# welcomyou/sherpa-vietnamese-asr

Measured on AMD Instinct MI355X. Metric: audio-sec/sec (xRT) Zipformer-68M offline decode, higher is better.
Workload: dtype bf16; 1 GPU; zipformer-68m greedy_search, batched planner chunks, 1 h per GPU; model=zipformer-68m, weights=greedy-calibrated, chunks_per_gpu=121, batch_pipeline=True, encoder_frames_per_gpu=98813

## Files before the change

include/zasr.h:

```cpp
#ifndef ZASR_H_
#define ZASR_H_

#include <stdint.h>

#ifdef __cplusplus
extern "C" {
#endif

typedef struct zasr_recognizer zasr_recognizer;
typedef struct zasr_result zasr_result;

enum {
  ZASR_OK = 0,
  ZASR_ERR_INVALID = 1,
  ZASR_ERR_NOT_FOUND = 2,
  ZASR_ERR_RUNTIME = 3,
};

enum {
  ZASR_PRECISION_FP32 = 0,
  ZASR_PRECISION_BF16 = 1,
  ZASR_PRECISION_BF16_ENC = 2,
  ZASR_PRECISION_BF16X3 = 3,
  ZASR_PRECISION_BF16X6 = 4,
  ZASR_PRECISION_F16X3 = 5
};

typedef struct zasr_config {
  const char* model_dir;
  const char* decoding_method;
  int32_t max_active_paths;
  float blank_penalty;
  const int32_t* hotword_tokens;
  const int32_t* hotword_lens;
  const float* hotword_scores;
  int32_t num_hotwords;
  int32_t device_id;
  int32_t precision;
} zasr_config;

int zasr_create(const zasr_config* cfg, zasr_recognizer** out);
void zasr_destroy(zasr_recognizer* h);

int zasr_convert_model(const char* model_dir, const char* out_dir);

int zasr_convert_stage_model(const char* kind, const char* model_dir, const char* out_dir);

int zasr_fbank(zasr_recognizer* h, const float* wav, int64_t n, int32_t sample_rate, float* out,
               int64_t cap, int64_t* n_frames);

int zasr_silence_flags(const float* d_wav, int64_t n, int32_t frame_len, float threshold,
                       uint8_t* d_flags, void* stream);

int zasr_decode_batch(zasr_recognizer* h, const float* const* wav, const int64_t* n,
                      int32_t count, int32_t beam, zasr_result** out);

int zasr_decode_features(zasr_recognizer* h, const float* const* feats, const int64_t* n_frames,
                         int32_t count, int32_t beam, zasr_result** out);

int zasr_decode_device(zasr_recognizer* h, const float* d_wav, const int64_t* wav_off,
                       const int64_t* n, int32_t count, int32_t beam, void* stream,
                       zasr_result** out);

int zasr_decode_device_batches(zasr_recognizer* h, const float* d_wav, const int64_t* wav_off,
                               const int64_t* n, int32_t count, const int32_t* batch_sizes,
                               int32_t n_batches, int32_t beam, void* stream, zasr_result** out);

int zasr_decode_host_batches(zasr_recognizer* h, const float* wav, const int64_t* wav_off,
                             const int64_t* n, int32_t count, const int32_t* batch_sizes,
                             int32_t n_batches, int32_t beam, void* stream, zasr_result** out);

int zasr_encode_features(zasr_recognizer* h, const float* const* feats, const int64_t* n_frames,
                         int32_t count, float* out, int64_t cap, int64_t* t_out);

int zasr_search_encoder_out(zasr_recognizer* h, const float* const* enc, const int64_t* t_out,
                            int32_t count, int32_t beam, zasr_result** out);

int32_t zasr_result_count(const zasr_result* r);
int32_t zasr_result_num_tokens(const zasr_result* r, int32_t i);
int32_t zasr_result_num_frames(const zasr_result* r, int32_t i);
const int32_t* zasr_result_tokens(const zasr_result* r, int32_t i);
const int32_t* zasr_result_frames(const zasr_result* r, int32_t i);
const double* zasr_result_log_probs(const zasr_result* r, int32_t i);
const float* zasr_result_token_stats(const zasr_result* r, int32_t i);
void zasr_result_free(zasr_result* r);

typedef struct zasr_stream zasr_stream;
int zasr_set_tokens(zasr_recognizer* h, const char* tokens_path);
int zasr_create_stream(zasr_recognizer* h, zasr_stream** out);
void zasr_destroy_stream(zasr_stream* s);
int zasr_stream_accept_waveform(zasr_stream* s, int32_t sample_rate, const float* samples,
                                int64_t n);
int zasr_decode_stream(zasr_recognizer* h, zasr_stream* s);
int zasr_decode_streams(zasr_recognizer* h, zasr_stream* const* streams, int32_t n);
int32_t zasr_stream_is_decoded(const zasr_stream* s);
int32_t zasr_stream_num_tokens(const zasr_stream* s);
int32_t zasr_stream_num_frames(const zasr_stream* s);
const int32_t* zasr_stream_tokens(const zasr_stream* s);
const int32_t* zasr_stream_frames(const zasr_stream* s);
const double* zasr_stream_log_probs(const zasr_stream* s);
const float* zasr_stream_token_stats(const zasr_stream* s);
int zasr_stream_result_json(const zasr_stream* s, char* buf, int64_t cap, int64_t* needed);

typedef struct zasr_campp zasr_campp;
int zasr_campp_create(const char* model_dir, int32_t device_id, zasr_campp** out);
void zasr_campp_destroy(zasr_campp* h);
int32_t zasr_campp_embedding_dim(const zasr_campp* h);
int zasr_campp_fbank(zasr_campp* h, const float* wav, int64_t n, float* out, int64_t cap,
                     int64_t* n_frames);
int zasr_campp_embed(zasr_campp* h, const float* feats, int32_t count, int32_t n_frames,
                     float* out);
int zasr_campp_embed_device(zasr_campp* h, const float* d_feats, int32_t count,
                            int32_t n_frames, float* d_out, void* stream);
int zasr_campp_windows_device(zasr_campp* h, const float* d_wav, const int64_t* region_off,
                              const int64_t* region_len, int32_t n_regions, int32_t window_frames,
                              int32_t step_frames, float* d_feats, int64_t max_windows,
                              int32_t* window_region, int32_t* window_first,
                              int32_t* window_nframes, int64_t* n_windows, void* stream);

typedef struct zasr_vibert zasr_vibert;
int zasr_vibert_create(const char* model_dir, int32_t device_id, zasr_vibert** out);
void zasr_vibert_destroy(zasr_vibert* h);
int32_t zasr_vibert_num_labels(const zasr_vibert* h);
int32_t zasr_vibert_num_detect(const zasr_vibert* h);
int zasr_vibert_run(zasr_vibert* h, const int64_t* input_ids, const int64_t* attention_mask,
                    const int64_t* token_type_ids, const int64_t* input_offsets, int32_t batch,
                    int32_t n_tokens, int32_t n_words, float* logits, float* detect_logits);

typedef struct zasr_vad zasr_vad;
int zasr_vad_create(const char* model_dir, int32_t device_id, zasr_vad** out);
void zasr_vad_destroy(zasr_vad* h);
int zasr_vad_probs(zasr_vad* h, const float* audio, const int64_t* offsets,
                   const int64_t* lengths, int32_t n_files, int32_t auto_boost, float* probs);
int zasr_vad_probs_device(zasr_vad* h, const float* d_audio, const int64_t* offsets,
                          const int64_t* lengths, int32_t n_files, int32_t auto_boost,
                          float* d_probs, void* stream);
int32_t zasr_vad_last_passes(const zasr_vad* h);
int zasr_vad_window(zasr_vad* h, const float* input, const float* state, int32_t n, float* prob,
                    float* state_out);

int32_t zasr_vocab_size(const zasr_recognizer* h);
int32_t zasr_joiner_dim(const zasr_recognizer* h);
int zasr_model_routes(zasr_recognizer* h, char* buf, int64_t cap);
int zasr_fbank_set_mel_banks(zasr_recognizer* h, const float* banks, int32_t n_bins);
int zasr_selftest_launch(int32_t block_threads);
int zasr_selftest_gemm_h3r(int32_t M, int32_t K, int32_t N, int32_t epi, const float* A,
                           const float* W, const float* bias, float* C);
int zasr_selftest_ffn_h3(int32_t R, int32_t D, int32_t F, const float* Y, const float* W1,
                         const float* b1, const float* W2, const float* b2,
                         const float* byp_orig, const float* byp_scale, float* X);
int zasr_selftest_ffn_bf16(int32_t R, int32_t D, int32_t F, const float* W1, const float* b1,
                           const float* W2, const float* b2, const float* byp_orig,
                           const float* byp_scale, float* X, int32_t form);
int zasr_selftest_ffn_bf16_oop(int32_t R, int32_t D, int32_t F, const float* W1, const float* b1,
                               const float* W2, const float* b2, const float* byp_orig,
                               const float* byp_scale, float* X, float* Xout, int32_t form);
int zasr_selftest_ffn_h3_oop(int32_t R, int32_t D, int32_t F, const float* W1, const float* b1,
                             const float* W2, const float* b2, const float* byp_orig,
                             const float* byp_scale, float* X, float* Xout);
int zasr_selftest_seam(int32_t nseq, const int32_t* L, int32_t d, int32_t ds, int32_t dn,
                       int32_t ds_next, int32_t c0, int32_t ldo, const float* xd,
                       const float* orig, const float* s, const float* wn8, const float* wo2,
                       float* next, float* xnext, float* out, float* next_ref, float* xnext_ref,
                       float* out_ref);
int zasr_selftest_attn_block_map(const int32_t* lens, int32_t nseq, int32_t units_per_seq,
                                 int32_t order, uint32_t* out, int64_t cap, int32_t* grid);

int zasr_profile_enable(zasr_recognizer* h, int32_t on);
int zasr_profile_reset(zasr_recognizer* h);
int zasr_profile_report(zasr_recognizer* h, char* buf, int64_t cap);

const char* zasr_last_error(void);
const char* zasr_version(void);

#ifdef __cplusplus
}
#endif
#endif
```

sherpa-vietnamese-asr_amd/csrc/engine.cpp:

```cpp
#include "engine.h"

#include <algorithm>
#include <cmath>
#include <cstring>
#include <deque>
#include <numeric>
#include <cstdlib>
#include <sstream>

#include "common.h"
#include "gemm.h"
#include "host_io.h"
#include "onnx_io.h"

namespace zasr {

namespace {
struct HwNode {
  int tok = -1;
  double tok_score = 0, node_score = 0, out_score = 0;
  bool is_end = false;
  std::vector<std::pair<int, int>> kids;
  int fail = 0, out = -1;
  int child(int t) const {
// ... 71 lines not shown
          break;
        }
      }
      nd[kid].out = o;
      if (o >= 0) nd[kid].out_score += nd[o].out_score;
      q.push_back(kid);
    }
  }
  dfa.tok2cls.assign(V, -1);
  std::vector<int> cls_tok;
  for (size_t i = 1; i < nd.size(); ++i) {
    int t = nd[i].tok;
    if (dfa.tok2cls[t] < 0) {
      dfa.tok2cls[t] = (int)cls_tok.size();
      cls_tok.push_back(t);
    }
  }
  dfa.num_states = (int)nd.size();
  dfa.num_cls = (int)cls_tok.size();
  dfa.next.resize((size_t)dfa.num_states * dfa.num_cls);
  dfa.delta.resize((size_t)dfa.num_states * dfa.num_cls);
  dfa.node_score.resize(dfa.num_states);
  for (int s = 0; s < dfa.num_states; ++s) {
    dfa.node_score[s] = nd[s].node_score;
    for (int c = 0; c < dfa.num_cls; ++c) {
      int t = cls_tok[c];
      int n;
      double score;
      int d = nd[s].child(t);
      if (d >= 0) {
        n = d;
        score = nd[n].tok_score;
      } else {
        n = nd[s].fail;
        while (nd[n].child(t) < 0) {
          n = nd[n].fail;
          if (nd[n].tok == -1) break;
        }
        int c2 = nd[n].child(t);
        if (c2 >= 0) n = c2;
        score = nd[n].node_score - nd[s].node_score;
      }
      if (nd[n].out_score != 0) {
        double matched = nd[n].is_end ? nd[n].node_score
                                      : (nd[n].out >= 0 ? nd[nd[n].out].node_score
                                                        : nd[n].node_score);
        score = score + matched - nd[n].node_score;
        n = 0;
      }
      dfa.next[(size_t)s * dfa.num_cls + c] = n;
      dfa.delta[(size_t)s * dfa.num_cls + c] = score;
    }
  }
  return dfa;
}

namespace {

ModelConfig parse_config(const std::string& text) {
  Json j = Json::parse(text);
  ModelConfig c;
  c.name = j.has("name") ? j.at("name").str : "zipformer";
  c.dims = j.at("encoder_dims").as_int_vec();
  c.layers = j.at("num_layers").as_int_vec();
  c.ff = j.at("ff_dims").as_int_vec();
  c.heads = j.at("num_heads").as_int_vec();
  c.ds = j.at("downsampling").as_int_vec();
  c.kernels = j.at("cnn_kernels").as_int_vec();
  c.qd = (int)j.at("query_head_dim").num;
  c.vd = (int)j.at("value_head_dim").num;
  c.pd = (int)j.at("pos_head_dim").num;
  c.pos_dim = (int)j.at("pos_dim").num;
  c.V = (int)j.at("vocab_size").num;
  c.dec_dim = (int)j.at("decoder_dim").num;
  c.joiner_dim = (int)j.at("joiner_dim").num;
  c.context = (int)j.at("context_size").num;
  if (j.has("layer1_channels")) c.c1 = (int)j.at("layer1_channels").num;
  if (j.has("layer2_channels")) c.c2 = (int)j.at("layer2_channels").num;
  if (j.has("layer3_channels")) c.c3 = (int)j.at("layer3_channels").num;
  ZASR_REQUIRE(c.qd == 32 && c.pd == 4, "kernels are specialised for query_head_dim 32, pos_head_dim 4");
  ZASR_REQUIRE(c.c1 == 8 && c.c2 == 32 && c.c3 == 128, "Conv2dSubsampling channels must be 8/32/128");
  ZASR_REQUIRE(c.context == 2, "decoder context_size must be 2");
  ZASR_REQUIRE(c.dec_dim == c.joiner_dim, "decoder_dim must equal joiner_dim");
  size_t ns = c.dims.size();
  ZASR_REQUIRE(c.layers.size() == ns && c.ff.size() == ns && c.heads.size() == ns &&
                   c.ds.size() == ns && c.kernels.size() == ns,
               "inconsistent stack config");
  for (size_t i = 0; i < ns; ++i) {
    ZASR_REQUIRE(c.dims[i] % 16 == 0, "encoder dims must be multiples of 16");
    ZASR_REQUIRE(c.ds[i] >= 1 && c.ds[i] <= 8, "downsampling factor must be 1..8");
  }
  return c;
}

}

template <class T>
T* Engine::ws(const std::string& name, size_t count) {
  size_t bytes = std::max<size_t>(count * sizeof(T), 256);
  Buf& b = ws_tag_.empty() ? ws_[name] : ws_[ws_tag_ + name];
  if (b.bytes < bytes) {
    if (b.p) {
      ZASR_HIP_CHECK(hipDeviceSynchronize());
      ZASR_HIP_CHECK(hipFree(b.p));
    }
    size_t alloc = bytes + bytes / 8;
    ZASR_HIP_CHECK(hipMalloc(&b.p, alloc));
    b.bytes = alloc;
  }
  return reinterpret_cast<T*>(b.p);
}

void Engine::upload(void* dst, const void* src, size_t bytes) {
  PinArena& a = pin_[pin_cur_];
  const size_t need = (bytes + 255) & ~size_t(255);
  if (a.used + need <= a.cap) {
    char* h = a.p + a.used;
    a.used += need;
    std::memcpy(h, src, bytes);
    ZASR_HIP_CHECK(hipMemcpyAsync(dst, h, bytes, hipMemcpyHostToDevice, st_));
    return;
  }
  a.want += need;
  ZASR_HIP_CHECK(hipMemcpyAsync(dst, src, bytes, hipMemcpyHostToDevice, st_));
}

void Engine::pin_reset(int arena) {
  PinArena& a = pin_[arena];
  const size_t want = std::max(a.want + a.used, a.cap);
  if (want > a.cap) {
    if (a.p) ZASR_HIP_CHECK(hipHostFree(a.p));
    a.cap = want + want / 4 + 4096;
    ZASR_HIP_CHECK(hipHostMalloc(reinterpret_cast<void**>(&a.p), a.cap, hipHostMallocDefault));
  }
  a.used = 0;
  a.want = 0;
  pin_cur_ = arena;
}

Engine::Engine(const std::string& dir, int device, int beam, bool greedy,
               const std::vector<std::vector<int>>& hotwords, const std::vector<float>& hotword_scores,
               int precision)
    : device_(device), beam_(beam), greedy_(greedy), precision_(precision) {
  ZASR_REQUIRE(precision >= 0 && precision <= 5,
               "precision must be 0 (fp32), 1 (bf16), 2 (bf16 encoder, f32 joiner + search), 3 "
               "(bf16x3: two-piece split-bf16 products), 4 (bf16x6: three-piece, f32 quality) or "
               "5 (f16x3: fp16 hi + scaled lo pieces, f32 quality)");
  SafeTensors W;
  ModelConfig cfg = parse_config(load_model_dir(dir, W));
  model_.cfg = cfg;
  hw_host_ = build_hotword_dfa(hotwords, hotword_scores, cfg.V);
  ZASR_HIP_CHECK(hipSetDevice(device_));
  if (const char* e = getenv("ZASR_SEARCH_CUS")) search_cus_ = atoi(e);
  int ncu = 0;
  ZASR_HIP_CHECK(hipDeviceGetAttribute(&ncu, hipDeviceAttributeMultiprocessorCount, device_));
  if (search_cus_ > 0 && search_cus_ < ncu) {
    std::vector<uint32_t> ms((ncu + 31) / 32, 0u), me((ncu + 31) / 32, 0u);
    for (int c = 0; c < ncu; ++c) (c < search_cus_ ? ms : me)[c / 32] |= 1u << (c % 32);
    ZASR_HIP_CHECK(hipExtStreamCreateWithCUMask(&stream2_, (uint32_t)ms.size(), ms.data()));
    ZASR_HIP_CHECK(hipExtStreamCreateWithCUMask(&stream3_, (uint32_t)ms.size(), ms.data()));
    ZASR_HIP_CHECK(hipExtStreamCreateWithCUMask(&stream_, (uint32_t)me.size(), me.data()));
    for (auto& x : enc_extra_)
      ZASR_HIP_CHECK(hipExtStreamCreateWithCUMask(&x, (uint32_t)me.size(), me.data()));
  } else {
    search_cus_ = 0;
    ZASR_HIP_CHECK(hipStreamCreateWithFlags(&stream_, hipStreamNonBlocking));
    int least = 0, greatest = 0;
    ZASR_HIP_CHECK(hipDeviceGetStreamPriorityRange(&least, &greatest));
    ZASR_HIP_CHECK(hipStreamCreateWithPriority(&stream2_, hipStreamNonBlocking, greatest));
    ZASR_HIP_CHECK(hipStreamCreateWithPriority(&stream3_, hipStreamNonBlocking, greatest));
    for (auto& x : enc_extra_) ZASR_HIP_CHECK(hipStreamCreateWithFlags(&x, hipStreamNonBlocking));
  }
  for (auto& e : part_ev_) ZASR_HIP_CHECK(hipEventCreateWithFlags(&e, hipEventDisableTiming));
  st_ = stream_;

  auto dev = [&](const float* src, size_t n) -> float* {
    float* p = nullptr;
    ZASR_HIP_CHECK(hipMalloc(&p, std::max<size_t>(n, 1) * sizeof(float)));
    ZASR_HIP_CHECK(hipMemcpy(p, src, n * sizeof(float), hipMemcpyHostToDevice));
    model_.allocations.push_back(p);
    return p;
  };
  auto tensor = [&](const std::string& name, std::initializer_list<int64_t> shape) {
    const HostTensor& t = W.get(name);
    std::vector<int64_t> want(shape);
    ZASR_REQUIRE(t.shape == want, "shape mismatch for " + name);
    return t;
  };
  auto lin = [&](const std::string& pre, int N, int K, bool bias = true) {
    DLin l;
    l.N = N;
    l.K = K;
    const float* hw = tensor(pre + ".weight", {N, K}).data;
    if (precision_ == 5) {
      for (size_t i = 0; i < (size_t)N * K; ++i)
        ZASR_REQUIRE(std::fabs(hw[i]) < 65504.f,
                     "precision f16x3: weight " + pre + " exceeds the fp16 range; use bf16x6");
    }
    l.w = dev(hw, (size_t)N * K);
    if (bias) l.b = dev(tensor(pre + ".bias", {N}).data, N);
    return l;
  };
  auto vec = [&](const std::string& name, int n) { return dev(tensor(name, {n}).data, n); };
  auto scalar = [&](const std::string& name) {
    const HostTensor& t = W.get(name);
    ZASR_REQUIRE(t.numel == 1, name + " must be a scalar");
    return t.data[0];
  };

  {
    const HostTensor& w0 = tensor("encoder_embed.conv.0.weight", {8, 1, 3, 3});
    model_.conv0_w = dev(w0.data, 72);
    model_.conv0_b = vec("encoder_embed.conv.0.bias", 8);
    const HostTensor& w4 = tensor("encoder_embed.conv.4.weight", {32, 8, 3, 3});
    std::vector<float> p4(32 * 72);
    for (int o = 0; o < 32; ++o)
      for (int c = 0; c < 8; ++c)
        for (int kk = 0; kk < 9; ++kk) p4[o * 72 + kk * 8 + c] = w4.data[(o * 8 + c) * 9 + kk];
    model_.conv4 = DLin{dev(p4.data(), p4.size()), vec("encoder_embed.conv.4.bias", 32), 32, 72};
    const HostTensor& w7 = tensor("encoder_embed.conv.7.weight", {128, 32, 3, 3});
    std::vector<float> p7(128 * 288);
    for (int o = 0; o < 128; ++o)
      for (int c = 0; c < 32; ++c)
        for (int kk = 0; kk < 9; ++kk) p7[o * 288 + kk * 32 + c] = w7.data[(o * 32 + c) * 9 + kk];
    model_.conv7 = DLin{dev(p7.data(), p7.size()), vec("encoder_embed.conv.7.bias", 128), 128, 288};
    model_.dw_w = dev(tensor("encoder_embed.convnext.depthwise_conv.weight", {128, 1, 7, 7}).data,
                      128 * 49);
    model_.dw_b = vec("encoder_embed.convnext.depthwise_conv.bias", 128);
    model_.pw1 = DLin{dev(tensor("encoder_embed.convnext.pointwise_conv1.weight", {384, 128, 1, 1})
                              .data, 384 * 128),
                      vec("encoder_embed.convnext.pointwise_conv1.bias", 384), 384, 128};
    model_.pw2 = DLin{dev(tensor("encoder_embed.convnext.pointwise_conv2.weight", {128, 384, 1, 1})
                              .data, 128 * 384),
                      vec("encoder_embed.convnext.pointwise_conv2.bias", 128), 128, 384};
    const int d0 = cfg.dims[0];
    const HostTensor& wo = tensor("encoder_embed.out.weight", {d0, 128 * 19});
    std::vector<float> po((size_t)d0 * 2432);
    for (int n = 0; n < d0; ++n)
      for (int c = 0; c < 128; ++c)
        for (int f = 0; f < 19; ++f) po[(size_t)n * 2432 + f * 128 + c] = wo.data[(size_t)n * 2432 + c * 19 + f];
    model_.out = DLin{dev(po.data(), po.size()), vec("encoder_embed.out.bias", d0), d0, 2432};
    model_.out_norm_b = vec("encoder_embed.out_norm.bias", d0);
    model_.out_norm_ls = scalar("encoder_embed.out_norm.log_scale");
  }
  const int qd = cfg.qd, vd = cfg.vd, pd = cfg.pd;
  for (size_t i = 0; i < cfg.dims.size(); ++i) {
    DStack s;
    s.d = cfg.dims[i];
    s.F = cfg.ff[i];
    s.h = cfg.heads[i];
    s.ds = cfg.ds[i];
    s.K = cfg.kernels[i];
    const int d = s.d, F = s.F, h = s.h;
    std::string pre = "encoder.encoders." + std::to_string(i) + ".";
    if (s.ds != 1) {
      const HostTensor& b = tensor(pre + "downsample.bias", {s.ds});
      double mx = -1e30, sum = 0;
      for (int u = 0; u < s.ds; ++u) mx = std::max(mx, (double)b.data[u]);
      std::vector<double> e(s.ds);
      for (int u = 0; u < s.ds; ++u) sum += (e[u] = std::exp((double)b.data[u] - mx));
      for (int u = 0; u < s.ds; ++u) s.ds_w[u] = (float)(e[u] / sum);
      s.comb = vec(pre + "out_combiner.bypass_scale", d);
      pre += "encoder.";
    }
    for (int j = 0; j < cfg.layers[i]; ++j) {
      DLayer L;
      std::string p = pre + "layers." + std::to_string(j) + ".";
      L.bypass = vec(p + "bypass.bypass_scale", d);
      L.bypass_mid = vec(p + "bypass_mid.bypass_scale", d);
      L.attn_in = lin(p + "self_attn_weights.in_proj", (2 * qd + pd) * h, d);
      const HostTensor& pw = tensor(p + "self_attn_weights.linear_pos.weight", {pd * h, cfg.pos_dim});
      L.pos_w.assign(pw.data, pw.data + pw.numel);
      for (int a = 0; a < 2; ++a) {
        std::string n = p + "self_attn" + std::to_string(a + 1);
        L.sa_in[a] = lin(n + ".in_proj", vd * h, d);
        L.sa_out[a] = lin(n + ".out_proj", d, vd * h);
      }
      const int fdims[3] = {(F * 3) / 4, F, (F * 5) / 4};
      for (int a = 0; a < 3; ++a) {
        std::string n = p + "feed_forward" + std::to_string(a + 1);
        L.ff_in[a] = lin(n + ".in_proj", fdims[a], d);
        L.ff_out[a] = lin(n + ".out_proj", d, fdims[a]);
      }
      const int hid = 3 * d / 4;
      L.na_in = lin(p + "nonlin_attention.in_proj", 3 * hid, d);
      L.na_out = lin(p + "nonlin_attention.out_proj", d, hid);
      for (int a = 0; a < 2; ++a) {
        std::string n = p + "conv_module" + std::to_string(a + 1);
        L.cv_in[a] = lin(n + ".in_proj", 2 * d, d);
        L.cv_out[a] = lin(n + ".out_proj", d, d);
        L.cv_dw_w[a] = dev(tensor(n + ".depthwise_conv.weight", {d, 1, s.K}).data, (size_t)d * s.K);
        L.cv_dw_b[a] = vec(n + ".depthwise_conv.bias", d);
      }
      L.norm_b = vec(p + "norm.bias", d);
      L.norm_ls = scalar(p + "norm.log_scale");
      s.layers.push_back(std::move(L));
    }
    model_.stacks.push_back(std::move(s));
  }
  {
    const HostTensor& b = tensor("encoder.downsample_output.bias", {2});
    double mx = std::max(b.data[0], b.data[1]);
    double e0 = std::exp(b.data[0] - mx), e1 = std::exp(b.data[1] - mx);
    model_.out_ds_w[0] = (float)(e0 / (e0 + e1));
    model_.out_ds_w[1] = (float)(e1 / (e0 + e1));
  }
// ... 86 lines not shown
            }
            ++routes_.ffn_fused_h3;
            for (auto [l, w] : {std::pair<DLin*, std::vector<float>*>{&L.ff_in[a], &w1},
                                std::pair<DLin*, std::vector<float>*>{&L.ff_out[a], &w2}}) {
              std::vector<__bf16> pk(2 * w->size());
              ffn_pack_h3_host(w->data(), l->N, l->K, pk.data());
              void* p = nullptr;
              ZASR_HIP_CHECK(hipMalloc(&p, pk.size() * 2));
              model_.allocations.push_back(p);
              ZASR_HIP_CHECK(hipMemcpy(p, pk.data(), pk.size() * 2, hipMemcpyHostToDevice));
              l->wp = p;
            }
          }
    }
    if (cfg.joiner_dim == 256 || cfg.joiner_dim == 512) {
      const long pe = gemm_rp_packed_elems(cfg.V, cfg.joiner_dim);
      void* p = nullptr;
      ZASR_HIP_CHECK(hipMalloc(&p, (size_t)pe * 2 * stored_pieces(split_pieces())));
      model_.allocations.push_back(p);
      for (int t = 0; t < stored_pieces(split_pieces()); ++t)
        gemm_rp_pack_weights(reinterpret_cast<const __bf16*>(model_.joiner.wx) + (long)t * cfg.V * cfg.joiner_dim,
                             cfg.V, cfg.joiner_dim, reinterpret_cast<__bf16*>(p) + t * pe, stream_);
      model_.joiner_packed = p;
      model_.joiner_plane = pe;
    }
    for (auto& s : model_.stacks)
      for (auto& L : s.layers) {
        for (int a = 0; a < 2; ++a) glu_interleave(L.cv_in[a]);
        for (DLin* l : {&L.attn_in, &L.na_in, &L.na_out}) mkx(*l);
        for (int a = 0; a < 2; ++a)
          for (DLin* l : {&L.sa_in[a], &L.sa_out[a], &L.cv_in[a], &L.cv_out[a]}) mkx(*l);
        for (int a = 0; a < 3; ++a)
          for (DLin* l : {&L.ff_in[a], &L.ff_out[a]}) mkx(*l);
      }
    ZASR_HIP_CHECK(hipStreamSynchronize(stream_));
    if (split_pieces() == kPiecesF16) {
      auto mkr = [&](DLin& l) {
        if (!gemm_h3r_supported(l.K, l.N, EPI_NONE)) return;
        std::vector<float> w((size_t)l.N * l.K);
        ZASR_HIP_CHECK(hipMemcpy(w.data(), l.w, w.size() * 4, hipMemcpyDeviceToHost));
        if (!ffn_h3_weights_ok(w.data(), (long)w.size())) {
          ++routes_.gemm_x3_range;
          return;
        }
        ++routes_.gemm_h3r;
        std::vector<__bf16> pk(2 * w.size());
        ffn_pack_h3_host(w.data(), l.N, l.K, pk.data());
        void* p = nullptr;
        ZASR_HIP_CHECK(hipMalloc(&p, pk.size() * 2));
        model_.allocations.push_back(p);
        ZASR_HIP_CHECK(hipMemcpy(p, pk.data(), pk.size() * 2, hipMemcpyHostToDevice));
        l.wr = p;
      };
      for (auto& s : model_.stacks)
        for (auto& L : s.layers) {
          for (DLin* l : {&L.attn_in, &L.na_in, &L.na_out}) mkr(*l);
          for (int a = 0; a < 2; ++a)
            for (DLin* l : {&L.sa_in[a], &L.sa_out[a], &L.cv_in[a], &L.cv_out[a]}) mkr(*l);
        }
      if (model_.pw1.K == 128 && model_.pw2.N == 128 && ffn_h3_supported(128, model_.pw1.N)) {
        std::vector<float> w1((size_t)model_.pw1.N * 128), w2(w1.size());
        ZASR_HIP_CHECK(hipMemcpy(w1.data(), model_.pw1.w, w1.size() * 4, hipMemcpyDeviceToHost));
        ZASR_HIP_CHECK(hipMemcpy(w2.data(), model_.pw2.w, w2.size() * 4, hipMemcpyDeviceToHost));
        const bool ok = ffn_h3_weights_ok(w1.data(), (long)w1.size()) && ffn_h3_weights_ok(w2.data(), (long)w2.size());
        routes_.cnx_ffn_h3 = ok ? 1 : 0;
        if (ok)
          for (auto [l, w] : {std::pair<DLin*, std::vector<float>*>{&model_.pw1, &w1},
                              std::pair<DLin*, std::vector<float>*>{&model_.pw2, &w2}}) {
            std::vector<__bf16> pk(2 * w->size());
            ffn_pack_h3_host(w->data(), l->N, l->K, pk.data());
            void* p = nullptr;
            ZASR_HIP_CHECK(hipMalloc(&p, pk.size() * 2));
            model_.allocations.push_back(p);
            ZASR_HIP_CHECK(hipMemcpy(p, pk.data(), pk.size() * 2, hipMemcpyHostToDevice));
            l->wr = p;
          }
      }
    }
  }
  if (precision_ == 1 || precision_ == 2) {
    for (auto& s : model_.stacks)
      for (auto& L : s.layers)
        for (int a = 0; a < 2; ++a) glu_interleave(L.cv_in[a]);
    auto mk = [&](DLin& l) {
      void* p = nullptr;
      ZASR_HIP_CHECK(hipMalloc(&p, (size_t)l.N * l.K * 2));
      model_.allocations.push_back(p);
      convert_to_bf16(l.w, p, (long)l.N * l.K, stream_);
      l.wh = p;
    };
    for (DLin* l : {&model_.conv4, &model_.conv7, &model_.pw1, &model_.pw2, &model_.out,
                    &model_.enc_proj})
      mk(*l);
    if (precision_ == 1) mk(model_.joiner);
    if (precision_ == 1 && (cfg.joiner_dim == 256 || cfg.joiner_dim == 512)) {
      void* p = nullptr;
      ZASR_HIP_CHECK(hipMalloc(&p, (size_t)gemm_rp_packed_elems(cfg.V, cfg.joiner_dim) * 2));
      model_.allocations.push_back(p);
      gemm_rp_pack_weights(model_.joiner.wh, cfg.V, cfg.joiner_dim, p, stream_);
      model_.joiner_packed = p;
    }
    for (auto& s : model_.stacks)
      for (auto& L : s.layers) {
        {
          DLin& l = L.attn_in;
          const int h = s.h;
          std::vector<float> rs(l.N, 1.f), bias(l.N);
          const float kLog2e = 1.4426950408889634f;
          for (int r = 0; r < l.N; ++r)
            if (r < 32 * h || r >= 64 * h) rs[r] = kLog2e;
          ZASR_HIP_CHECK(hipMemcpy(bias.data(), l.b, l.N * sizeof(float), hipMemcpyDeviceToHost));
          for (int r = 0; r < l.N; ++r) bias[r] *= rs[r];
          float* d_rs = dev(rs.data(), rs.size());
          l.bh = dev(bias.data(), bias.size());
          void* p = nullptr;
          ZASR_HIP_CHECK(hipMalloc(&p, (size_t)l.N * l.K * 2));
          model_.allocations.push_back(p);
          convert_rows_to_bf16(l.w, d_rs, p, l.N, l.K, stream_);
          l.wh = p;
        }
        for (DLin* l : {&L.na_in, &L.na_out}) mk(*l);
        for (int a = 0; a < 2; ++a)
          for (DLin* l : {&L.sa_in[a], &L.sa_out[a], &L.cv_in[a], &L.cv_out[a]}) mk(*l);
        for (int a = 0; a < 3; ++a)
          for (DLin* l : {&L.ff_in[a], &L.ff_out[a]}) mk(*l);
      }
    ZASR_HIP_CHECK(hipStreamSynchronize(stream_));
    for (DLin* l : {&model_.pw1, &model_.pw2}) {
      std::vector<__bf16> h((size_t)l->N * l->K), pk(h.size());
      ZASR_HIP_CHECK(hipMemcpy(h.data(), l->wh, h.size() * 2, hipMemcpyDeviceToHost));
      pack_frag32_host(h.data(), l->N, l->K, pk.data());
      void* p = nullptr;
      ZASR_HIP_CHECK(hipMalloc(&p, pk.size() * 2));
      model_.allocations.push_back(p);
      ZASR_HIP_CHECK(hipMemcpy(p, pk.data(), pk.size() * 2, hipMemcpyHostToDevice));
      l->wp = p;
    }
    for (auto& s : model_.stacks)
      for (auto& L : s.layers)
        for (int a = 0; a < 3; ++a) {
          const int F = L.ff_in[a].N, d = L.ff_in[a].K;
          if (d < 256 || !ffn_fused_supported(d) || F % 32 != 0 || F > 2048) continue;
          for (DLin* l : {&L.ff_in[a], &L.ff_out[a]}) {
            std::vector<__bf16> h((size_t)l->N * l->K), pk(h.size());
            ZASR_HIP_CHECK(hipMemcpy(h.data(), l->wh, h.size() * 2, hipMemcpyDeviceToHost));
            ffn_pack_host(h.data(), l->N, l->K, pk.data());
            void* p = nullptr;
            ZASR_HIP_CHECK(hipMalloc(&p, pk.size() * 2));
            model_.allocations.push_back(p);
            ZASR_HIP_CHECK(hipMemcpy(p, pk.data(), pk.size() * 2, hipMemcpyHostToDevice));
            l->wp = p;
          }
        }
  }
  {
    const double gb = (double)cfg.V * cfg.V * cfg.joiner_dim * 4.0 / 1e9;
    double max_gb = 24.0;
    if (const char* e = getenv("ZASR_DEC_TABLE_MAX_GB")) max_gb = atof(e);
    if (gb <= max_gb) {
      void* p = nullptr;
      ZASR_HIP_CHECK(hipMalloc(&p, (size_t)cfg.V * cfg.V * cfg.joiner_dim * sizeof(float)));
      model_.allocations.push_back(p);
      model_.dec_table = reinterpret_cast<float*>(p);
      DecoderW dw{model_.dec_tap0, model_.dec_tap1, model_.dec_proj.b, cfg.joiner_dim};
      launch_dec_table(dw, model_.dec_proj.w, cfg.V, model_.dec_table, stream_);
      ZASR_HIP_CHECK(hipStreamSynchronize(stream_));
    }
  }

  {
    std::vector<double> tw(512);
    for (int j = 0; j < 256; ++j) {
      double a = -2.0 * M_PI * j / 512.0;
      tw[2 * j] = std::cos(a);
      tw[2 * j + 1] = std::sin(a);
    }
    ZASR_HIP_CHECK(hipMalloc(&d_twiddle_, 512 * sizeof(double)));
    ZASR_HIP_CHECK(hipMemcpy(d_twiddle_, tw.data(), 512 * sizeof(double), hipMemcpyHostToDevice));
    std::vector<float> win(400);
    for (int i = 0; i < 400; ++i)
      win[i] = (float)std::pow(0.5 - 0.5 * std::cos(2.0 * M_PI / 399.0 * i), 0.85);
    d_window_ = dev(win.data(), 400);
    auto mel = [](float f) { return 1127.0f * logf(1.0f + f / 700.0f); };
    const float mlo = mel(20.0f), mhi = mel(7600.0f);
    const float delta = (mhi - mlo) / 81.0f;
    std::vector<float> banks(80 * 256, 0.f);
    for (int b = 0; b < 80; ++b) {
      float left = mlo + (float)b * delta, center = mlo + (float)(b + 1) * delta,
            right = mlo + (float)(b + 2) * delta;
      for (int i = 0; i < 256; ++i) {
        float m = mel(31.25f * (float)i);
        if (m > left && m < right)
          banks[b * 256 + i] = (m <= center) ? (m - left) / (center - left) : (right - m) / (right - center);
      }
    }
    set_mel_banks(banks.data(), 256);
  }
  hw_.num_states = hw_host_.num_states;
  hw_.num_cls = hw_host_.num_cls;
  if (hw_host_.num_states > 0) {
    int *t2c = nullptr, *nx = nullptr;
    double *dl = nullptr, *ns = nullptr;
    ZASR_HIP_CHECK(hipMalloc(&t2c, hw_host_.tok2cls.size() * sizeof(int)));
    ZASR_HIP_CHECK(hipMalloc(&nx, std::max<size_t>(hw_host_.next.size(), 1) * sizeof(int)));
    ZASR_HIP_CHECK(hipMalloc(&dl, std::max<size_t>(hw_host_.delta.size(), 1) * sizeof(double)));
    ZASR_HIP_CHECK(hipMalloc(&ns, hw_host_.node_score.size() * sizeof(double)));
    ZASR_HIP_CHECK(hipMemcpy(t2c, hw_host_.tok2cls.data(), hw_host_.tok2cls.size() * sizeof(int), hipMemcpyHostToDevice));
    ZASR_HIP_CHECK(hipMemcpy(nx, hw_host_.next.data(), hw_host_.next.size() * sizeof(int), hipMemcpyHostToDevice));
    ZASR_HIP_CHECK(hipMemcpy(dl, hw_host_.delta.data(), hw_host_.delta.size() * sizeof(double), hipMemcpyHostToDevice));
    ZASR_HIP_CHECK(hipMemcpy(ns, hw_host_.node_score.data(), hw_host_.node_score.size() * sizeof(double), hipMemcpyHostToDevice));
    model_.allocations.push_back(t2c);
    model_.allocations.push_back(nx);
    model_.allocations.push_back(dl);
    model_.allocations.push_back(ns);
    hw_.tok2cls = t2c;
    hw_.next = nx;
    hw_.delta = dl;
    hw_.node_score = ns;
  }
  ZASR_HIP_CHECK(hipHostMalloc(reinterpret_cast<void**>(&h_pinned_), 64, hipHostMallocDefault));
  ZASR_HIP_CHECK(hipDeviceSynchronize());
}

void Engine::set_mel_banks(const float* banks, int n_bins) {
  ZASR_REQUIRE(n_bins == 256 || n_bins == 257, "mel banks: 256 or 257 bins per filter");
  std::vector<int> meta(240);
  std::vector<float> wts;
  for (int b = 0; b < 80; ++b) {
    const float* row = banks + (size_t)b * n_bins;
    if (n_bins == 257)
      ZASR_REQUIRE(row[256] == 0.f, "mel banks: the Nyquist bin must carry no weight");
    int st = -1, en = -1;
    for (int i = 0; i < 256; ++i)
      if (row[i] != 0.f) {
        if (st < 0) st = i;
        en = i;
      }
    if (st < 0) st = en = 0;
    meta[b] = st;
    meta[80 + b] = en - st + 1;
    meta[160 + b] = (int)wts.size();
    for (int i = st; i <= en; ++i) wts.push_back(row[i]);
  }
  ZASR_HIP_CHECK(hipDeviceSynchronize());
  if (!d_mel_meta_) ZASR_HIP_CHECK(hipMalloc(&d_mel_meta_, 240 * sizeof(int)));
  ZASR_HIP_CHECK(hipMemcpy(d_mel_meta_, meta.data(), 240 * sizeof(int), hipMemcpyHostToDevice));
  if (d_mel_w_) ZASR_HIP_CHECK(hipFree(d_mel_w_));
  d_mel_w_ = nullptr;
  ZASR_HIP_CHECK(hipMalloc(&d_mel_w_, wts.size() * sizeof(float)));
  ZASR_HIP_CHECK(hipMemcpy(d_mel_w_, wts.data(), wts.size() * sizeof(float), hipMemcpyHostToDevice));
}

std::string Engine::routes_json() const {
  std::ostringstream os;
  os << "{\"precision\": " << precision_ << ", \"ffn_fused_h3\": " << routes_.ffn_fused_h3
     << ", \"ffn_gemm_pair\": " << routes_.ffn_gemm_pair << ", \"gemm_h3r\": " << routes_.gemm_h3r
     << ", \"gemm_x3_range\": " << routes_.gemm_x3_range << ", \"cnx_ffn_h3\": " << routes_.cnx_ffn_h3
     << ", \"dec_table\": " << (model_.dec_table ? 1 : 0) << "}";
  return os.str();
}

Engine::~Engine() {
  (void)hipSetDevice(device_);
  (void)hipStreamSynchronize(stream_);
  for (void* p : model_.allocations) (void)hipFree(p);
  for (auto& s : model_.stacks)
    for (auto& l : s.layers)
      if (l.pos_tab) (void)hipFree(l.pos_tab);
  for (auto& kv : ws_)
    if (kv.second.p) (void)hipFree(kv.second.p);
  if (d_twiddle_) (void)hipFree(d_twiddle_);
  if (d_mel_meta_) (void)hipFree(d_mel_meta_);
  if (d_mel_w_) (void)hipFree(d_mel_w_);
  for (auto e : event_pool_) (void)hipEventDestroy(e);
  for (auto& pe : prof_pending_) {
    (void)hipEventDestroy(pe.a);
    (void)hipEventDestroy(pe.b);
  }
  if (copy_st_) (void)hipStreamSynchronize(copy_st_);
  for (auto e : upload_ev_)
    if (e) (void)hipEventDestroy(e);
  if (copy_st_) (void)hipStreamDestroy(copy_st_);
  (void)hipStreamSynchronize(stream2_);
  (void)hipStreamSynchronize(stream3_);
  if (stream4_) (void)hipStreamSynchronize(stream4_);
  if (h_pinned_) (void)hipHostFree(h_pinned_);
  for (auto& r : res_pin_)
    if (r.p) (void)hipHostFree(r.p);
  for (auto& a : pin_)
    if (a.p) (void)hipHostFree(a.p);
  for (auto e : part_ev_) (void)hipEventDestroy(e);
  (void)hipStreamDestroy(stream2_);
  (void)hipStreamDestroy(stream3_);
  if (stream4_) (void)hipStreamDestroy(stream4_);
  for (auto x : enc_extra_) {
    (void)hipStreamSynchronize(x);
    (void)hipStreamDestroy(x);
  }
  (void)hipStreamDestroy(stream_);
}

void Engine::ensure_pos_tables(int need) {
  if (need <= model_.pmax) return;
  ZASR_HIP_CHECK(hipDeviceSynchronize());
  int pmax = 1024;
  while (pmax < need) pmax *= 2;
// ... 80 lines not shown
    acc.second += ms;
    event_pool_.push_back(pe.a);
    event_pool_.push_back(pe.b);
  }
  prof_pending_.clear();
  std::ostringstream os;
  for (auto& kv : prof_acc_) os << kv.first << " " << kv.second.first << " " << kv.second.second << "\n";
  return os.str();
}

std::string Engine::shape_key(const char* cls, int M, int K, int N, bool w16, bool a16, bool c16,
                              int epi) {
  std::ostringstream os;
  os << cls << "|" << M << "|" << K << "|" << N << "|" << (int)w16 << "|" << (int)a16 << "|"
     << (int)c16 << "|" << epi;
  return os.str();
}

void Engine::linear(const DLin& l, const float* A, int lda, int M, float* C, int ldc, int epi,
                    const char* cls, const float* byp_orig, const float* byp_scale) {
  GemmParams p{};
  p.A = A;
  p.lda = lda;
  p.B = l.w;
  p.sbk = 1;
  p.sbn = l.K;
  p.C = C;
  p.ldc = ldc;
  p.bias = l.b;
  p.M = M;
  p.N = l.N;
  p.K = l.K;
  p.alpha = 1.f;
  p.max_M = M;
  ZASR_REQUIRE(byp_orig == nullptr || l.wx, "bypass epilogue: split-mode weights only");
  p.byp_orig = byp_orig;
  p.byp_scale = byp_scale;
  if (prof_shapes_ && prof_on_)
    prof_begin(shape_key(cls, M, l.K, l.N, l.wh != nullptr, false, false, epi));
  else
    prof_begin(cls);
  if (l.wr && lda == l.K && byp_orig == nullptr && gemm_h3r_supported(l.K, l.N, epi))
    gemm_h3r(A, l.wr, l.b, C, ldc, M, l.N, l.K, epi, st_);
  else if (l.wx)
    gemm_x3(p, l.wx, (long)l.N * l.K, epi, ALOAD_DENSE, st_, split_pieces());
  else if (l.wh)
    gemm_bf16(p, l.wh, epi, ALOAD_DENSE, st_);
  else
    gemm_f32(p, epi, ALOAD_DENSE, false, st_);
  prof_end();
}

void Engine::linear_h(const DLin& l, const void* A, bool a_bf16, int lda, int M, void* C,
                      bool c_bf16, int ldc, int epi, const float* byp_orig,
                      const float* byp_scale) {
  ZASR_REQUIRE(l.wh != nullptr, "linear_h needs bf16 weights");
  GemmParams p{};
  p.A = reinterpret_cast<const float*>(A);
  p.lda = lda;
  p.B = l.w;
  p.sbk = 1;
  p.sbn = l.K;
  p.C = reinterpret_cast<float*>(C);
  p.ldc = ldc;
  p.bias = l.bh ? l.bh : l.b;
  p.M = M;
  p.N = l.N;
  p.K = l.K;
  p.alpha = 1.f;
  p.max_M = M;
  p.byp_orig = byp_orig;
  p.byp_scale = byp_scale;
  if (prof_shapes_ && prof_on_)
    prof_begin(shape_key("enc_gemm", M, l.K, l.N, true, a_bf16, c_bf16, epi));
  else
    prof_begin("enc_gemm");
  gemm_bf16(p, l.wh, epi, ALOAD_DENSE, st_, a_bf16, c_bf16);
  prof_end();
}

void Engine::run_fbank(const float* d_wav, const std::vector<long>& wav_off,
                       const std::vector<long>& n, float* d_feats, std::vector<int>& frames) {
  const int B = (int)n.size();
  std::vector<long> off(B);
  std::vector<int> ns(B), fo(B + 1, 0);
  frames.resize(B);
  for (int b = 0; b < B; ++b) {
    off[b] = wav_off[b];
    ns[b] = (int)n[b];
    frames[b] = n[b] > 0 ? (int)((n[b] + 80) / 160) : 0;
    fo[b + 1] = fo[b] + frames[b];
  }
  long* d_off = ws<long>("fb_wavoff", B);
  int* d_meta = ws<int>("fb_meta", 2 * B + 1);
  std::vector<int> meta(ns);
  meta.insert(meta.end(), fo.begin(), fo.end());
  upload(d_off, off.data(), B * sizeof(long));
  upload(d_meta, meta.data(), meta.size() * sizeof(int));
  FbankTables t{d_twiddle_, d_window_, d_mel_meta_, d_mel_meta_ + 80, d_mel_meta_ + 160, d_mel_w_};
  prof_begin("fbank");
  launch_fbank(d_wav, d_off, d_meta, d_meta + B, B, fo[B], t, d_feats, st_);
  prof_end();
}

namespace {
struct LevelMeta {
  std::vector<int> len;
  std::vector<int> off;
  int total = 0, maxlen = 0;
};
LevelMeta make_level(const std::vector<int>& len) {
  LevelMeta m;
  m.len = len;
  m.off.assign(len.size() + 1, 0);
  for (size_t b = 0; b < len.size(); ++b) {
    m.off[b + 1] = m.off[b] + len[b];
    m.maxlen = std::max(m.maxlen, len[b]);
  }
  m.total = m.off.back();
  return m;
}
struct MetaPack {
  std::vector<char> bytes;
  size_t add(const void* p, size_t n) {
    size_t at = (bytes.size() + 15) & ~size_t(15);
    bytes.resize(at + n);
    if (n) std::memcpy(bytes.data() + at, p, n);
    return at;
  }
};
}

bool Engine::ff1_fused(const DStack& S, const DLayer& Ly) const {
  const DLin& fi = Ly.ff_in[0];
  if (fi.wh) return ffn_fused_supported(S.d) && (S.d < 256 || fi.wp);
  return fi.wp && split_pieces() == kPiecesF16 && ffn_h3_oop_ok(S.d);
}

float* Engine::layer_forward(const DStack& S, const DLayer& Ly, float* X, float* Xalt, int R,
                             const int* d_off, const int* d_map,
                             const std::vector<int>& lens, const long* d_aoff,
                             const void* d_slices_nl, int maxL, const int* d_o8, int R8,
                             const AttnBlockMaps& bm, bool orig_ready, bool copy_for_next) {
  const int d = S.d, h = S.h, B = (int)lens.size();
  const int hid = 3 * d / 4;
  const bool oop = ff1_fused(S, Ly);
  float* O = X;
  if (!oop) {
    O = ws<float>("ly_orig", (size_t)R * d);
    if (!orig_ready)
      ZASR_HIP_CHECK(hipMemcpyAsync(O, X, (size_t)R * d * sizeof(float), hipMemcpyDeviceToDevice, st_));
  }
  const bool bf16 = precision_ == 1 || precision_ == 2;
  const int np = split_pieces();
  float* qkp = nullptr;
  float* A = nullptr;
  __bf16* A16 = nullptr;
  float* stats = nullptr;
  AttnFlashArgs fa{};
  if (bf16) {
    __bf16* qkp16 = ws<__bf16>("ly_qkp_h", (size_t)R * 68 * h);
    linear_h(Ly.attn_in, X, false, d, R, qkp16, true, 68 * h, EPI_NONE);
    A16 = ws<__bf16>("ly_attn_h", 1);
    stats = ws<float>("ly_attn_stats", (size_t)R * h);
    fa = AttnFlashArgs{qkp16, h, Ly.pos_tab, model_.pmax, d_off, d_aoff, B, maxL, A16,
                       nullptr, nullptr, stats, stats};
  } else if (np) {
    qkp = ws<float>("ly_qkp", (size_t)R * 68 * h);
    linear(Ly.attn_in, X, d, R, qkp, 68 * h, EPI_NONE);
    A = ws<float>("ly_attn", 1);
    stats = ws<float>("ly_attn_stats", (size_t)R * h);
    fa = AttnFlashArgs{qkp, h, Ly.pos_tab, model_.pmax, d_off, d_aoff, B, maxL, A,
                       nullptr, nullptr, stats, stats, np};
    if (np != kPiecesF16) {
      AttnFlashArgs a = fa;
      a.map = bm.head0;
      a.map_len = bm.n_head0;
      prof_begin("attn_softmax");
      launch_attn_flash(a, 0, st_);
      prof_end();
    }
  } else {
    qkp = ws<float>("ly_qkp", (size_t)R * 68 * h);
    linear(Ly.attn_in, X, d, R, qkp, 68 * h, EPI_NONE);
    A = ws<float>("ly_attn", 1);
    stats = ws<float>("ly_attn_stats", (size_t)R * h * 2);
    AttnArgs a{qkp, h, Ly.pos_tab, model_.pmax, d_off, d_aoff, B, maxL, A, stats, 1};
    prof_begin("attn_softmax");
    launch_attn_softmax(a, st_);
    prof_end();
  }
  auto ff = [&](int k, const float* src = nullptr) {
    const DLin& fi = Ly.ff_in[k];
    const float* bo = (bf16 && k == 1) ? O : nullptr;
    const float* bs = (bf16 && k == 1) ? Ly.bypass_mid : nullptr;
    if (fi.wh && ffn_fused_supported(d) && (d < 256 || fi.wp)) {
      prof_begin("ffn_fused");
      launch_ffn_fused(X, R, d, fi.N, d < 256 ? fi.wh : fi.wp, fi.b,
                       d < 256 ? Ly.ff_out[k].wh : Ly.ff_out[k].wp, Ly.ff_out[k].b, st_, bo, bs, src);
      prof_end();
      return;
    }
    ZASR_REQUIRE(src == nullptr || (!fi.wh && fi.wp && np == kPiecesF16),
                 "feed-forward: only the fused kernels run out of place");
    if (fi.wh) {
      __bf16* H = ws<__bf16>("ly_hid_h", (size_t)R * fi.N);
      linear_h(fi, X, false, d, R, H, true, fi.N, EPI_SWOOSHL);
      linear_h(Ly.ff_out[k], H, true, fi.N, R, X, false, d, EPI_RESADD, bo, bs);
    } else if (fi.wp && np == kPiecesF16) {
      prof_begin("ffn_fused");
      launch_ffn_fused_h3(X, R, d, fi.N, fi.wp, fi.b, Ly.ff_out[k].wp, Ly.ff_out[k].b, st_,
                          k == 1 ? O : nullptr, k == 1 ? Ly.bypass_mid : nullptr, nullptr, src);
      prof_end();
    } else {
      const bool byp = k == 1 && Ly.ff_out[k].wx != nullptr;
      float* H = ws<float>("ly_hid", (size_t)R * fi.N);
      linear(fi, X, d, R, H, fi.N, EPI_SWOOSHL);
      linear(Ly.ff_out[k], H, fi.N, R, X, d, EPI_RESADD, "enc_gemm", byp ? O : nullptr,
             byp ? Ly.bypass_mid : nullptr);
    }
  };
  auto self_attn = [&](int k) {
    if (bf16) {
      __bf16* vv = ws<__bf16>("ly_vv_h", (size_t)R * 12 * h);
      __bf16* oa = ws<__bf16>("ly_oa_h", (size_t)R * 12 * h);
      linear_h(Ly.sa_in[k], X, false, d, R, vv, true, 12 * h, EPI_NONE);
      AttnFlashArgs a = fa;
      a.v = vv;
      a.out = oa;
      a.map = bm.heads;
      a.map_len = bm.n_heads;
      prof_begin("attn_apply");
      launch_attn_flash(a, k == 0 ? 1 : 2, st_);
      prof_end();
      linear_h(Ly.sa_out[k], oa, true, 12 * h, R, X, false, d, EPI_RESADD);
      return;
    }
    float* vv = ws<float>("ly_vv", (size_t)R * 12 * h);
    float* oa = ws<float>("ly_oa", (size_t)R * 12 * h);
    linear(Ly.sa_in[k], X, d, R, vv, 12 * h, EPI_NONE);
    if (np) {
      AttnFlashArgs a = fa;
      a.v = vv;
      a.out = oa;
      a.map = bm.heads;
      a.map_len = bm.n_heads;
      prof_begin("attn_apply");
      launch_attn_flash(a, k == 0 ? 1 : 2, st_);
      prof_end();
      linear(Ly.sa_out[k], oa, 12 * h, R, X, d, EPI_RESADD);
      return;
    }
    AttnSAArgs sa{qkp, h, Ly.pos_tab, model_.pmax, d_off, B, maxL, stats, vv, oa, stats};
    prof_begin("attn_apply");
    launch_attn_sa(sa, k == 0, false, st_);
    prof_end();
    linear(Ly.sa_out[k], oa, 12 * h, R, X, d, EPI_RESADD);
  };
  auto conv = [&](int k) {
    if (Ly.cv_in[k].wh) {
      __bf16* dc = ws<__bf16>("ly_dc_h", (size_t)R * d);
      if (Ly.cv_in[k].glu) {
        __bf16* g = ws<__bf16>("ly_glu_h", (size_t)R * d);
        linear_h(Ly.cv_in[k], X, false, d, R, g, true, d, EPI_GLU);
        prof_begin("dwconv1d");
        launch_dwconv1d_post_glu_bf16(g, d_off, d_map, R, d, S.K, Ly.cv_dw_w[k], Ly.cv_dw_b[k], dc, st_);
        prof_end();
      } else {
        __bf16* g2 = ws<__bf16>("ly_g2_h", (size_t)R * 2 * d);
        linear_h(Ly.cv_in[k], X, false, d, R, g2, true, 2 * d, EPI_NONE);
        prof_begin("dwconv1d");
        launch_glu_dwconv1d_bf16(g2, d_off, d_map, R, d, S.K, Ly.cv_dw_w[k], Ly.cv_dw_b[k], dc, st_);
        prof_end();
      }
      linear_h(Ly.cv_out[k], dc, true, d, R, X, false, d, EPI_RESADD);
      return;
    }
    float* dc = ws<float>("ly_dc", (size_t)R * d);
    if (Ly.cv_in[k].glu) {
      float* g = ws<float>("ly_glu", (size_t)R * d);
      linear(Ly.cv_in[k], X, d, R, g, d, EPI_GLU);
      prof_begin("dwconv1d");
      launch_dwconv1d_post_glu(g, d_off, d_map, R, d, S.K, Ly.cv_dw_w[k], Ly.cv_dw_b[k], dc, st_);
      prof_end();
    } else {
      float* g2 = ws<float>("ly_g2", (size_t)R * 2 * d);
      linear(Ly.cv_in[k], X, d, R, g2, 2 * d, EPI_NONE);
      prof_begin("dwconv1d");
      launch_glu_dwconv1d(g2, d_off, d_map, R, d, S.K, Ly.cv_dw_w[k], Ly.cv_dw_b[k], dc, st_);
      prof_end();
    }
    linear(Ly.cv_out[k], dc, d, R, X, d, EPI_RESADD);
  };
  if (oop) {
    X = Xalt;
    ff(0, O);
  } else {
    ff(0);
  }
  if (bf16) {
    __bf16* h3 = ws<__bf16>("ly_h3_h", (size_t)R * 3 * hid);
    __bf16* t1t = ws<__bf16>("ly_t1t", (size_t)hid * R8);
    __bf16* z = ws<__bf16>("ly_z_h", (size_t)R * hid);
    linear_h(Ly.na_in, X, false, d, R, h3, true, 3 * hid, EPI_NONE);
    prof_begin("elementwise");
    launch_nonlin_prep_t(h3, true, d_off, d_o8, d_map, R, hid, R8, t1t, st_);
    prof_end();
    AttnFlashArgs a = fa;
    a.t1t = t1t;
    a.o8 = d_o8;
    a.ldt = R8;
    a.hid = hid;
    a.y = h3 + 2 * hid;
    a.ldy = 3 * hid;
    a.z = z;
    a.map = bm.head0;
    a.map_len = bm.n_head0;
    prof_begin("attn_nonlin");
    launch_attn_flash(a, 3, st_);
    prof_end();
    linear_h(Ly.na_out, z, true, hid, R, X, false, d, EPI_RESADD);
  } else if (np) {
    float* h3 = ws<float>("ly_h3", (size_t)R * 3 * hid);
    __bf16* t1t = ws<__bf16>("ly_t1t_x", (size_t)stored_pieces(np) * hid * R8);
    float* z = ws<float>("ly_z", (size_t)R * hid);
    linear(Ly.na_in, X, d, R, h3, 3 * hid, EPI_NONE);
    prof_begin("elementwise");
    launch_nonlin_prep_t(h3, false, d_off, d_o8, d_map, R, hid, R8, t1t, st_, np);
    prof_end();
    if (np == kPiecesF16) {
      AttnFlashArgs a = fa;
      a.t1t = t1t;
      a.o8 = d_o8;
      a.ldt = R8;
      a.hid = hid;
      a.y = h3 + 2 * hid;
      a.ldy = 3 * hid;
      a.z = z;
      a.map = bm.head0;
      a.map_len = bm.n_head0;
      prof_begin("attn_nonlin");
      launch_attn_flash(a, 3, st_);
      prof_end();
    } else {
    GemmParams p{};
    p.A = A;
    p.B = nullptr;
    p.sbk = 1;
    p.sbn = R8;
    p.C = z;
    p.ldc = hid;
    p.N = hid;
    p.alpha = 1.f;
    p.aux = h3 + 2 * hid;
    p.ldaux = 3 * hid;
    p.slices = reinterpret_cast<const GemmSlice*>(d_slices_nl);
    p.num_slices = B;
    p.max_M = maxL;
    prof_begin("attn_nonlin");
    gemm_x3(p, t1t, (long)hid * R8, EPI_MULAUX, ALOAD_DENSE, st_, np);
    prof_end();
    }
    linear(Ly.na_out, z, hid, R, X, d, EPI_RESADD);
  } else {
    float* h3 = ws<float>("ly_h3", (size_t)R * 3 * hid);
    float* t1 = ws<float>("ly_t1", (size_t)R * hid);
    float* z = ws<float>("ly_z", (size_t)R * hid);
    linear(Ly.na_in, X, d, R, h3, 3 * hid, EPI_NONE);
    prof_begin("elementwise");
    launch_nonlin_prep(h3, t1, R, hid, st_);
    prof_end();
    GemmParams p{};
    p.A = A;
    p.B = t1;
    p.sbk = hid;
    p.sbn = 1;
    p.C = z;
    p.ldc = hid;
    p.N = hid;
    p.alpha = 1.f;
    p.aux = h3 + 2 * hid;
    p.ldaux = 3 * hid;
    p.slices = reinterpret_cast<const GemmSlice*>(d_slices_nl);
    p.num_slices = B;
    p.max_M = maxL;
    prof_begin("attn_nonlin");
    gemm_f32(p, EPI_MULAUX, ALOAD_DENSE, true, st_);
    prof_end();
    linear(Ly.na_out, z, hid, R, X, d, EPI_RESADD);
  }
  self_attn(0);
  conv(0);
  ff(1);
  if (!bf16 && Ly.ff_out[1].wx == nullptr) {
    prof_begin("elementwise");
    launch_bypass(X, O, Ly.bypass_mid, R, d, st_);
    prof_end();
  }
  self_attn(1);
  conv(1);
  ff(2);
  prof_begin("elementwise");
  launch_bias_norm(X, R, d, Ly.norm_b, Ly.norm_ls, O, Ly.bypass, st_,
                   copy_for_next ? ws<float>("ly_orig", (size_t)R * d) : nullptr);
  prof_end();
  return X;
}

void Engine::run_encoder(const float* d_feats, const std::vector<int>& T, float* d_enc,
                         std::vector<int>& t_out) {
  const ModelConfig& cfg = model_.cfg;
  const int B = (int)T.size();
  std::vector<int> t1(B), l2(B), L(B), tout(B);
  for (int b = 0; b < B; ++b) {
    ZASR_REQUIRE(T[b] >= 9, "encoder needs >= 9 fbank frames per chunk");
    t1[b] = T[b] - 2;
    l2[b] = (T[b] - 3) / 2;
    L[b] = (T[b] - 7) / 2;
    tout[b] = (L[b] + 1) / 2;
  }
  t_out = tout;
  LevelMeta mfb = make_level(T), mc1 = make_level(t1), mc2 = make_level(l2), mL = make_level(L),
            mout = make_level(tout);
  const int ns = (int)model_.stacks.size();
  std::vector<LevelMeta> mst(ns);
  std::vector<std::vector<long>> aoff(ns);
  std::vector<std::vector<GemmSlice>> sl_nl(ns);
  std::vector<std::vector<int>> o8(ns);
  std::vector<int> R8(ns, 0);
  const bool bf16 = precision_ == 1 || precision_ == 2;
  const bool flash = bf16 || split_pieces() > 0;
  size_t attn_floats = 0;
  int maxL_all = 0;
  for (int i = 0; i < ns; ++i) {
    const DStack& s = model_.stacks[i];
    std::vector<int> len(B);
    for (int b = 0; b < B; ++b) len[b] = (L[b] + s.ds - 1) / s.ds;
    mst[i] = make_level(len);
    maxL_all = std::max(maxL_all, mst[i].maxlen);
    long acc = 0;
    const int hid = 3 * s.d / 4;
    int c8 = 0;
    for (int b = 0; b < B; ++b) {
      const int Lb = len[b], L4 = (Lb + 3) & ~3, L8 = (Lb + 31) & ~31;
      const int Lp = flash ? L8 : L4;
      aoff[i].push_back(acc);
      o8[i].push_back(c8);
      GemmSlice g{};
      g.a_off = acc;
      g.b_off = flash ? (long)c8 : (long)mst[i].off[b] * hid;
      g.c_off = (long)mst[i].off[b] * hid;
      g.aux_off = (long)mst[i].off[b] * 3 * hid;
      g.M = Lb;
      g.K = flash ? L8 : Lb;
      g.lda = Lp;
      sl_nl[i].push_back(g);
      acc += (long)Lb * Lp;
      c8 += L8;
    }
    o8[i].push_back(c8);
    R8[i] = c8;
    attn_floats = std::max(attn_floats, (size_t)acc);
  }
  ensure_pos_tables(maxL_all + 192);
  std::vector<GemmSlice> sl_c2(B), sl_c3(B);
  for (int b = 0; b < B; ++b) {
    sl_c2[b] = GemmSlice{(long)mc1.off[b] * 640, 0, (long)mc2.off[b] * 39 * 32, 0, l2[b] * 39, 72, 0, 0};
    sl_c3[b] = GemmSlice{(long)mc2.off[b] * 39 * 32, 0, (long)mL.off[b] * 19 * 128, 0, L[b] * 19, 288, 0, 0};
  }
  MetaPack mp;
  size_t o_fb = mp.add(mfb.off.data(), (B + 1) * 4), o_c1 = mp.add(mc1.off.data(), (B + 1) * 4),
         o_L = mp.add(mL.off.data(), (B + 1) * 4), o_out = mp.add(mout.off.data(), (B + 1) * 4);
  size_t o_c2s = mp.add(sl_c2.data(), B * sizeof(GemmSlice)),
         o_c3s = mp.add(sl_c3.data(), B * sizeof(GemmSlice));
  std::vector<size_t> o_st(ns), o_ao(ns), o_sn(ns), o_o8(ns), o_bmh(ns), o_bm0(ns);
  std::vector<int> n_bmh(ns, 0), n_bm0(ns, 0);
  std::vector<unsigned> bmap;
  for (int i = 0; i < ns; ++i) {
    o_st[i] = mp.add(mst[i].off.data(), (B + 1) * 4);
    o_o8[i] = mp.add(o8[i].data(), (B + 1) * 4);
    o_ao[i] = mp.add(aoff[i].data(), B * sizeof(long));
    o_sn[i] = mp.add(sl_nl[i].data(), sl_nl[i].size() * sizeof(GemmSlice));
    if (flash) {
      const DStack& s = model_.stacks[i];
      const int np = split_pieces();
      const bool fused_nl = bf16 || np == kPiecesF16;
      n_bmh[i] = build_attn_block_map(mst[i].len.data(), B, s.h, 0, bmap);
      o_bmh[i] = mp.add(bmap.data(), bmap.size() * sizeof(unsigned));
      n_bm0[i] = build_attn_block_map(mst[i].len.data(), B,
                                      fused_nl ? attn_nonlin_chunks(3 * s.d / 4, bf16 ? 1 : np) : 1,
                                      0, bmap);
      o_bm0[i] = mp.add(bmap.data(), bmap.size() * sizeof(unsigned));
    }
  }
  char* d_meta = ws<char>("enc_meta", mp.bytes.size());
  upload(d_meta, mp.bytes.data(), mp.bytes.size());
  auto I = [&](size_t o) { return reinterpret_cast<const int*>(d_meta + o); };
  int* c1_map = ws<int>("map_c1", mc1.total);
  int* L_map = ws<int>("map_L", mL.total);
  int* out_map = ws<int>("map_out", mout.total);
  launch_row2seq(I(o_c1), B, mc1.total, c1_map, st_);
  launch_row2seq(I(o_L), B, mL.total, L_map, st_);
  launch_row2seq(I(o_out), B, mout.total, out_map, st_);
  std::vector<int*> st_map(ns);
  for (int i = 0; i < ns; ++i) {
    st_map[i] = ws<int>("map_st" + std::to_string(i), mst[i].total);
    launch_row2seq(I(o_st[i]), B, mst[i].total, st_map[i], st_);
  }

  const bool fe16 = model_.conv4.wh != nullptr && model_.conv7.wh != nullptr;
  void* c1 = fe16 ? (void*)ws<__bf16>("fe_c1_h", (size_t)mc1.total * 640)
                  : (void*)ws<float>("fe_c1", (size_t)mc1.total * 640);
  prof_begin("frontend_conv");
  launch_conv1(d_feats, I(o_fb), I(o_c1), c1_map, mc1.total, model_.conv0_w, model_.conv0_b, c1,
               fe16, st_, split_pieces() == kPiecesF16);
  prof_end();
  void* c2 = fe16 ? (void*)ws<__bf16>("fe_c2_h", (size_t)mc2.total * 39 * 32)
                  : (void*)ws<float>("fe_c2", (size_t)mc2.total * 39 * 32);
  {
    GemmParams p{};
    p.A = reinterpret_cast<const float*>(c1);
    p.B = model_.conv4.w;
    p.sbk = 1;
    p.sbn = 72;
    p.C = reinterpret_cast<float*>(c2);
    p.ldc = 32;
    p.bias = model_.conv4.b;
    p.N = 32;
    p.alpha = 1.f;
    p.slices = reinterpret_cast<const GemmSlice*>(d_meta + o_c2s);
    p.num_slices = B;
    p.max_M = mc2.maxlen * 39;
    prof_begin("frontend_conv");
    if (fe16)
      gemm_bf16(p, model_.conv4.wh, EPI_SWOOSHR, ALOAD_CONV2, st_, true, true);
    else if (model_.conv4.wx)
      gemm_x3(p, model_.conv4.wx, 32L * 72, EPI_SWOOSHR, ALOAD_CONV2, st_, split_pieces());
    else if (model_.conv4.wh)
      gemm_bf16(p, model_.conv4.wh, EPI_SWOOSHR, ALOAD_CONV2, st_);
    else
      gemm_f32(p, EPI_SWOOSHR, ALOAD_CONV2, false, st_);
    prof_end();
  }
  const int d0 = cfg.dims[0];
  float* e0 = ws<float>("fe_e0", (size_t)mL.total * d0);
  {
// ... 831 lines not shown
```

sherpa-vietnamese-asr_amd/csrc/engine.h:

```cpp
#pragma once
#include <hip/hip_runtime.h>

#include <map>
#include <mutex>
#include <string>
#include <vector>

#include "gemm.h"
#include "kernels.h"

namespace zasr {

struct ModelConfig {
  std::string name;
  std::vector<int> dims, layers, ff, heads, ds, kernels;
  int qd = 32, vd = 12, pd = 4, pos_dim = 48;
  int V = 0, dec_dim = 0, joiner_dim = 0, context = 2;
  int c1 = 8, c2 = 32, c3 = 128;
  int max_dim() const {
    int m = 0;
    for (int d : dims) m = d > m ? d : m;
    return m;
  }
};
// ... 33 lines not shown
  ModelConfig cfg;
  float *conv0_w = nullptr, *conv0_b = nullptr;
  DLin conv4, conv7, pw1, pw2, out, enc_proj, dec_proj, joiner;
  float *dw_w = nullptr, *dw_b = nullptr;
  float* out_norm_b = nullptr;
  float out_norm_ls = 0.f;
  std::vector<DStack> stacks;
  float out_ds_w[2] = {0, 0};
  float* dec_emb = nullptr;
  float* dec_conv = nullptr;
  void* joiner_packed = nullptr;
  long joiner_plane = 0;
  float* dec_table = nullptr;
  float* dec_tap0 = nullptr;
  float* dec_tap1 = nullptr;
  int pmax = 0;
  std::vector<void*> allocations;
};

struct HotwordDFA {
  int num_states = 0, num_cls = 0;
  std::vector<int> tok2cls, next;
  std::vector<double> delta, node_score;
};
HotwordDFA build_hotword_dfa(const std::vector<std::vector<int>>& phrases,
                             const std::vector<float>& scores, int V);

struct TokenResult {
  std::vector<int> tok, frame;
  std::vector<double> lp;
  std::vector<float> stats;
  int t_out = 0;
};

class Engine {
 public:
  Engine(const std::string& model_dir, int device, int beam, bool greedy,
         const std::vector<std::vector<int>>& hotwords, const std::vector<float>& hotword_scores,
         int precision);
  ~Engine();

  int vocab() const { return model_.cfg.V; }
  int joiner_dim() const { return model_.cfg.joiner_dim; }
  int default_beam() const { return beam_; }
  hipStream_t stream() const { return stream_; }

  std::vector<TokenResult> decode_device(const float* d_wav, const std::vector<long>& wav_off,
                                         const std::vector<long>& n, int beam, hipStream_t st);
  std::vector<TokenResult> decode_device_batches(const float* d_wav, const std::vector<long>& wav_off,
                                                 const std::vector<long>& n,
                                                 const std::vector<int>& batch_sizes, int beam,
                                                 hipStream_t st);
  std::vector<TokenResult> decode_host_batches(const float* h_wav, const std::vector<long>& wav_off,
                                               const std::vector<long>& n,
                                               const std::vector<int>& batch_sizes, int beam,
                                               hipStream_t st);
  std::vector<TokenResult> decode_features(const std::vector<const float*>& feats,
                                           const std::vector<long>& frames, int beam);
  void fbank_host(const float* wav, long n, float* out);
  void encode_host(const std::vector<const float*>& feats, const std::vector<long>& frames,
                   std::vector<float>& out, std::vector<int>& t_out);
  std::vector<TokenResult> search_host(const std::vector<const float*>& enc,
                                       const std::vector<long>& t_out, int beam);

  void profile_enable(int mode) {
    prof_on_ = mode > 0;
    prof_shapes_ = mode == 2;
  }
  void profile_reset();
  std::string profile_report();

  std::string routes_json() const;
  void set_mel_banks(const float* banks, int n_bins);

  std::mutex mu;

 private:
  struct Buf {
    void* p = nullptr;
    size_t bytes = 0;
  };
  template <class T>
  T* ws(const std::string& name, size_t count);
  void upload(void* dst, const void* src, size_t bytes);

  struct Pending {
    int B = 0;
    std::vector<int> valid, t_out;
    float* enc = nullptr;
    hipEvent_t ready = nullptr;
  };
  void encode_stage(const float* d_wav, const std::vector<long>& wav_off, const std::vector<long>& n,
                    int out_slot, int ws_slot, hipStream_t stream, Pending& p);
  std::vector<TokenResult> search_stage(Pending& p, int beam);
  std::vector<TokenResult> decode_batches_two_searches(const float* d_wav,
                                                       const std::vector<long>& wav_off,
                                                       const std::vector<long>& n,
                                                       const std::vector<int>& batch_sizes,
                                                       int beam, hipStream_t main_st);
  struct PinArena {
    char* p = nullptr;
    size_t cap = 0, used = 0, want = 0;
  };
  static constexpr int kMaxEnc = 3;
  static constexpr int kMaxJobs = 3;
  PinArena pin_[kMaxEnc + 1 + kMaxJobs];
  std::string ws_tag_;
  int pin_cur_ = 0;
  void pin_reset(int arena);

  void run_fbank(const float* d_wav, const std::vector<long>& wav_off, const std::vector<long>& n,
                 float* d_feats, std::vector<int>& frames);
  void run_encoder(const float* d_feats, const std::vector<int>& T, float* d_enc,
                   std::vector<int>& t_out);
  std::vector<TokenResult> run_search(const float* d_enc, const std::vector<int>& t_out, int beam);
  struct SearchJob {
    int S_all = 0, S = 0, cap = 0, set = 0, Tmax = 0;
    std::vector<int> order, t_out;
    bool check_finite = false;
    hipStream_t stream = nullptr;
  };
  void launch_search(const float* d_enc, const std::vector<int>& t_out, int beam, int set,
                     hipStream_t stream, bool split_groups, SearchJob& job);
  std::vector<TokenResult> collect_search(SearchJob& job);
  struct ResPin {
    char* p = nullptr;
    size_t cap = 0;
  };
  ResPin res_pin_[kMaxJobs];
  float* layer_forward(const DStack& stk, const DLayer& ly, float* X, float* Xalt, int R,
                       const int* d_off, const int* d_map, const std::vector<int>& lens,
                       const long* d_aoff, const void* d_slices_nl, int maxL, const int* d_o8,
                       int R8, const AttnBlockMaps& bm, bool orig_ready, bool copy_for_next);
  bool ff1_fused(const DStack& stk, const DLayer& ly) const;
  void linear(const DLin& l, const float* A, int lda, int M, float* C, int ldc, int epi,
              const char* cls = "enc_gemm", const float* byp_orig = nullptr,
              const float* byp_scale = nullptr);
  void linear_h(const DLin& l, const void* A, bool a_bf16, int lda, int M, void* C, bool c_bf16,
                int ldc, int epi, const float* byp_orig = nullptr,
                const float* byp_scale = nullptr);
  void ensure_pos_tables(int max_len);

  struct ProfEvent {
    std::string name;
    hipEvent_t a, b;
  };
  void prof_begin(const char* name);
  void prof_begin(const std::string& name);
  void prof_end();
  static std::string shape_key(const char* cls, int M, int K, int N, bool w16, bool a16,
                               bool c16, int epi);
  bool prof_on_ = false;
  bool prof_shapes_ = false;
  std::vector<ProfEvent> prof_pending_;
  std::map<std::string, std::pair<long, double>> prof_acc_;
  std::vector<hipEvent_t> event_pool_;
  hipEvent_t take_event();

  DModel model_;
  struct Routes {
    int ffn_fused_h3 = 0, ffn_gemm_pair = 0;
    int gemm_h3r = 0, gemm_x3_range = 0;
    int cnx_ffn_h3 = -1;
  } routes_;
  int device_ = 0;
  int beam_ = 8;
  [[maybe_unused]] bool greedy_ = false;
  void order_after_encoders(const hipStream_t* enc_st, int E, hipStream_t main_st);
  int precision_ = 0;
  int split_pieces() const {
    return precision_ == 3 ? 2 : precision_ == 4 ? 3 : precision_ == 5 ? kPiecesF16 : 0;
  }
  hipStream_t stream_ = nullptr;
  hipStream_t stream2_ = nullptr;
  hipStream_t stream3_ = nullptr;
  hipStream_t stream4_ = nullptr;
  int search_cus_ = 0;
  hipStream_t enc_extra_[kMaxEnc - 1] = {};
  hipEvent_t part_ev_[kMaxEnc + 4 + kMaxJobs] = {};
  hipStream_t st_ = nullptr;
  const float* host_wav_ = nullptr;
  hipStream_t copy_st_ = nullptr;
  hipEvent_t upload_ev_[kMaxEnc + 1] = {};
  std::map<std::string, Buf> ws_;
  double* d_twiddle_ = nullptr;
  float* d_window_ = nullptr;
  int* d_mel_meta_ = nullptr;
  float* d_mel_w_ = nullptr;
  int* h_pinned_ = nullptr;
  HotwordDFA hw_host_;
  HotwordTables hw_{};
};

}
```

sherpa-vietnamese-asr_amd/csrc/ffn_kernels.hip:

```cpp
#include <cmath>
#include <cstring>
#include <cstdlib>
#include <type_traits>
#include <vector>

#include "common.h"
#include "kernels.h"

namespace zasr {

#ifdef ZASR_FFN_STAMPS
__device__ long long g_ffn_stamps[4896];
#define FFN_STAMP(i) \
  if (blockIdx.x == 0 && threadIdx.x == 0 && (i) < 4896) g_ffn_stamps[(i)] = clock64();
#else
#define FFN_STAMP(i)
#endif

namespace {

__device__ __forceinline__ void lds_barrier() {
  asm volatile("s_waitcnt lgkmcnt(0)" ::: "memory");
  __builtin_amdgcn_s_barrier();
}

typedef float f32x16 __attribute__((ext_vector_type(16)));
typedef __bf16 bf16x8 __attribute__((ext_vector_type(8)));
typedef __bf16 bf16x4 __attribute__((ext_vector_type(4)));

constexpr int kTok = 128;
constexpr int kMaxF = 2048;
constexpr int kW2Ld = 40;

__device__ __forceinline__ int w2_slot(int k) { return (k & 0x13) | ((k & 4) << 1) | ((k & 8) >> 1); }

__device__ __forceinline__ __amdgpu_buffer_rsrc_t wave_rsrc(const void* p, long bytes) {
  const unsigned lo = __builtin_amdgcn_readfirstlane((unsigned)(unsigned long)p);
  const unsigned hi = __builtin_amdgcn_readfirstlane((unsigned)((unsigned long)p >> 32));
  const int n = __builtin_amdgcn_readfirstlane((int)bytes);
  return __builtin_amdgcn_make_buffer_rsrc((void*)(((unsigned long)hi << 32) | lo), 0, n, 0x00020000);
}
template <typename V>
__device__ __forceinline__ V buf_load16(__amdgpu_buffer_rsrc_t rs, int voff, int soff) {
  return __builtin_bit_cast(V, __builtin_amdgcn_raw_buffer_load_b128(rs, voff, soff, 0));
}

}

__device__ __forceinline__ void lds_wait_ge(int* p, int target) {
  while (__hip_atomic_load(p, __ATOMIC_ACQUIRE, __HIP_MEMORY_SCOPE_WORKGROUP) < target)
    __builtin_amdgcn_s_sleep(1);
}
__device__ __forceinline__ void lds_signal(int* p, int lane) {
  asm volatile("s_waitcnt lgkmcnt(0)" ::: "memory");
  if (lane == 0) __hip_atomic_fetch_add(p, 1, __ATOMIC_RELEASE, __HIP_MEMORY_SCOPE_WORKGROUP);
}

template <int D, bool OOP = false>
__global__ __launch_bounds__(256, (D <= 192 ? 2 : 1)) void ffn_fused_kernel(float* __restrict__ X, int R, int F,
                                                           const __bf16* __restrict__ W1,
                                                           const float* __restrict__ b1,
                                                           const __bf16* __restrict__ W2,
                                                           const float* __restrict__ b2,
                                                           const float* __restrict__ byp_orig,
                                                           const float* __restrict__ byp_scale,
                                                           const float* __restrict__ Xsrc) {
  const float* Xin = OOP ? Xsrc : X;
  constexpr int KS = D / 16;
  constexpr int OT = D / 32;
  constexpr int W1LD = D + 8;
  constexpr int W1P = 32 * D / 8;
  constexpr int W2P = D * 4;
  constexpr int P1 = (W1P + 255) / 256, P2 = (W2P + 255) / 256;
  __shared__ __attribute__((aligned(16))) __bf16 sW1[2][32 * W1LD];
  __shared__ __attribute__((aligned(16))) __bf16 sW2[2][D * kW2Ld];
  __shared__ float sB1[2][32];

  const int tid = threadIdx.x, lane = tid & 63, wid = tid >> 6;
  const int col = lane & 31, h2 = lane >> 5;
  const int tok = blockIdx.x * kTok + wid * 32 + col;
  const int tokc = tok < R ? tok : R - 1;
  const int nch = (F + 31) / 32;

  bf16x8 g1[P1], g2[P2];
  float gb = 0.f;
  auto gload = [&](int c) {
#pragma unroll
    for (int i = 0; i < P1; ++i) {
      const int e = tid + 256 * i < W1P ? tid + 256 * i : W1P - 1;
      const int row = e / (D / 8), k8 = e - row * (D / 8);
      int hr = c * 32 + row;
      hr = hr < F ? hr : F - 1;
      g1[i] = *reinterpret_cast<const bf16x8*>(W1 + (long)hr * D + 8 * k8);
    }
#pragma unroll
    for (int i = 0; i < P2; ++i) {
      const int e = tid + 256 * i < W2P ? tid + 256 * i : W2P - 1;
      const int row = e >> 2, q = e & 3;
      const int k0 = c * 32 + 8 * q;
      bf16x8 v = *reinterpret_cast<const bf16x8*>(W2 + (long)row * F + (k0 < F ? k0 : 0));
      if (k0 >= F) {
#pragma unroll
        for (int t = 0; t < 8; ++t) v[t] = (__bf16)0.f;
      }
      g2[i] = v;
    }
    const int bi = c * 32 + (tid & 31);
    const float bv = b1[bi < F ? bi : F - 1];
    gb = bi < F ? bv : 0.f;
  };
  auto sstore = [&](int buf) {
#pragma unroll
    for (int i = 0; i < P1; ++i) {
      const int e = tid + 256 * i;
      if (e < W1P) {
        const int row = e / (D / 8), k8 = e - row * (D / 8);
        *reinterpret_cast<bf16x8*>(&sW1[buf][row * W1LD + 8 * k8]) = g1[i];
      }
    }
#pragma unroll
    for (int i = 0; i < P2; ++i) {
      const int e = tid + 256 * i;
      if (e >= W2P) break;
      const int row = e >> 2, q = e & 3;
      bf16x4 lo, hi;
      lo[0] = g2[i][0]; lo[1] = g2[i][1]; lo[2] = g2[i][2]; lo[3] = g2[i][3];
      hi[0] = g2[i][4]; hi[1] = g2[i][5]; hi[2] = g2[i][6]; hi[3] = g2[i][7];
      *reinterpret_cast<bf16x4*>(&sW2[buf][row * kW2Ld + w2_slot(8 * q)]) = lo;
      *reinterpret_cast<bf16x4*>(&sW2[buf][row * kW2Ld + w2_slot(8 * q + 4)]) = hi;
    }
    if (tid < 32) sB1[buf][tid] = gb;
  };

  gload(0);
  bf16x8 xf[KS];
  {
    const float* xr = Xin + (long)tokc * D + 8 * h2;
#pragma unroll
    for (int s = 0; s < KS; ++s) {
      const float4 a = *reinterpret_cast<const float4*>(xr + 16 * s);
      const float4 b = *reinterpret_cast<const float4*>(xr + 16 * s + 4);
      xf[s][0] = (__bf16)a.x; xf[s][1] = (__bf16)a.y; xf[s][2] = (__bf16)a.z; xf[s][3] = (__bf16)a.w;
      xf[s][4] = (__bf16)b.x; xf[s][5] = (__bf16)b.y; xf[s][6] = (__bf16)b.z; xf[s][7] = (__bf16)b.w;
    }
  }
  sstore(0);
  __syncthreads();

  f32x16 o[OT];
#pragma unroll
  for (int t = 0; t < OT; ++t)
#pragma unroll
    for (int r = 0; r < 16; ++r) o[t][r] = 0.f;

  for (int c = 0; c < nch; ++c) {
    const int cur = c & 1;
    if (c + 1 < nch) gload(c + 1);
    f32x16 hacc;
#pragma unroll
    for (int r = 0; r < 16; ++r) hacc[r] = 0.f;
    const __bf16* w1 = &sW1[cur][col * W1LD + 8 * h2];
#pragma unroll
    for (int s = 0; s < KS; ++s)
      hacc = __builtin_amdgcn_mfma_f32_32x32x16_bf16(*reinterpret_cast<const bf16x8*>(w1 + 16 * s),
                                                     xf[s], hacc, 0, 0, 0);
    bf16x8 pf[2];
#pragma unroll
    for (int r = 0; r < 16; ++r) {
      const int hrow = (r & 3) + 8 * (r >> 2) + 4 * h2;
      pf[r >> 3][r & 7] = (__bf16)swooshl_fast(hacc[r] + sB1[cur][hrow]);
    }
#pragma unroll
    for (int t = 0; t < OT; ++t) {
      const __bf16* w2 = &sW2[cur][(t * 32 + col) * kW2Ld + 8 * h2];
      o[t] = __builtin_amdgcn_mfma_f32_32x32x16_bf16(*reinterpret_cast<const bf16x8*>(w2), pf[0], o[t], 0, 0, 0);
      o[t] = __builtin_amdgcn_mfma_f32_32x32x16_bf16(*reinterpret_cast<const bf16x8*>(w2 + 16), pf[1], o[t], 0, 0, 0);
    }
    if (c + 1 < nch) sstore(cur ^ 1);
    __syncthreads();
  }

  if (tok >= R) return;
  float* xr = X + (long)tok * D;
  const float* xi = OOP ? Xin + (long)tok * D : xr;
#pragma unroll
  for (int t = 0; t < OT; ++t)
#pragma unroll
    for (int g = 0; g < 4; ++g) {
      const int ch = t * 32 + 8 * g + 4 * h2;
      const float4 bb = *reinterpret_cast<const float4*>(b2 + ch);
      float4 v = *reinterpret_cast<const float4*>(xi + ch);
      v.x += o[t][4 * g + 0] + bb.x;
      v.y += o[t][4 * g + 1] + bb.y;
      v.z += o[t][4 * g + 2] + bb.z;
      v.w += o[t][4 * g + 3] + bb.w;
      if (byp_orig != nullptr) {
        const float4 b0 = *reinterpret_cast<const float4*>(byp_orig + (long)tok * D + ch);
        const float4 k = *reinterpret_cast<const float4*>(byp_scale + ch);
        v.x = b0.x + (v.x - b0.x) * k.x;
        v.y = b0.y + (v.y - b0.y) * k.y;
        v.z = b0.z + (v.z - b0.z) * k.z;
        v.w = b0.w + (v.w - b0.w) * k.w;
      }
      *reinterpret_cast<float4*>(xr + ch) = v;
    }
}

template <int D, bool EB = true, bool OOP = false>
__global__ __launch_bounds__(512, 1) void ffn_wide_kernel(float* __restrict__ X, int R, int F,
                                                          const __bf16* __restrict__ W1,
                                                          const float* __restrict__ b1,
                                                          const __bf16* __restrict__ W2,
                                                          const float* __restrict__ b2,
                                                          const float* __restrict__ byp_orig,
                                                          const float* __restrict__ byp_scale,
                                                          const float* __restrict__ Xsrc) {
  const float* Xin = OOP ? Xsrc : X;
  typedef float f32x4 __attribute__((ext_vector_type(4)));
  constexpr int TT = 64, HC = 128, NW = 8;
  constexpr int XLD = D + 16, HLD = HC + 16;
  constexpr int KS = D / 32;
  constexpr int OW = D / NW, OT = OW / 16;
  __shared__ __attribute__((aligned(16))) __bf16 sX[TT * XLD];
  constexpr int NB = D >= 384 ? 2 : 1;
  __shared__ __attribute__((aligned(16))) __bf16 sH[NB][TT * HLD];
  __shared__ __attribute__((aligned(16))) float sB1[kMaxF];

  const int tid = threadIdx.x, lane = tid & 63;
  const int wid = __builtin_amdgcn_readfirstlane(tid >> 6);
  const int r16 = lane & 15, g4 = lane >> 4;
  const long t0 = (long)blockIdx.x * TT;

  FFN_STAMP(0)
  {
    constexpr int NE = TT * D / 4 / (64 * NW);
    float4 v[NE];
#pragma unroll
    for (int i = 0; i < NE; ++i) {
      const int e = tid + 64 * NW * i, row = e / (D / 4), c4 = e - row * (D / 4);
      const long r = t0 + row < R ? t0 + row : R - 1;
      v[i] = *reinterpret_cast<const float4*>(Xin + r * D + 4 * c4);
    }
#pragma unroll
    for (int i = 0; i < NE; ++i) {
      const int e = tid + 64 * NW * i, row = e / (D / 4), c4 = e - row * (D / 4);
      bf16x4 b;
      b[0] = (__bf16)v[i].x; b[1] = (__bf16)v[i].y; b[2] = (__bf16)v[i].z; b[3] = (__bf16)v[i].w;
      *reinterpret_cast<bf16x4*>(&sX[row * XLD + 4 * c4]) = b;
    }
  }

  f32x4 o[OT][4];
#pragma unroll
  for (int t = 0; t < OT; ++t)
#pragma unroll
    for (int u = 0; u < 4; ++u) o[t][u] = f32x4{0.f, 0.f, 0.f, 0.f};

  const int nch = (F + HC - 1) / HC;
  const int S2 = F / 32;
  bf16x8 w1f[KS];
  auto load_w1 = [&](int c) {
    const int rg = min((c * HC) / 16 + wid, F / 16 - 1);
    const __bf16* p = W1 + ((long)rg * KS * 64 + lane) * 8;
#pragma unroll
    for (int s = 0; s < KS; ++s) w1f[s] = *reinterpret_cast<const bf16x8*>(p + s * 512);
  };
#ifndef ZASR_FFN_W2SETS
#define ZASR_FFN_W2SETS 2
#endif

  constexpr int W2S = ZASR_FFN_W2SETS;
  bf16x8 w2f[W2S][4][OT];
  auto load_w2 = [&](int c, auto set) {
    constexpr int S = decltype(set)::value;
#pragma unroll
    for (int s = 0; s < 4; ++s) {
      const int ks = min(c * (HC / 32) + s, S2 - 1);
#pragma unroll
      for (int t = 0; t < OT; ++t)
        w2f[S][s][t] = *reinterpret_cast<const bf16x8*>(W2 + (((long)(wid * OW / 16 + t) * S2 + ks) * 64 + lane) * 8);
    }
  };
  using I0 = std::integral_constant<int, 0>;
  using I1 = std::integral_constant<int, W2S - 1>;
  load_w1(0);
  load_w2(0, I0{});
  for (int e = tid; e < F; e += 64 * NW) sB1[e] = b1[e];
  lds_barrier();
  FFN_STAMP(1)
  auto chunk = [&](int c, auto set) {
    constexpr int S = decltype(set)::value;
    const int hid0 = c * HC + wid * 16;
    const bool hvalid = hid0 < F;
    FFN_STAMP(2 + 4 * c)
    __bf16* sHc = sH[NB == 2 ? (c & 1) : 0];
    f32x4 ha[4];
#pragma unroll
    for (int u = 0; u < 4; ++u) ha[u] = f32x4{0.f, 0.f, 0.f, 0.f};
#pragma unroll
    for (int s = 0; s < KS; ++s) {
#pragma unroll
      for (int u = 0; u < 4; ++u) {
        const bf16x8 xb = *reinterpret_cast<const bf16x8*>(&sX[(16 * u + r16) * XLD + 32 * s + 8 * g4]);
        ha[u] = __builtin_amdgcn_mfma_f32_16x16x32_bf16(w1f[s], xb, ha[u], 0, 0, 0);
      }
    }
    FFN_STAMP(3 + 4 * c)
    if constexpr (NB == 1) lds_barrier();
    FFN_STAMP(4 + 4 * c)
    if (hvalid) {
      const float4 bb = *reinterpret_cast<const float4*>(&sB1[hid0 + 4 * g4]);
      const float bv[4] = {bb.x, bb.y, bb.z, bb.w};
#pragma unroll
      for (int u = 0; u < 4; ++u) {
        bf16x4 p;
#pragma unroll
        for (int q = 0; q < 4; ++q) p[q] = (__bf16)swooshl_fast(ha[u][q] + bv[q]);
        *reinterpret_cast<bf16x4*>(&sHc[(16 * u + r16) * HLD + wid * 16 + 4 * g4]) = p;
      }
    } else {
      const bf16x4 z = {(__bf16)0.f, (__bf16)0.f, (__bf16)0.f, (__bf16)0.f};
#pragma unroll
      for (int u = 0; u < 4; ++u) *reinterpret_cast<bf16x4*>(&sHc[(16 * u + r16) * HLD + wid * 16 + 4 * g4]) = z;
    }
    lds_barrier();
    FFN_STAMP(5 + 4 * c)
    load_w1(min(c + 1, nch - 1));
    if constexpr (W2S == 2) load_w2(min(c + 1, nch - 1), std::integral_constant<int, 1 - S>{});
#pragma unroll
    for (int s = 0; s < 4; ++s) {
      bf16x8 hf[4];
#pragma unroll
      for (int u = 0; u < 4; ++u) hf[u] = *reinterpret_cast<const bf16x8*>(&sHc[(16 * u + r16) * HLD + 32 * s + 8 * g4]);
#pragma unroll
      for (int t = 0; t < OT; ++t)
#pragma unroll
        for (int u = 0; u < 4; ++u) o[t][u] = __builtin_amdgcn_mfma_f32_16x16x32_bf16(w2f[S][s][t], hf[u], o[t][u], 0, 0, 0);
    }
    if constexpr (W2S == 1) load_w2(min(c + 1, nch - 1), I0{});
  };
  for (int c = 0; c < nch; c += W2S) {
    chunk(c, I0{});
    if constexpr (W2S == 2) {
      if (c + 1 < nch) chunk(c + 1, I1{});
    }
  }

  if constexpr (EB) {
    float4 bv[OT], kv[OT];
#pragma unroll
    for (int t = 0; t < OT; ++t) {
      const int ch = wid * OW + 16 * t + 4 * g4;
      bv[t] = *reinterpret_cast<const float4*>(b2 + ch);
      if (byp_orig != nullptr) kv[t] = *reinterpret_cast<const float4*>(byp_scale + ch);
    }
#pragma unroll
    for (int u0 = 0; u0 < 4; u0 += 2) {
    float4 xv[2][OT], b0v[2][OT];
#pragma unroll
    for (int du = 0; du < 2; ++du) {
      const long tok = min(t0 + 16 * (u0 + du) + r16, (long)R - 1);
#pragma unroll
      for (int t = 0; t < OT; ++t) {
        const int ch = wid * OW + 16 * t + 4 * g4;
        xv[du][t] = *reinterpret_cast<const float4*>(Xin + tok * D + ch);
        if (byp_orig != nullptr) b0v[du][t] = *reinterpret_cast<const float4*>(byp_orig + tok * D + ch);
      }
    }
#pragma unroll
    for (int du = 0; du < 2; ++du) {
      const int u = u0 + du;
      const long tok = t0 + 16 * u + r16;
      if (tok >= R) continue;
      float* xr = X + tok * D;
#pragma unroll
      for (int t = 0; t < OT; ++t) {
        const int ch = wid * OW + 16 * t + 4 * g4;
        float4 v = xv[du][t];
        v.x += o[t][u][0] + bv[t].x;
        v.y += o[t][u][1] + bv[t].y;
        v.z += o[t][u][2] + bv[t].z;
        v.w += o[t][u][3] + bv[t].w;
        if (byp_orig != nullptr) {
          const float4 b0 = b0v[du][t], k = kv[t];
          v.x = b0.x + (v.x - b0.x) * k.x;
          v.y = b0.y + (v.y - b0.y) * k.y;
          v.z = b0.z + (v.z - b0.z) * k.z;
          v.w = b0.w + (v.w - b0.w) * k.w;
        }
        *reinterpret_cast<float4*>(xr + ch) = v;
      }
    }
    }
    return;
  }
#pragma unroll
  for (int u = 0; u < 4; ++u) {
    const long tok = t0 + 16 * u + r16;
    if (tok >= R) continue;
    float* xr = X + tok * D;
    const float* xi = OOP ? Xin + tok * D : xr;
#pragma unroll
    for (int t = 0; t < OT; ++t) {
      const int ch = wid * OW + 16 * t + 4 * g4;
      const float4 bv = *reinterpret_cast<const float4*>(b2 + ch);
      float4 v = *reinterpret_cast<const float4*>(xi + ch);
      v.x += o[t][u][0] + bv.x;
      v.y += o[t][u][1] + bv.y;
      v.z += o[t][u][2] + bv.z;
      v.w += o[t][u][3] + bv.w;
      if (byp_orig != nullptr) {
        const float4 b0 = *reinterpret_cast<const float4*>(byp_orig + tok * D + ch);
        const float4 k = *reinterpret_cast<const float4*>(byp_scale + ch);
        v.x = b0.x + (v.x - b0.x) * k.x;
        v.y = b0.y + (v.y - b0.y) * k.y;
        v.z = b0.z + (v.z - b0.z) * k.z;
        v.w = b0.w + (v.w - b0.w) * k.w;
      }
      *reinterpret_cast<float4*>(xr + ch) = v;
    }
  }
}

template <int D, bool EB, bool OOP = false>
__global__ __launch_bounds__(512, 2) void ffn_rows_kernel(float* __restrict__ X, int R, int F,
                                                          const __bf16* W1,
                                                          const float* __restrict__ b1,
                                                          const __bf16* W2,
                                                          const float* __restrict__ b2,
                                                          const float* __restrict__ byp_orig,
                                                          const float* __restrict__ byp_scale,
                                                          int rpb, const float* __restrict__ Xsrc) {
  const float* Xin = OOP ? Xsrc : X;
  typedef float f32x4 __attribute__((ext_vector_type(4)));
  constexpr int TUM = 4, HC = 128, NW = 8;
  constexpr int XLD = D + 16, HLD = HC + 16;
  constexpr int KS = D / 32;
  constexpr int OW = D / NW, OT = OW / 16;
  __shared__ __attribute__((aligned(16))) __bf16 sX[16 * TUM * XLD];
  constexpr int NB = D >= 384 ? 2 : 1;
  __shared__ __attribute__((aligned(16))) __bf16 sH[NB][16 * TUM * HLD];
  __shared__ __attribute__((aligned(16))) float sB1[kMaxF];

  const int tid = threadIdx.x, lane = tid & 63;
  const int wid = __builtin_amdgcn_readfirstlane(tid >> 6);
  const int r16 = lane & 15, g4 = lane >> 4;
  const long r0 = (long)blockIdx.x * rpb;
  const long r1 = r0 + rpb < R ? r0 + rpb : R;
  const int nch = (F + HC - 1) / HC;
  const int S2 = F / 32;
  bf16x8 w1f[KS];
  auto load_w1 = [&](int c) {
    const int rg = min((c * HC) / 16 + wid, F / 16 - 1);
    const __bf16* p = W1 + ((long)rg * KS * 64 + lane) * 8;
#pragma unroll
    for (int s = 0; s < KS; ++s) w1f[s] = *reinterpret_cast<const bf16x8*>(p + s * 512);
  };
  constexpr int W2S = ZASR_FFN_W2SETS;
  bf16x8 w2f[W2S][4][OT];
  auto load_w2 = [&](int c, auto set) {
    constexpr int S = decltype(set)::value;
#pragma unroll
    for (int s = 0; s < 4; ++s) {
      const int ks = min(c * (HC / 32) + s, S2 - 1);
#pragma unroll
      for (int t = 0; t < OT; ++t)
        w2f[S][s][t] = *reinterpret_cast<const bf16x8*>(W2 + (((long)(wid * OW / 16 + t) * S2 + ks) * 64 + lane) * 8);
    }
  };
  using I0 = std::integral_constant<int, 0>;
  using I1 = std::integral_constant<int, W2S - 1>;
  for (int e = tid; e < F; e += 64 * NW) sB1[e] = b1[e];

  auto tile = [&](auto tu_c, const long t0) __attribute__((always_inline)) {
    constexpr int TU = decltype(tu_c)::value, TT = 16 * TU;
    int tix = tid;
    asm volatile("" : "+v"(tix));
    {
      static_assert(TT * D / 4 % (64 * NW) == 0, "X tile staging");
      constexpr int NE = TT * D / 4 / (64 * NW);
      float4 v[NE];
#pragma unroll
      for (int i = 0; i < NE; ++i) {
        const int e = tix + 64 * NW * i, row = e / (D / 4), c4 = e - row * (D / 4);
        const long r = t0 + row < R ? t0 + row : R - 1;
        v[i] = *reinterpret_cast<const float4*>(Xin + r * D + 4 * c4);
      }
#pragma unroll
      for (int i = 0; i < NE; ++i) {
        const int e = tix + 64 * NW * i, row = e / (D / 4), c4 = e - row * (D / 4);
        bf16x4 b;
        b[0] = (__bf16)v[i].x; b[1] = (__bf16)v[i].y; b[2] = (__bf16)v[i].z; b[3] = (__bf16)v[i].w;
        *reinterpret_cast<bf16x4*>(&sX[row * XLD + 4 * c4]) = b;
      }
    }
    load_w1(0);
    load_w2(0, I0{});
    lds_barrier();

    f32x4 o[OT][TU];
#pragma unroll
    for (int t = 0; t < OT; ++t)
#pragma unroll
      for (int u = 0; u < TU; ++u) o[t][u] = f32x4{0.f, 0.f, 0.f, 0.f};

    auto chunk = [&](int c, auto set) __attribute__((always_inline)) {
      constexpr int S = decltype(set)::value;
      const int hid0 = c * HC + wid * 16;
      const bool hvalid = hid0 < F;
      __bf16* sHc = sH[NB == 2 ? (c & 1) : 0];
      f32x4 ha[TU];
#pragma unroll
      for (int u = 0; u < TU; ++u) ha[u] = f32x4{0.f, 0.f, 0.f, 0.f};
#pragma unroll
      for (int s = 0; s < KS; ++s) {
#pragma unroll
        for (int u = 0; u < TU; ++u) {
          const bf16x8 xb = *reinterpret_cast<const bf16x8*>(&sX[(16 * u + r16) * XLD + 32 * s + 8 * g4]);
          ha[u] = __builtin_amdgcn_mfma_f32_16x16x32_bf16(w1f[s], xb, ha[u], 0, 0, 0);
        }
      }
      if constexpr (NB == 1) lds_barrier();
      if (hvalid) {
        const float4 bb = *reinterpret_cast<const float4*>(&sB1[hid0 + 4 * g4]);
        const float bv[4] = {bb.x, bb.y, bb.z, bb.w};
#pragma unroll
        for (int u = 0; u < TU; ++u) {
          bf16x4 p;
#pragma unroll
          for (int q = 0; q < 4; ++q) p[q] = (__bf16)swooshl_fast(ha[u][q] + bv[q]);
          *reinterpret_cast<bf16x4*>(&sHc[(16 * u + r16) * HLD + wid * 16 + 4 * g4]) = p;
        }
      } else {
        const bf16x4 z = {(__bf16)0.f, (__bf16)0.f, (__bf16)0.f, (__bf16)0.f};
#pragma unroll
        for (int u = 0; u < TU; ++u) *reinterpret_cast<bf16x4*>(&sHc[(16 * u + r16) * HLD + wid * 16 + 4 * g4]) = z;
      }
      lds_barrier();
      const int cn = min(c + 1, nch - 1);
      load_w1(cn);
      if constexpr (W2S == 2) load_w2(cn, std::integral_constant<int, 1 - S>{});
#pragma unroll
      for (int s = 0; s < 4; ++s) {
        bf16x8 hf[TU];
#pragma unroll
        for (int u = 0; u < TU; ++u) hf[u] = *reinterpret_cast<const bf16x8*>(&sHc[(16 * u + r16) * HLD + 32 * s + 8 * g4]);
#pragma unroll
        for (int t = 0; t < OT; ++t)
#pragma unroll
          for (int u = 0; u < TU; ++u) o[t][u] = __builtin_amdgcn_mfma_f32_16x16x32_bf16(w2f[S][s][t], hf[u], o[t][u], 0, 0, 0);
      }
      if constexpr (W2S == 1) load_w2(cn, I0{});
    };
    for (int c = 0; c < nch; c += W2S) {
      chunk(c, I0{});
      if constexpr (W2S == 2) {
        if (c + 1 < nch) chunk(c + 1, I1{});
      }
    }

    int g4e = g4;
    asm volatile("" : "+v"(g4e));
    float4 bv[OT], kv[OT];
#pragma unroll
    for (int t = 0; t < OT; ++t) {
      const int ch = wid * OW + 16 * t + 4 * g4e;
      bv[t] = *reinterpret_cast<const float4*>(b2 + ch);
      if (byp_orig != nullptr) kv[t] = *reinterpret_cast<const float4*>(byp_scale + ch);
    }
    constexpr int UB = EB ? 2 : 1;
#pragma unroll
    for (int u0 = 0; u0 < TU; u0 += UB) {
      float4 xv[UB][OT], b0v[UB][OT];
// ... 357 lines not shown
      }
    }
  } else {
#pragma unroll
  for (int u = 0; u < TU; ++u) {
    const long tok = t0 + 16 * u + r16;
    if (tok >= r1) continue;
    float* xr = X + tok * D;
    const float* xi = OOP ? Xin + tok * D : xr;
#pragma unroll
    for (int t = 0; t < OT; ++t) {
      const int ch = wid * OW + 16 * t + 4 * g4;
      const float4 bv = *reinterpret_cast<const float4*>(b2 + ch);
      float4 v = *reinterpret_cast<const float4*>(xi + ch);
      v.x += o[t][u][0] * kF16LoInv + bv.x;
      v.y += o[t][u][1] * kF16LoInv + bv.y;
      v.z += o[t][u][2] * kF16LoInv + bv.z;
      v.w += o[t][u][3] * kF16LoInv + bv.w;
      if (byp_orig != nullptr) {
        const float4 b0 = *reinterpret_cast<const float4*>(byp_orig + tok * D + ch);
        const float4 k = *reinterpret_cast<const float4*>(byp_scale + ch);
        v.x = b0.x + (v.x - b0.x) * k.x;
        v.y = b0.y + (v.y - b0.y) * k.y;
        v.z = b0.z + (v.z - b0.z) * k.z;
        v.w = b0.w + (v.w - b0.w) * k.w;
      }
      *reinterpret_cast<float4*>(xr + ch) = v;
    }
  }
  }
  FFN_TSTAMP(90)
#ifdef ZASR_FFN_STAMPS
  ++kt;
#endif
  };

  using T1 = std::integral_constant<int, 1>;
  using T2 = std::integral_constant<int, 2>;
  using T3 = std::integral_constant<int, 3>;
  using TM = std::integral_constant<int, TUM>;
  long t0 = r0;
  for (; t0 + TTM <= r1; t0 += TTM) tile(TM{}, t0);
  const int tail = (int)((r1 - t0 + 15) / 16);
  if (tail == 1) tile(T1{}, t0);
  if constexpr (TUM > 2) if (tail == 2) tile(T2{}, t0);
  if constexpr (TUM > 3) if (tail == 3) tile(T3{}, t0);
  if constexpr (TUM > 4) if (tail == 4) tile(std::integral_constant<int, 4>{}, t0);
  if constexpr (TUM > 5) if (tail == 5) tile(std::integral_constant<int, 5>{}, t0);
  if constexpr (TUM > 6) if (tail == 6) tile(std::integral_constant<int, 6>{}, t0);
  if constexpr (TUM > 7) if (tail == 7) tile(std::integral_constant<int, 7>{}, t0);
  static_assert(TUM <= 8, "tail tiles");
  if (tail == TUM) tile(TM{}, t0);
}

static int g_ffn_split = 1;
void ffn_h3_set_split(int on) { g_ffn_split = on; }

bool ffn_h3_supported(int D, int F) {
  return ((D == 128 || D == 256 || D == 384 || D == 512) && F % 32 == 0 && F >= 32) ||
         (D == 192 && F % 64 == 0 && F >= 64);
}

bool ffn_h3_oop_ok(int D) { return D == 192 || D == 256 || D == 384; }

bool ffn_h3_weights_ok(const float* w, long n) {
  for (long i = 0; i < n; ++i)
    if (!(std::fabs(w[i]) < 31.f)) return false;
  return true;
}

void ffn_pack_h3_host(const float* w, int rows, int cols, __bf16* out) {
  const size_t n = (size_t)rows * cols;
  std::vector<__bf16> piece(n);
  for (int t = 0; t < 2; ++t) {
    for (size_t i = 0; i < n; ++i) {
      const _Float16 hi = (_Float16)w[i];
      const _Float16 v = t == 0 ? hi : (_Float16)((w[i] - (float)hi) * 2048.f);
      std::memcpy(&piece[i], &v, 2);
    }
    ffn_pack_host(piece.data(), rows, cols, out + t * n);
  }
}

void launch_ffn_fused_h3(float* X, int R, int D, int F, const void* W1, const float* b1,
                         const void* W2, const float* b2, hipStream_t st, const float* byp_orig,
                         const float* byp_scale, const float* Y, const float* Xin) {
  if (R <= 0) return;
  if (Xin == X) Xin = nullptr;
  ZASR_REQUIRE(Xin == nullptr || Y == nullptr, "ffn_fused_h3: out of place reads its rows from Xin");
  if (Xin != nullptr) Y = Xin;
  if (Y == nullptr) Y = X;
  ZASR_REQUIRE(ffn_h3_supported(D, F), "ffn_fused_h3: unsupported model / feed-forward dim");
  const __bf16* w1 = reinterpret_cast<const __bf16*>(W1);
  const __bf16* w2 = reinterpret_cast<const __bf16*>(W2);
  static int cus[64] = {0};
  int dev = 0;
  ZASR_HIP_CHECK(hipGetDevice(&dev));
  if (dev < 0 || dev >= 64) dev = 0;
  if (cus[dev] == 0) {
    int n = 0;
    ZASR_HIP_CHECK(hipDeviceGetAttribute(&n, hipDeviceAttributeMultiprocessorCount, dev));
    cus[dev] = n > 0 ? n : 256;
  }
  const int bpc = D == 192 ? 2 : 1;
  const int rpb = 16 * cdiv(cdiv(R, bpc * persist_blocks(cus[dev])), 16);
  const dim3 grid(cdiv(R, rpb));
#define ZASR_FFNH3_(DV, TUV, NBV, NWV, OOPV)                                                          \
  if (NBV == 1 && g_ffn_split && DV != 128)                                                           \
    ZASR_LAUNCH((ffn_wide_h3_kernel<DV, TUV, NBV, NWV, NBV == 1, DV != 128, OOPV>), grid,              \
                dim3(64 * NWV), 0, st, X, R, F, w1, b1, w2, b2, byp_orig, byp_scale, rpb, Y);          \
  else                                                                                                 \
    ZASR_LAUNCH((ffn_wide_h3_kernel<DV, TUV, NBV, NWV, false, DV != 128, OOPV>), grid, dim3(64 * NWV), \
                0, st, X, R, F, w1, b1, w2, b2, byp_orig, byp_scale, rpb, Y)
#define ZASR_FFNH3(DV, TUV, NBV, NWV)        \
  if (Xin != nullptr) {                      \
    ZASR_FFNH3_(DV, TUV, NBV, NWV, true);    \
  } else {                                   \
    ZASR_FFNH3_(DV, TUV, NBV, NWV, false);   \
  }
  switch (D) {
    case 128: ZASR_FFNH3(128, 8, 1, 8); break;
    case 192: ZASR_FFNH3(192, 4, 1, 4); break;
    case 256: ZASR_FFNH3(256, 5, 1, 8); break;
    case 384: ZASR_FFNH3(384, 4, 1, 8); break;
    default: ZASR_FFNH3(512, 3, 2, 8); break;
  }
#undef ZASR_FFNH3
#undef ZASR_FFNH3_
}

void ffn_pack_host(const __bf16* w, int rows, int cols, __bf16* out) {
  for (int g = 0; g < rows / 16; ++g)
    for (int s = 0; s < cols / 32; ++s)
      for (int l = 0; l < 64; ++l)
        for (int j = 0; j < 8; ++j)
          out[(((size_t)g * (cols / 32) + s) * 64 + l) * 8 + j] =
              w[(size_t)(16 * g + (l & 15)) * cols + 32 * s + 8 * (l >> 4) + j];
}

static int g_ffnw_rows = -1;
void ffn_set_rows(int on) { g_ffnw_rows = on ? 1 : 0; }
int ffn_rows_on() {
  if (g_ffnw_rows < 0) {
    const char* e = getenv("ZASR_FFN_ROWS");
    g_ffnw_rows = e != nullptr && atoi(e) == 1 ? 1 : 0;
  }
  return g_ffnw_rows;
}

bool ffn_fused_supported(int D) {
  return D == 64 || D == 96 || D == 128 || D == 192 || D == 256 || D == 384 || D == 512;
}

void launch_ffn_fused(float* X, int R, int D, int F, const void* W1, const float* b1,
                      const void* W2, const float* b2, hipStream_t st, const float* byp_orig,
                      const float* byp_scale, const float* Xin) {
  if (R <= 0) return;
  if (Xin == X) Xin = nullptr;
  ZASR_REQUIRE(ffn_fused_supported(D), "ffn_fused: unsupported model dim");
  ZASR_REQUIRE(F % 8 == 0, "ffn_fused: feed-forward dim must be a multiple of 8");
  const __bf16* w1 = reinterpret_cast<const __bf16*>(W1);
  const __bf16* w2 = reinterpret_cast<const __bf16*>(W2);
  if (D >= 256) {
    ZASR_REQUIRE(F % 32 == 0 && F >= 32 && F <= kMaxF,
                 "ffn_fused: feed-forward dim must be a multiple of 32 in [32, 2048] for D >= 256");
    const dim3 grid(cdiv(R, 64));
    static int cus[64] = {0};
    int dev = 0;
    ZASR_HIP_CHECK(hipGetDevice(&dev));
    if (dev < 0 || dev >= 64) dev = 0;
    if (cus[dev] == 0) {
      int n = 0;
      ZASR_HIP_CHECK(hipDeviceGetAttribute(&n, hipDeviceAttributeMultiprocessorCount, dev));
      cus[dev] = n > 0 ? n : 256;
    }
    if (D == 384 && ffn_rows_on()) {
      const int rpb = 16 * cdiv(cdiv(R, persist_blocks(cus[dev])), 16);
      if (Xin != nullptr)
        ZASR_LAUNCH((ffn_rows_kernel<384, true, true>), dim3(cdiv(R, rpb)), dim3(512), 0, st, X, R, F, w1,
                    b1, w2, b2, byp_orig, byp_scale, rpb, Xin);
      else
        ZASR_LAUNCH((ffn_rows_kernel<384, true, false>), dim3(cdiv(R, rpb)), dim3(512), 0, st, X, R, F, w1,
                    b1, w2, b2, byp_orig, byp_scale, rpb, Xin);
      return;
    }
#define ZASR_FFNW(DV)                                                                                  \
  if (Xin != nullptr)                                                                                  \
    ZASR_LAUNCH((ffn_wide_kernel<DV, DV == 384, true>), grid, dim3(512), 0, st, X, R, F, w1, b1, w2, b2, \
                byp_orig, byp_scale, Xin);                                                             \
  else                                                                                                 \
    ZASR_LAUNCH((ffn_wide_kernel<DV, DV == 384, false>), grid, dim3(512), 0, st, X, R, F, w1, b1, w2,  \
                b2, byp_orig, byp_scale, Xin)
    switch (D) {
      case 256: ZASR_FFNW(256); break;
      case 384: ZASR_FFNW(384); break;
      default: ZASR_FFNW(512); break;
    }
#undef ZASR_FFNW
    return;
  }
  const dim3 grid(cdiv(R, kTok));
#define ZASR_FFN(DV)                                                                                \
  if (Xin != nullptr)                                                                               \
    ZASR_LAUNCH((ffn_fused_kernel<DV, true>), grid, dim3(256), 0, st, X, R, F, w1, b1, w2, b2, byp_orig, \
                byp_scale, Xin);                                                                    \
  else                                                                                              \
    ZASR_LAUNCH((ffn_fused_kernel<DV, false>), grid, dim3(256), 0, st, X, R, F, w1, b1, w2, b2,     \
                byp_orig, byp_scale, Xin)
  switch (D) {
    case 64: ZASR_FFN(64); break;
    case 96: ZASR_FFN(96); break;
    case 128: ZASR_FFN(128); break;
    default: ZASR_FFN(192); break;
  }
#undef ZASR_FFN
}

}
```

sherpa-vietnamese-asr_amd/csrc/kernels.h:

```cpp
#pragma once
#include <cstdint>
#include <vector>

#include <hip/hip_runtime.h>

namespace zasr {

struct FbankTables {
  const double* twiddle;
  const float* window;
  const int* mel_start;
  const int* mel_len;
  const int* mel_woff;
  const float* mel_w;
};
void launch_fbank(const float* wav, const long* wav_off, const int* nsamp, const int* fr_off,
                  int nseq, int total_frames, const FbankTables& tabs, float* out,
                  hipStream_t st, bool campp = false);

void launch_silence_flags(const float* wav, long n, int frame_len, float threshold,
                          unsigned char* flags, hipStream_t st);

void launch_selftest_noop(int block_threads);
void selftest_gemm_h3r(int M, int K, int N, int epi, const float* A, const float* W,
                       const float* bias, float* C);
void selftest_ffn_h3(int R, int D, int F, const float* Y, const float* W1, const float* b1,
                     const float* W2, const float* b2, const float* byp_orig,
                     const float* byp_scale, float* X, float* Xout = nullptr);
void selftest_ffn_bf16(int R, int D, int F, const float* W1, const float* b1, const float* W2,
                       const float* b2, const float* byp_orig, const float* byp_scale, float* X,
                       int form, float* Xout = nullptr);

struct CamppConv2d {
  const float* x;
  const float* w;
  const float* scale;
  const float* shift;
  const float* res;
  float* y;
  int n, ci, fi, fo, T, sf;
  int relu, tdnn_out;
  int in_tf;
  const float* wk = nullptr;
};
void campp_conv2d_permute_weights(const float* w, int ks, float* out);
void launch_campp_conv2d(const CamppConv2d& a, int ks, hipStream_t st);
void launch_campp_bnrelu(const float* x, int ldx, long R, int C, const float* s, const float* b,
                         float* y, hipStream_t st);
void launch_campp_im2col1d(const float* x, int ldx, int N, int Tin, int Tout, int C, int K,
                           int stride, int dil, int pad, float* out, hipStream_t st);
struct CamppCamMask {
  const float* h;
  const float* w1;
  const float* b1;
  const float* w2;
  const float* b2;
  float* mexp;
  int n, T, seg_len;
};
void launch_campp_cam_mask(const CamppCamMask& a, hipStream_t st);
void launch_campp_stats(const float* x, int N, int T, int C, const float* s, const float* b,
                        float* out, hipStream_t st);
void launch_campp_cmvn(float* x, const int* fr_off, int nseq, hipStream_t st);
void launch_campp_gather(const float* rows, const int* win_row, const int* win_n, int nwin,
                         int wf, float* out, hipStream_t st);

struct VibertEmbedArgs {
  const long* ids;
  const long* tt;
  const float* word;
  const float* pos;
  const float* type;
  const float* ln_g;
  const float* ln_b;
  float* x;
  int L, H;
  float eps;
};
void launch_vibert_embed(const VibertEmbedArgs& a, long rows, hipStream_t st);
void launch_vibert_layernorm(float* x, long rows, int H, const float* g, const float* b, float eps,
                             hipStream_t st);
struct VibertAttnArgs {
  const float* qkv;
  const long* mask;
  float* ctx;
  int L, H;
  float scale;
};
void launch_vibert_attention(const VibertAttnArgs& a, int B, int heads, hipStream_t st);
void launch_vibert_gather(const float* x, const long* offsets, int B, int L, int W, int H, float* g,
                          hipStream_t st);

struct VadFramesArgs {
  const float* audio;
  const long* off;
  const long* win_start;
  const unsigned* maxabs;
  const float* rows576;
  float* frames;
  int n_files;
};
void launch_vad_maxabs(const float* audio, const long* off, const long* len, int n_files,
                       unsigned* mx, hipStream_t st);
void launch_vad_frames(const VadFramesArgs& a, long n_windows, hipStream_t st);
void launch_vad_mag_im2col(const float* S, int ldS, int bins, int Kp, long n_windows, float* A,
                           hipStream_t st);
void launch_vad_im2col(const float* Y, long N, int T, int C, int stride, int Tout, float* A,
                       hipStream_t st);
struct VadLstmArgs {
  const float* gx;
  const float* whh;
  const float* bhh;
  const float* wd;
  float bd;
  const long* seg_start;
  const int* seg_count;
  const int* seg_warm;
  const float* init;
  float* s_out;
  float* e_out;
  float* probs;
};
void launch_vad_lstm(const VadLstmArgs& a, int n_segments, hipStream_t st);

void launch_conv1(const float* fb, const int* fb_off, const int* c1_off, const int* c1_map,
                  int total_rows, const float* w , const float* b, void* out,
                  bool out_bf16, hipStream_t st, bool fast = false);
void pack_frag32_host(const __bf16* w, int rows, int cols, __bf16* out);
void launch_convnext_bf16(const void* x, const int* L_off, const int* L_map, int total_rows,
                          const float* dw_w, const float* dw_b, const void* w1, const float* b1,
                          const void* w2, const float* b2, void* ytmp, void* out,
                          hipStream_t st);
void launch_convnext_mlp_h3(const float* y, const float* x, long npos, const void* w1p,
                            const float* b1, const void* w2p, const float* b2, float* out,
                            hipStream_t st);
void launch_dwconv2d_tiled(const float* x, const int* L_off, const int* L_map, int total_rows,
                           const float* w, const float* b, float* out, hipStream_t st);

void selftest_seam(int nseq, const int* L, int d, int ds, int dn, int ds_next, int c0, int ldo,
                   const float* xd, const float* orig, const float* s, const float* wn8,
                   const float* wo2, float* next, float* xnext, float* out, float* next_ref,
                   float* xnext_ref, float* out_ref);
void launch_bias_norm(float* x, int rows, int d, const float* bias, float log_scale,
                      const float* orig, const float* bypass_scale, hipStream_t st,
                      float* copy_out = nullptr);
void launch_bypass(float* x, const float* orig, const float* s, long rows, int d, hipStream_t st);
void launch_glu(const float* x2, float* g, long rows, int d, hipStream_t st);
void launch_dwconv1d_post_glu(const float* g, const int* off, const int* map, int total_rows,
                              int d, int K, const float* w, const float* b, float* out,
                              hipStream_t st);
void launch_dwconv1d_post_glu_bf16(const void* g, const int* off, const int* map,
                                   int total_rows, int d, int K, const float* w, const float* b,
                                   void* out, hipStream_t st);
void launch_glu_dwconv1d(const float* x2, const int* off, const int* map, int total_rows, int d,
                         int K, const float* w, const float* b, float* out, hipStream_t st);
void launch_glu_dwconv1d_bf16(const void* x2, const int* off, const int* map, int total_rows,
                              int d, int K, const float* w, const float* b, void* out,
                              hipStream_t st);
void launch_nonlin_prep(const float* h3, float* t1, long rows, int hid, hipStream_t st);
void launch_downsample(const float* x, const int* off_in, const int* off_out, const int* map_out,
                       int total_out, int d, int ds, const float* w_host8, float* out,
                       hipStream_t st);
void launch_upsample_combine(const float* xd, const float* orig, const int* off_in,
                             const int* off_ds, const int* map_in, int total_rows, int d, int ds,
                             const float* s, float* y, hipStream_t st);
void launch_stack_glue(const float* xd, const float* orig, const int* off_in, const int* off_ds,
                       const int* map_in, int rows, int d, int ds, const float* s, float* next,
                       int dn, float* full, int ldf, int c0, hipStream_t st);
struct SeamDesc {
  const float* xd = nullptr;
  const float* orig = nullptr;
  const float* s = nullptr;
  const int* off_in = nullptr;
  const int* off_ds = nullptr;
  const int* off_run = nullptr;
  const int* map_run = nullptr;
  int runs = 0;
  int rows = 0;
  int d = 0, ds = 1;
  float* next = nullptr;
  int dn = 0;
  int ds_next = 1;
  float* xnext = nullptr;
  const float* wn_host8 = nullptr;
  float* out = nullptr;
  const int* off_out = nullptr;
  const float* wo_host2 = nullptr;
  int ldo = 0, c0 = 0;
};
void launch_seam(const SeamDesc& s, hipStream_t st);
void launch_row2seq(const int* off, int nseq, int total, int* map, hipStream_t st);
void launch_copy_cols(const float* src, int lds, int c0, float* dst, int ldd, int d0, int ncols,
                      long rows, bool zero_rest, int dst_width, hipStream_t st);

struct AttnArgs {
  const float* qkp;
  int H;
  const float* pos_tab;
  int pmax;
  const int* row_off;
  const long* a_off;
  int nseq;
  int max_len;
  float* attn;
  float* stats;
  int write_heads;
};
void launch_attn_softmax(const AttnArgs& a, hipStream_t st);
struct AttnFlashArgs {
  const void* qkp;
  int H;
  const float* pos_tab;
  int pmax;
  const int* row_off;
  const long* a_off;
  int nseq;
  int max_len;
  void* attn;
  const void* v;
  void* out;
  const float* stats_in;
  float* stats_out;
  int pieces = 1;
  const void* t1t = nullptr;
  const int* o8 = nullptr;
  int ldt = 0;
  int hid = 0;
  const void* y = nullptr;
  int ldy = 0;
  void* z = nullptr;
  const unsigned* map = nullptr;
  int map_len = 0;
};
void launch_attn_flash(const AttnFlashArgs& a, int mode, hipStream_t st);
inline int attn_nonlin_frags(int hid, int pieces) {
  const int nft = (hid + 31) / 32;
  if (pieces != 1) return 3;
  return (nft % 5 == 0 || nft == 9) ? 5 : 6;
}
inline int attn_nonlin_chunks(int hid, int pieces) {
  const int nf = attn_nonlin_frags(hid, pieces);
  return ((hid + 31) / 32 + nf - 1) / nf;
}
constexpr int kAttnXcds = 8;
constexpr unsigned kAttnMapNone = 0xffffffffu;
constexpr int kAttnMapMaxSeq = 1 << 20, kAttnMapMaxUnits = 16, kAttnMapMaxTiles = 256;
inline unsigned attn_map_pack(int seq, int unit, int tile) {
  return (unsigned)seq << 12 | (unsigned)unit << 8 | (unsigned)tile;
}
struct AttnBlockMaps {
  const unsigned* heads;
  int n_heads;
  const unsigned* head0;
  int n_head0;
};
int build_attn_block_map(const int* lens, int nseq, int units_per_seq, int order,
                         std::vector<unsigned>& map);
void launch_nonlin_prep_t(const void* h3, bool h3_bf16, const int* off, const int* o8,
                          const int* map, int R, int hid, int R8, void* t1t, hipStream_t st,
                          int pieces = 1);
struct AttnSAArgs {
  const float* qkp;
  int H;
  const float* pos_tab;
  int pmax;
  const int* row_off;
  int nseq;
  int max_len;
  const float* stats;
  const float* v;
  float* out;
  float* stats_out;
};
void launch_attn_sa(const AttnSAArgs& a, bool online, bool bf16, hipStream_t st);

bool ffn_fused_supported(int D);
void ffn_pack_host(const __bf16* w, int rows, int cols, __bf16* out);
void launch_ffn_fused(float* X, int R, int D, int F, const void* W1, const float* b1,
                      const void* W2, const float* b2, hipStream_t st,
                      const float* byp_orig = nullptr, const float* byp_scale = nullptr,
                      const float* Xin = nullptr);
bool ffn_h3_supported(int D, int F);
void ffn_h3_set_split(int on);
void ffn_set_rows(int on);
int ffn_rows_on();
bool ffn_h3_weights_ok(const float* w, long n);
bool ffn_h3_oop_ok(int D);
void ffn_pack_h3_host(const float* w, int rows, int cols, __bf16* out);
void launch_ffn_fused_h3(float* X, int R, int D, int F, const void* W1, const float* b1,
                         const void* W2, const float* b2, hipStream_t st,
                         const float* byp_orig = nullptr, const float* byp_scale = nullptr,
                         const float* Y = nullptr, const float* Xin = nullptr);

struct SearchState {
  double* lp;
  int* lpf;
  unsigned long long* hash;
  int* len;
  int* y1;
  int* y2;
  int* hw;
  int* node;
  int* nh;
  int* node_tok;
  int* node_frame;
  int* node_parent;
  double* node_lp;
  float4* node_stats;
  int* node_count;
  int node_cap;
};
struct HotwordTables {
  int num_states;
  int num_cls;
  const int* tok2cls;
  const int* next;
  const double* delta;
  const double* node_score;
};
struct DecoderW {
  const float* tap0;
  const float* tap1;
  const float* bp;
  int D;
};
struct DecJoinArgs {
  DecoderW dw;
  const float* wp;
  const int* y1;
  const int* y2;
  const float* enc;
  const int* enc_off;
  void* J;
  int M, H, t;
  int j_bf16;
};
struct JoinerArgs {
  const float* J;
  const float* W;
  const float* bias;
  float* out;
  int M, V, D;
  const int* live_t = nullptr;
  const int* live_len = nullptr;
  int live_f = 0;
  const __bf16* Wx = nullptr;
  int pieces = 0;
};
struct JoinerBf16Args {
  const __bf16* J;
  const __bf16* W;
  const float* bias;
  float* out;
  int M, V, D;
  const int* live_t = nullptr;
  const int* live_len = nullptr;
  int live_f = 0;
};
struct DecTable {
  const float* table;
  int V;
  const float* enc;
  const int* enc_off;
  const int* enc_len;
  void* J;
  int D;
  int j_bf16;
  int j_packed = 0;
  int j_pieces = 0;
  long j_plane = 0;
};
struct JoinerPackedArgs {
  const void* Jp;
  const void* Wp;
  const float* bias;
  float* out;
  int M, V, D;
  const int* live_t = nullptr;
  const int* live_len = nullptr;
  int live_f = 0;
  int pieces = 0;
  long j_plane = 0, w_plane = 0;
};
void launch_joiner_packed(const JoinerPackedArgs& j, hipStream_t st);
void launch_nonfinite_check(const float* x, long n, int* flag, hipStream_t st);
inline long joiner_packed_rows(long M) { return (M + 63) / 64 * 64; }
void launch_search_init(const SearchState& s, int S, int Hmax, hipStream_t st);
void launch_decjoin(const DecJoinArgs& a, hipStream_t st);
void launch_joiner(const JoinerArgs& j, hipStream_t st);
void launch_joiner_bf16(const JoinerBf16Args& j, hipStream_t st);
void launch_dec_table(const DecoderW& dw, const float* wp, int V, float* table, hipStream_t st);
void launch_table_init(const DecTable& dt, int S, int Hmax, hipStream_t st);
void launch_search_step(const SearchState& s, const float* logits, int V, int S, int Hmax,
                        int beam, int t, const int* enc_len, const HotwordTables& hw,
                        const DecTable* dt, hipStream_t st);
void launch_greedy_spec_init(const DecTable& dt, int S, int F, int* t_cur, int* active,
                             hipStream_t st);
void launch_greedy_spec(const SearchState& s, const float* logits, int V, int S, int F,
                        int* t_cur, const int* enc_len, const HotwordTables& hw,
                        const DecTable& dt, int* active, int parity, hipStream_t st);
struct GreedyFusedArgs {
  JoinerPackedArgs j;
  int ldo;
  SearchState st;
  int* t_cur;
  const int* enc_len;
  HotwordTables hw;
  DecTable dt;
  int* active;
  int parity;
  int* cnt;
  int S;
};
void launch_joiner_greedy(const GreedyFusedArgs& a, hipStream_t st);
inline int joiner_greedy_ldo(int V) { return (V + 31) / 32 * 32; }
void launch_search_final(const SearchState& s, int S, int Hmax, const HotwordTables& hw,
                         int out_cap, int* out_tok, int* out_frame, double* out_lp,
                         float4* out_stats, int* out_count, hipStream_t st);

}
```

sherpa-vietnamese-asr_amd/csrc/selftest.cpp:

```cpp
#include <cstring>
#include <memory>
#include <vector>

#include "common.h"
#include "gemm.h"
#include "kernels.h"

namespace zasr {
namespace {
struct DevBuf {
  void* p = nullptr;
  explicit DevBuf(size_t bytes) { ZASR_HIP_CHECK(hipMalloc(&p, bytes > 0 ? bytes : 4)); }
  ~DevBuf() { (void)hipFree(p); }
  template <class T>
  T* as() const { return reinterpret_cast<T*>(p); }
};
void up(DevBuf& d, const void* h, size_t bytes) {
  if (bytes) ZASR_HIP_CHECK(hipMemcpy(d.p, h, bytes, hipMemcpyHostToDevice));
}
}

void selftest_gemm_h3r(int M, int K, int N, int epi, const float* A, const float* W,
                       const float* bias, float* C) {
  ZASR_REQUIRE(M >= 1, "selftest gemm_h3r: M >= 1");
  ZASR_REQUIRE(gemm_h3r_supported(K, N, epi), "selftest gemm_h3r: unsupported K / N / epilogue");
  ZASR_REQUIRE(ffn_h3_weights_ok(W, (long)N * K), "selftest gemm_h3r: |w| must stay below 31");
  const int ncol = epi == EPI_GLU ? N / 2 : N;
  std::vector<__bf16> pk(2 * (size_t)N * K);
  ffn_pack_h3_host(W, N, K, pk.data());
  DevBuf dA((size_t)M * K * 4), dW(pk.size() * 2), dB((size_t)N * 4), dC((size_t)M * ncol * 4);
  up(dA, A, (size_t)M * K * 4);
  up(dW, pk.data(), pk.size() * 2);
  if (bias) up(dB, bias, (size_t)N * 4);
  up(dC, C, (size_t)M * ncol * 4);
  gemm_h3r(dA.as<float>(), dW.p, bias ? dB.as<float>() : nullptr, dC.as<float>(), ncol, M, N, K,
           epi, nullptr);
  ZASR_HIP_CHECK(hipDeviceSynchronize());
  ZASR_HIP_CHECK(hipMemcpy(C, dC.p, (size_t)M * ncol * 4, hipMemcpyDeviceToHost));
}

void selftest_ffn_h3(int R, int D, int F, const float* Y, const float* W1, const float* b1,
                     const float* W2, const float* b2, const float* byp_orig,
                     const float* byp_scale, float* X, float* Xout) {
  ZASR_REQUIRE(R >= 1, "selftest ffn_h3: R >= 1");
  ZASR_REQUIRE(Xout == nullptr || Y == nullptr, "selftest ffn_h3: out of place reads X");
  ZASR_REQUIRE(ffn_h3_supported(D, F), "selftest ffn_h3: unsupported model / feed-forward dim");
  ZASR_REQUIRE(ffn_h3_weights_ok(W1, (long)F * D) && ffn_h3_weights_ok(W2, (long)F * D),
               "selftest ffn_h3: |w| must stay below 31");
  std::vector<__bf16> p1(2 * (size_t)F * D), p2(p1.size());
  ffn_pack_h3_host(W1, F, D, p1.data());
  ffn_pack_h3_host(W2, D, F, p2.data());
  const size_t xb = (size_t)R * D * 4;
  DevBuf dY(xb), dX(xb), d1(p1.size() * 2), d2(p2.size() * 2), db1((size_t)F * 4),
      db2((size_t)D * 4), dbo(byp_orig ? xb : 4), dbs((size_t)D * 4), dO(Xout ? xb : 4);
  if (Y) up(dY, Y, xb);
  up(dX, X, xb);
  if (Xout) up(dO, Xout, xb);
  up(d1, p1.data(), p1.size() * 2);
  up(d2, p2.data(), p2.size() * 2);
  up(db1, b1, (size_t)F * 4);
  up(db2, b2, (size_t)D * 4);
  if (byp_orig) {
    ZASR_REQUIRE(byp_scale != nullptr, "selftest ffn_h3: bypass needs its scale");
    up(dbo, byp_orig, xb);
    up(dbs, byp_scale, (size_t)D * 4);
  }
  launch_ffn_fused_h3(Xout ? dO.as<float>() : dX.as<float>(), R, D, F, d1.p, db1.as<float>(), d2.p,
                      db2.as<float>(), nullptr, byp_orig ? dbo.as<float>() : nullptr,
                      byp_orig ? dbs.as<float>() : nullptr, Y ? dY.as<float>() : nullptr,
                      Xout ? dX.as<float>() : nullptr);
  ZASR_HIP_CHECK(hipDeviceSynchronize());
  ZASR_HIP_CHECK(hipMemcpy(X, dX.p, xb, hipMemcpyDeviceToHost));
  if (Xout) ZASR_HIP_CHECK(hipMemcpy(Xout, dO.p, xb, hipMemcpyDeviceToHost));
}

void selftest_ffn_bf16(int R, int D, int F, const float* W1, const float* b1, const float* W2,
                       const float* b2, const float* byp_orig, const float* byp_scale, float* X,
                       int form, float* Xout) {
  ZASR_REQUIRE(form == 0 || form == 1, "selftest ffn_bf16: form 0 (default route) or 1 (rows form)");
  ZASR_REQUIRE(R >= 1, "selftest ffn_bf16: R >= 1");
  ZASR_REQUIRE(ffn_fused_supported(D), "selftest ffn_bf16: unsupported model dim");
  std::vector<__bf16> h1((size_t)F * D), h2((size_t)D * F);
  for (size_t i = 0; i < h1.size(); ++i) h1[i] = (__bf16)W1[i];
  for (size_t i = 0; i < h2.size(); ++i) h2[i] = (__bf16)W2[i];
  if (D >= 256) {
    std::vector<__bf16> p1(h1.size()), p2(h2.size());
    ffn_pack_host(h1.data(), F, D, p1.data());
    ffn_pack_host(h2.data(), D, F, p2.data());
    h1.swap(p1);
    h2.swap(p2);
  }
  const size_t xb = (size_t)R * D * 4;
  DevBuf dX(xb), d1(h1.size() * 2), d2(h2.size() * 2), db1((size_t)F * 4), db2((size_t)D * 4),
      dbo(byp_orig ? xb : 4), dbs((size_t)D * 4), dO(Xout ? xb : 4);
  up(dX, X, xb);
  if (Xout) up(dO, Xout, xb);
  up(d1, h1.data(), h1.size() * 2);
  up(d2, h2.data(), h2.size() * 2);
  up(db1, b1, (size_t)F * 4);
  up(db2, b2, (size_t)D * 4);
  if (byp_orig) {
    ZASR_REQUIRE(byp_scale != nullptr, "selftest ffn_bf16: bypass needs its scale");
    up(dbo, byp_orig, xb);
    up(dbs, byp_scale, (size_t)D * 4);
  }
  const int saved = ffn_rows_on();
  ffn_set_rows(form);
  try {
    launch_ffn_fused(Xout ? dO.as<float>() : dX.as<float>(), R, D, F, d1.p, db1.as<float>(), d2.p,
                     db2.as<float>(), nullptr, byp_orig ? dbo.as<float>() : nullptr,
                     byp_orig ? dbs.as<float>() : nullptr, Xout ? dX.as<float>() : nullptr);
  } catch (...) {
    ffn_set_rows(saved);
    throw;
  }
  ffn_set_rows(saved);
  ZASR_HIP_CHECK(hipDeviceSynchronize());
  ZASR_HIP_CHECK(hipMemcpy(X, dX.p, xb, hipMemcpyDeviceToHost));
  if (Xout) ZASR_HIP_CHECK(hipMemcpy(Xout, dO.p, xb, hipMemcpyDeviceToHost));
}

void selftest_seam(int nseq, const int* L, int d, int ds, int dn, int ds_next, int c0, int ldo,
                   const float* xd, const float* orig, const float* s, const float* wn8,
                   const float* wo2, float* next, float* xnext, float* out, float* next_ref,
                   float* xnext_ref, float* out_ref) {
  ZASR_REQUIRE(nseq >= 1 && d >= 4 && dn >= 0 && ds >= 1 && ds_next >= 1 && c0 >= 0,
               "selftest seam: sizes");
  ZASR_REQUIRE(ldo % 4 == 0 && ldo >= d, "selftest seam: output row stride >= d, a multiple of 4");
  const bool has_x = ds_next > 1 && dn > 0, has_out = c0 < d;
  auto level = [&](int f, std::vector<int>& off) {
    off.assign(nseq + 1, 0);
    for (int b = 0; b < nseq; ++b) {
      ZASR_REQUIRE(L[b] >= 1, "selftest seam: every sequence needs a frame");
      off[b + 1] = off[b] + (L[b] + f - 1) / f;
    }
    return off[nseq];
  };
  std::vector<int> oL, oS, oN, oO;
  const int rows = level(1, oL), rs = level(ds, oS), rn = level(ds_next, oN), ro = level(2, oO);
  const size_t ib = (size_t)(nseq + 1) * 4;
  DevBuf dL(ib), dS(ib), dN(ib), dO(ib), mL((size_t)rows * 4), mN((size_t)rn * 4),
      mO((size_t)ro * 4);
  up(dL, oL.data(), ib);
  up(dS, oS.data(), ib);
  up(dN, oN.data(), ib);
  up(dO, oO.data(), ib);
  launch_row2seq(dL.as<int>(), nseq, rows, mL.as<int>(), nullptr);
  launch_row2seq(dN.as<int>(), nseq, rn, mN.as<int>(), nullptr);
  launch_row2seq(dO.as<int>(), nseq, ro, mO.as<int>(), nullptr);
  const size_t bo = (size_t)rows * d * 4, bx = (size_t)rs * d * 4, bn = (size_t)rows * dn * 4,
               bxn = (size_t)rn * dn * 4, bout = (size_t)ro * ldo * 4, bfull = (size_t)rows * ldo * 4;
  DevBuf dorig(bo), dxd(bx), ds_(d * 4), dnext(bn), dxn(bxn), dout(bout), dnext_r(bn), dxn_r(bxn),
      dout_r(bout), dfull(bfull);
  up(dorig, orig, bo);
  if (ds > 1) {
    up(dxd, xd, bx);
    up(ds_, s, (size_t)d * 4);
  }
  up(dnext, next, bn);
  up(dnext_r, next, bn);
  if (has_x) {
    up(dxn, xnext, bxn);
    up(dxn_r, xnext, bxn);
  }
  up(dout, out, bout);
  up(dout_r, out, bout);
  ZASR_HIP_CHECK(hipMemset(dfull.p, 0, bfull > 0 ? bfull : 4));
  SeamDesc sd;
  sd.xd = dxd.as<float>();
  sd.orig = dorig.as<float>();
  sd.s = ds_.as<float>();
  sd.off_in = dL.as<int>();
  sd.off_ds = dS.as<int>();
  sd.off_run = ds_next > 1 ? dN.as<int>() : dO.as<int>();
  sd.map_run = ds_next > 1 ? mN.as<int>() : mO.as<int>();
  sd.runs = ds_next > 1 ? rn : ro;
  sd.rows = rows;
  sd.d = d;
  sd.ds = ds;
  sd.next = dn > 0 ? dnext.as<float>() : nullptr;
  sd.dn = dn;
  sd.ds_next = ds_next;
  if (has_x) {
    sd.xnext = dxn.as<float>();
    sd.wn_host8 = wn8;
  }
  if (has_out) {
    sd.out = dout.as<float>();
    sd.off_out = dO.as<int>();
    sd.wo_host2 = wo2;
    sd.ldo = ldo;
    sd.c0 = c0;
  }
  launch_seam(sd, nullptr);
  launch_stack_glue(dxd.as<float>(), dorig.as<float>(), dL.as<int>(), dS.as<int>(), mL.as<int>(),
                    rows, d, ds, ds_.as<float>(), dn > 0 ? dnext_r.as<float>() : nullptr, dn,
                    has_out ? dfull.as<float>() : nullptr, ldo, c0, nullptr);
  if (has_x)
    launch_downsample(dnext_r.as<float>(), dL.as<int>(), dN.as<int>(), mN.as<int>(), rn, dn,
                      ds_next, wn8, dxn_r.as<float>(), nullptr);
  if (has_out)
    launch_downsample(dfull.as<float>(), dL.as<int>(), dO.as<int>(), mO.as<int>(), ro, ldo, 2, wo2,
                      dout_r.as<float>(), nullptr);
  ZASR_HIP_CHECK(hipDeviceSynchronize());
  auto down = [](void* h, const DevBuf& dv, size_t bytes) {
    if (bytes) ZASR_HIP_CHECK(hipMemcpy(h, dv.p, bytes, hipMemcpyDeviceToHost));
  };
  down(next, dnext, bn);
  down(next_ref, dnext_r, bn);
  if (has_x) {
    down(xnext, dxn, bxn);
    down(xnext_ref, dxn_r, bxn);
  }
  down(out, dout, bout);
  down(out_ref, dout_r, bout);
}

}
```

sherpa-vietnamese-asr_amd/csrc/zasr_api.cpp:

```cpp
#include <cstdio>
#include <cstring>
#include <fstream>
#include <memory>
#include <mutex>
#include <sstream>
#include <string>
#include <vector>

#include "../../include/zasr.h"
#include "campp.h"
#include "common.h"
#include "vad.h"
#include "vibert.h"
#include "engine.h"
#include "host_io.h"
#include "onnx_io.h"

using zasr::Engine;
using zasr::TokenResult;

struct zasr_recognizer {
  std::unique_ptr<Engine> eng;
  std::string model_dir;
  std::string tokens_path;
// ... 515 lines not shown
    for (int i = 0; i < count; ++i) {
      if (n_frames[i] < 9) return fail(ZASR_ERR_INVALID, "chunk shorter than 9 fbank frames");
      need += ((n_frames[i] - 7) / 2 + 1) / 2;
    }
    if (need * e->joiner_dim() > cap) return fail(ZASR_ERR_INVALID, "output buffer too small");
    std::vector<float> enc;
    std::vector<int> to;
    e->encode_host(f, fr, enc, to);
    std::memcpy(out, enc.data(), enc.size() * sizeof(float));
    for (int i = 0; i < count; ++i) t_out[i] = to[i];
    return (int)ZASR_OK;
  });
}

int zasr_search_encoder_out(zasr_recognizer* h, const float* const* enc, const int64_t* t_out,
                            int32_t count, int32_t beam, zasr_result** out) {
  if (!h || !enc || !t_out || !out || count < 0) return fail(ZASR_ERR_INVALID, "null argument");
  *out = nullptr;
  return guarded([&]() {
    Engine* e = h->eng.get();
    std::lock_guard<std::mutex> lk(e->mu);
    std::vector<const float*> p(enc, enc + count);
    std::vector<long> t(t_out, t_out + count);
    auto r = std::make_unique<zasr_result>();
    r->items = e->search_host(p, t, resolve_beam(h, beam));
    *out = r.release();
    return (int)ZASR_OK;
  });
}

int32_t zasr_result_count(const zasr_result* r) { return r ? (int32_t)r->items.size() : 0; }
static const TokenResult* item(const zasr_result* r, int32_t i) {
  return (r && i >= 0 && i < (int32_t)r->items.size()) ? &r->items[i] : nullptr;
}
int32_t zasr_result_num_tokens(const zasr_result* r, int32_t i) {
  auto* t = item(r, i);
  return t ? (int32_t)t->tok.size() : 0;
}
int32_t zasr_result_num_frames(const zasr_result* r, int32_t i) {
  auto* t = item(r, i);
  return t ? t->t_out : 0;
}
const int32_t* zasr_result_tokens(const zasr_result* r, int32_t i) {
  auto* t = item(r, i);
  return t ? t->tok.data() : nullptr;
}
const int32_t* zasr_result_frames(const zasr_result* r, int32_t i) {
  auto* t = item(r, i);
  return t ? t->frame.data() : nullptr;
}
const double* zasr_result_log_probs(const zasr_result* r, int32_t i) {
  auto* t = item(r, i);
  return t ? t->lp.data() : nullptr;
}
const float* zasr_result_token_stats(const zasr_result* r, int32_t i) {
  auto* t = item(r, i);
  return t ? t->stats.data() : nullptr;
}
void zasr_result_free(zasr_result* r) { delete r; }

int32_t zasr_vocab_size(const zasr_recognizer* h) { return h ? h->eng->vocab() : 0; }
int32_t zasr_joiner_dim(const zasr_recognizer* h) { return h ? h->eng->joiner_dim() : 0; }

int zasr_profile_enable(zasr_recognizer* h, int32_t on) {
  if (!h) return fail(ZASR_ERR_INVALID, "null handle");
  if (on < 0 || on > 2) return fail(ZASR_ERR_INVALID, "profile mode must be 0, 1 or 2");
  h->eng->profile_enable((int)on);
  return ZASR_OK;
}
int zasr_profile_reset(zasr_recognizer* h) {
  if (!h) return fail(ZASR_ERR_INVALID, "null handle");
  return guarded([&]() {
    h->eng->profile_reset();
    return (int)ZASR_OK;
  });
}
int zasr_profile_report(zasr_recognizer* h, char* buf, int64_t cap) {
  if (!h || !buf || cap <= 0) return fail(ZASR_ERR_INVALID, "null argument");
  return guarded([&]() {
    std::string s = h->eng->profile_report();
    if ((int64_t)s.size() + 1 > cap) return fail(ZASR_ERR_INVALID, "report buffer too small");
    std::memcpy(buf, s.c_str(), s.size() + 1);
    return (int)ZASR_OK;
  });
}

int zasr_model_routes(zasr_recognizer* h, char* buf, int64_t cap) {
  if (!h || !buf || cap <= 0) return fail(ZASR_ERR_INVALID, "null argument");
  return guarded([&]() {
    const std::string s = h->eng->routes_json();
    if ((int64_t)s.size() + 1 > cap) return fail(ZASR_ERR_INVALID, "routes buffer too small");
    std::memcpy(buf, s.c_str(), s.size() + 1);
    return (int)ZASR_OK;
  });
}

int zasr_fbank_set_mel_banks(zasr_recognizer* h, const float* banks, int32_t n_bins) {
  if (!h || !banks) return fail(ZASR_ERR_INVALID, "null argument");
  if (n_bins != 256 && n_bins != 257) return fail(ZASR_ERR_INVALID, "n_bins must be 256 or 257");
  return guarded([&]() {
    std::lock_guard<std::mutex> lk(h->eng->mu);
    h->eng->set_mel_banks(banks, n_bins);
    return (int)ZASR_OK;
  });
}

int zasr_selftest_launch(int32_t block_threads) {
  if (block_threads <= 0) return fail(ZASR_ERR_INVALID, "block_threads must be positive");
  return guarded([&]() {
    zasr::launch_selftest_noop(block_threads);
    return (int)ZASR_OK;
  });
}

int zasr_selftest_gemm_h3r(int32_t M, int32_t K, int32_t N, int32_t epi, const float* A,
                           const float* W, const float* bias, float* C) {
  if (!A || !W || !C) return fail(ZASR_ERR_INVALID, "null argument");
  return guarded([&]() {
    zasr::selftest_gemm_h3r(M, K, N, epi, A, W, bias, C);
    return (int)ZASR_OK;
  });
}

int zasr_selftest_ffn_h3(int32_t R, int32_t D, int32_t F, const float* Y, const float* W1,
                         const float* b1, const float* W2, const float* b2,
                         const float* byp_orig, const float* byp_scale, float* X) {
  if (!Y || !W1 || !b1 || !W2 || !b2 || !X) return fail(ZASR_ERR_INVALID, "null argument");
  return guarded([&]() {
    zasr::selftest_ffn_h3(R, D, F, Y, W1, b1, W2, b2, byp_orig, byp_scale, X);
    return (int)ZASR_OK;
  });
}

int zasr_selftest_ffn_bf16(int32_t R, int32_t D, int32_t F, const float* W1, const float* b1,
                           const float* W2, const float* b2, const float* byp_orig,
                           const float* byp_scale, float* X, int32_t form) {
  if (!W1 || !b1 || !W2 || !b2 || !X) return fail(ZASR_ERR_INVALID, "null argument");
  return guarded([&]() {
    zasr::selftest_ffn_bf16(R, D, F, W1, b1, W2, b2, byp_orig, byp_scale, X, form);
    return (int)ZASR_OK;
  });
}

int zasr_selftest_ffn_bf16_oop(int32_t R, int32_t D, int32_t F, const float* W1, const float* b1,
                               const float* W2, const float* b2, const float* byp_orig,
                               const float* byp_scale, float* X, float* Xout, int32_t form) {
  if (!W1 || !b1 || !W2 || !b2 || !X || !Xout) return fail(ZASR_ERR_INVALID, "null argument");
  return guarded([&]() {
    zasr::selftest_ffn_bf16(R, D, F, W1, b1, W2, b2, byp_orig, byp_scale, X, form, Xout);
    return (int)ZASR_OK;
  });
}

int zasr_selftest_ffn_h3_oop(int32_t R, int32_t D, int32_t F, const float* W1, const float* b1,
                             const float* W2, const float* b2, const float* byp_orig,
                             const float* byp_scale, float* X, float* Xout) {
  if (!W1 || !b1 || !W2 || !b2 || !X || !Xout) return fail(ZASR_ERR_INVALID, "null argument");
  return guarded([&]() {
    zasr::selftest_ffn_h3(R, D, F, nullptr, W1, b1, W2, b2, byp_orig, byp_scale, X, Xout);
    return (int)ZASR_OK;
  });
}

int zasr_selftest_seam(int32_t nseq, const int32_t* L, int32_t d, int32_t ds, int32_t dn,
                       int32_t ds_next, int32_t c0, int32_t ldo, const float* xd,
                       const float* orig, const float* s, const float* wn8, const float* wo2,
                       float* next, float* xnext, float* out, float* next_ref, float* xnext_ref,
                       float* out_ref) {
  if (!L || !orig || !wn8 || !wo2 || !next || !xnext || !out || !next_ref || !xnext_ref ||
      !out_ref || (ds > 1 && (!xd || !s)))
    return fail(ZASR_ERR_INVALID, "null argument");
  return guarded([&]() {
    zasr::selftest_seam(nseq, L, d, ds, dn, ds_next, c0, ldo, xd, orig, s, wn8, wo2, next, xnext,
                        out, next_ref, xnext_ref, out_ref);
    return (int)ZASR_OK;
  });
}

int zasr_selftest_attn_block_map(const int32_t* lens, int32_t nseq, int32_t units_per_seq,
                                 int32_t order, uint32_t* out, int64_t cap, int32_t* grid) {
  if (!lens || !grid || (cap > 0 && !out) || cap < 0) return fail(ZASR_ERR_INVALID, "null argument");
  return guarded([&]() {
    std::vector<unsigned> map;
    *grid = zasr::build_attn_block_map(lens, nseq, units_per_seq, order, map);
    if ((int64_t)map.size() > cap) return fail(ZASR_ERR_INVALID, "block map buffer too small");
    std::copy(map.begin(), map.end(), out);
    return (int)ZASR_OK;
  });
}

int zasr_silence_flags(const float* d_wav, int64_t n, int32_t frame_len, float threshold,
                       uint8_t* d_flags, void* stream) {
  if (n < 0 || (n > 0 && (!d_wav || !d_flags))) return fail(ZASR_ERR_INVALID, "null argument");
  return guarded([&]() {
    zasr::launch_silence_flags(d_wav, (long)n, (int)frame_len, threshold, d_flags,
                               reinterpret_cast<hipStream_t>(stream));
    return (int)ZASR_OK;
  });
}

int zasr_set_tokens(zasr_recognizer* h, const char* tokens_path) {
  if (!h || !tokens_path) return fail(ZASR_ERR_INVALID, "null argument");
  return guarded([&]() {
    std::ifstream f(tokens_path);
    if (!f) return fail(ZASR_ERR_NOT_FOUND, std::string("tokens file not found: ") + tokens_path);
    std::lock_guard<std::mutex> lk(h->sym_mu);
    h->tokens_path = tokens_path;
    h->syms.reset();
    return (int)ZASR_OK;
  });
}

int zasr_create_stream(zasr_recognizer* h, zasr_stream** out) {
  if (!h || !out) return fail(ZASR_ERR_INVALID, "null argument");
  return guarded([&]() {
    auto* s = new zasr_stream;
    s->rec = h;
    *out = s;
    return (int)ZASR_OK;
  });
}

void zasr_destroy_stream(zasr_stream* s) { delete s; }

int zasr_stream_accept_waveform(zasr_stream* s, int32_t sample_rate, const float* samples,
                                int64_t n) {
  if (!s || n < 0 || (n > 0 && !samples)) return fail(ZASR_ERR_INVALID, "null argument");
  if (sample_rate != 16000) return fail(ZASR_ERR_INVALID, "sample rate must be 16000");
  if (s->decoded) return fail(ZASR_ERR_INVALID, "stream already decoded");
  return guarded([&]() {
    s->samples.insert(s->samples.end(), samples, samples + n);
    return (int)ZASR_OK;
  });
}

int zasr_decode_stream(zasr_recognizer* h, zasr_stream* s) {
  return zasr_decode_streams(h, &s, 1);
}

int zasr_decode_streams(zasr_recognizer* h, zasr_stream* const* ss, int32_t n) {
  if (!h || n < 0 || (n > 0 && !ss)) return fail(ZASR_ERR_INVALID, "null argument");
  for (int32_t i = 0; i < n; ++i) {
    if (!ss[i]) return fail(ZASR_ERR_INVALID, "null stream");
    if (ss[i]->rec != h) return fail(ZASR_ERR_INVALID, "stream belongs to another recognizer");
    for (int32_t j = 0; j < i; ++j)
      if (ss[j] == ss[i]) return fail(ZASR_ERR_INVALID, "stream listed twice");
  }
  return guarded([&]() {
    decode_streams_impl(h, ss, n);
    return (int)ZASR_OK;
  });
}

int32_t zasr_stream_is_decoded(const zasr_stream* s) { return s && s->decoded ? 1 : 0; }
int32_t zasr_stream_num_tokens(const zasr_stream* s) {
  return s ? (int32_t)s->res.tok.size() : 0;
}
int32_t zasr_stream_num_frames(const zasr_stream* s) { return s ? s->res.t_out : 0; }
const int32_t* zasr_stream_tokens(const zasr_stream* s) { return s ? s->res.tok.data() : nullptr; }
const int32_t* zasr_stream_frames(const zasr_stream* s) { return s ? s->res.frame.data() : nullptr; }
const double* zasr_stream_log_probs(const zasr_stream* s) { return s ? s->res.lp.data() : nullptr; }
const float* zasr_stream_token_stats(const zasr_stream* s) {
  return s ? s->res.stats.data() : nullptr;
}

int zasr_stream_result_json(const zasr_stream* s, char* buf, int64_t cap, int64_t* needed) {
  if (!s || !needed) return fail(ZASR_ERR_INVALID, "null argument");
  if (!s->decoded) return fail(ZASR_ERR_INVALID, "stream not decoded");
  return guarded([&]() {
    const std::shared_ptr<const std::vector<std::string>> tab = symbols(s->rec);
    const std::vector<std::string>& sym = *tab;
    const TokenResult& r = s->res;
    std::ostringstream os;
    std::string text;
    std::vector<std::string> toks;
    for (int t : r.tok) {
      toks.push_back(t >= 0 && t < (int)sym.size() ? sym[t] : std::string());
      text += toks.back();
    }
    os << "{\"lang\": \"\", \"emotion\": \"\", \"event\": \"\", \"text\": ";
    json_string(os, text);
    os << ", \"timestamps\": [";
    char b[40];
    for (size_t i = 0; i < r.frame.size(); ++i) {
      std::snprintf(b, sizeof b, "%s%.2f", i ? ", " : "", (float)(0.04f * (float)r.frame[i]));
      os << b;
    }
    os << "], \"tokens\": [";
    for (size_t i = 0; i < toks.size(); ++i) {
      if (i) os << ", ";
      json_string(os, toks[i]);
    }
    os << "], \"ys_log_probs\": [";
    for (size_t i = 0; i < r.lp.size(); ++i) {
      std::snprintf(b, sizeof b, "%s%.17g", i ? ", " : "", r.lp[i]);
      os << b;
    }
    os << "], \"words\": []}";
    const std::string js = os.str();
    *needed = (int64_t)js.size() + 1;
    if (!buf || cap < *needed) return fail(ZASR_ERR_INVALID, "result buffer too small");
    std::memcpy(buf, js.c_str(), js.size() + 1);
    return (int)ZASR_OK;
  });
}

// ... 5 lines not shown
```

sherpa-vietnamese-asr_amd/zasr/binding.py:

```python
from __future__ import annotations

import ctypes as C
import dataclasses
import os
from typing import List, Optional, Sequence

import numpy as np

_PKG = os.path.dirname(os.path.dirname(os.path.abspath(__file__)))
DEFAULT_LIB = os.path.join(_PKG, "lib", "libzasr.so")

EXPORTS = (
    "zasr_create", "zasr_destroy", "zasr_convert_model", "zasr_convert_stage_model", "zasr_fbank", "zasr_decode_batch", "zasr_decode_features",
    "zasr_decode_device", "zasr_decode_device_batches", "zasr_encode_features", "zasr_search_encoder_out",
    "zasr_result_count", "zasr_result_num_tokens", "zasr_result_num_frames",
    "zasr_result_tokens", "zasr_result_frames", "zasr_result_log_probs",
    "zasr_result_token_stats", "zasr_result_free", "zasr_vocab_size", "zasr_joiner_dim",
    "zasr_profile_enable", "zasr_profile_reset", "zasr_profile_report", "zasr_last_error",
    "zasr_version", "zasr_campp_create", "zasr_campp_destroy", "zasr_campp_embedding_dim",
    "zasr_campp_fbank", "zasr_campp_embed", "zasr_campp_embed_device", "zasr_campp_windows_device",
    "zasr_vibert_create", "zasr_vibert_destroy", "zasr_vibert_num_labels",
    "zasr_vibert_num_detect", "zasr_vibert_run",
    "zasr_vad_create", "zasr_vad_destroy", "zasr_vad_probs", "zasr_vad_probs_device",
    "zasr_vad_window", "zasr_vad_last_passes", "zasr_silence_flags",
    "zasr_create_stream", "zasr_destroy_stream", "zasr_stream_accept_waveform",
    "zasr_decode_stream", "zasr_decode_streams", "zasr_stream_is_decoded",
    "zasr_stream_num_tokens", "zasr_stream_num_frames", "zasr_stream_tokens",
    "zasr_stream_frames", "zasr_stream_log_probs", "zasr_stream_token_stats",
    "zasr_stream_result_json", "zasr_set_tokens", "zasr_model_routes",
    "zasr_fbank_set_mel_banks", "zasr_selftest_launch", "zasr_decode_host_batches",
    "zasr_selftest_gemm_h3r", "zasr_selftest_ffn_h3", "zasr_selftest_ffn_bf16",
    "zasr_selftest_attn_block_map", "zasr_selftest_seam", "zasr_selftest_ffn_bf16_oop",
    "zasr_selftest_ffn_h3_oop",
)


PRECISIONS = {"fp32": 0, "bf16": 1, "bf16_enc": 2, "bf16x3": 3, "bf16x6": 4, "f16x3": 5}


C_FP = C.POINTER(C.c_float)


class ZasrError(RuntimeError):
    pass


class _Config(C.Structure):
    _fields_ = [
        ("model_dir", C.c_char_p),
        ("decoding_method", C.c_char_p),
        ("max_active_paths", C.c_int32),
        ("blank_penalty", C.c_float),
        ("hotword_tokens", C.POINTER(C.c_int32)),
        ("hotword_lens", C.POINTER(C.c_int32)),
        ("hotword_scores", C.POINTER(C.c_float)),
        ("num_hotwords", C.c_int32),
        ("device_id", C.c_int32),
        ("precision", C.c_int32),
    ]


_lib = None


def load_library(path: Optional[str] = None) -> C.CDLL:
    global _lib
    if _lib is not None and path is None:
        return _lib
    p = path or os.environ.get("ZASR_LIB", DEFAULT_LIB)
    if not os.path.exists(p):
        raise ZasrError(f"libzasr.so not found at {p}; build it with "
                        f"`make -C sherpa-vietnamese-asr_amd/csrc` (or __graft_entry__.build())")
    lib = C.CDLL(p)
    P, I32, I64 = C.c_void_p, C.c_int32, C.c_int64
    fp = C.POINTER(C.c_float)
    lib.zasr_create.argtypes = [C.POINTER(_Config), C.POINTER(P)]
    lib.zasr_create.restype = C.c_int
    lib.zasr_destroy.argtypes = [P]
    lib.zasr_destroy.restype = None
    lib.zasr_convert_model.argtypes = [C.c_char_p, C.c_char_p]
    lib.zasr_convert_model.restype = C.c_int
    lib.zasr_convert_stage_model.argtypes = [C.c_char_p, C.c_char_p, C.c_char_p]
    lib.zasr_convert_stage_model.restype = C.c_int
    lib.zasr_fbank.argtypes = [P, fp, I64, I32, fp, I64, C.POINTER(I64)]
    lib.zasr_fbank.restype = C.c_int
    lib.zasr_decode_batch.argtypes = [P, C.POINTER(fp), C.POINTER(I64), I32, I32, C.POINTER(P)]
    lib.zasr_decode_batch.restype = C.c_int
    lib.zasr_decode_features.argtypes = [P, C.POINTER(fp), C.POINTER(I64), I32, I32, C.POINTER(P)]
    lib.zasr_decode_features.restype = C.c_int
    lib.zasr_decode_device.argtypes = [P, P, C.POINTER(I64), C.POINTER(I64), I32, I32, P,
                                       C.POINTER(P)]
    lib.zasr_decode_device.restype = C.c_int
    lib.zasr_decode_device_batches.argtypes = [P, P, C.POINTER(I64), C.POINTER(I64), I32,
                                               C.POINTER(I32), I32, I32, P, C.POINTER(P)]
    lib.zasr_decode_device_batches.restype = C.c_int
    lib.zasr_decode_host_batches.argtypes = [P, P, C.POINTER(I64), C.POINTER(I64), I32,
                                             C.POINTER(I32), I32, I32, P, C.POINTER(P)]
    lib.zasr_decode_host_batches.restype = C.c_int
    lib.zasr_encode_features.argtypes = [P, C.POINTER(fp), C.POINTER(I64), I32, fp, I64,
                                         C.POINTER(I64)]
    lib.zasr_encode_features.restype = C.c_int
    lib.zasr_search_encoder_out.argtypes = [P, C.POINTER(fp), C.POINTER(I64), I32, I32,
                                            C.POINTER(P)]
    lib.zasr_search_encoder_out.restype = C.c_int
    for n in ("zasr_result_count",):
        getattr(lib, n).argtypes = [P]
        getattr(lib, n).restype = I32
    for n in ("zasr_result_num_tokens", "zasr_result_num_frames"):
        getattr(lib, n).argtypes = [P, I32]
        getattr(lib, n).restype = I32
    lib.zasr_result_tokens.argtypes = [P, I32]
    lib.zasr_result_tokens.restype = C.POINTER(I32)
    lib.zasr_result_frames.argtypes = [P, I32]
    lib.zasr_result_frames.restype = C.POINTER(I32)
    lib.zasr_result_log_probs.argtypes = [P, I32]
    lib.zasr_result_log_probs.restype = C.POINTER(C.c_double)
    lib.zasr_result_token_stats.argtypes = [P, I32]
    lib.zasr_result_token_stats.restype = fp
    lib.zasr_result_free.argtypes = [P]
    lib.zasr_result_free.restype = None
    lib.zasr_vocab_size.argtypes = [P]
    lib.zasr_vocab_size.restype = I32
    lib.zasr_joiner_dim.argtypes = [P]
    lib.zasr_joiner_dim.restype = I32
    lib.zasr_profile_enable.argtypes = [P, I32]
    lib.zasr_profile_enable.restype = C.c_int
    lib.zasr_profile_reset.argtypes = [P]
    lib.zasr_profile_reset.restype = C.c_int
    lib.zasr_profile_report.argtypes = [P, C.c_char_p, I64]
    lib.zasr_profile_report.restype = C.c_int
    lib.zasr_last_error.argtypes = []
    lib.zasr_last_error.restype = C.c_char_p
    lib.zasr_version.argtypes = []
    lib.zasr_version.restype = C.c_char_p
    lib.zasr_campp_create.argtypes = [C.c_char_p, I32, C.POINTER(P)]
    lib.zasr_campp_create.restype = C.c_int
    lib.zasr_campp_destroy.argtypes = [P]
    lib.zasr_campp_destroy.restype = None
    lib.zasr_campp_embedding_dim.argtypes = [P]
    lib.zasr_campp_embedding_dim.restype = I32
    lib.zasr_campp_fbank.argtypes = [P, fp, I64, fp, I64, C.POINTER(I64)]
    lib.zasr_campp_fbank.restype = C.c_int
    lib.zasr_campp_embed.argtypes = [P, fp, I32, I32, fp]
    lib.zasr_campp_embed.restype = C.c_int
    lib.zasr_campp_embed_device.argtypes = [P, P, I32, I32, P, P]
    lib.zasr_campp_embed_device.restype = C.c_int
    i32p = C.POINTER(I32)
    lib.zasr_campp_windows_device.argtypes = [P, P, C.POINTER(I64), C.POINTER(I64), I32, I32, I32,
                                              P, I64, i32p, i32p, i32p, C.POINTER(I64), P]
    lib.zasr_campp_windows_device.restype = C.c_int
    lib.zasr_vibert_create.argtypes = [C.c_char_p, I32, C.POINTER(P)]
    lib.zasr_vibert_create.restype = C.c_int
    lib.zasr_vibert_destroy.argtypes = [P]
    lib.zasr_vibert_destroy.restype = None
    for n in ("zasr_vibert_num_labels", "zasr_vibert_num_detect"):
        getattr(lib, n).argtypes = [P]
        getattr(lib, n).restype = I32
    i64p = C.POINTER(I64)
    lib.zasr_vibert_run.argtypes = [P, i64p, i64p, i64p, i64p, I32, I32, I32, fp, fp]
    lib.zasr_vibert_run.restype = C.c_int
    lib.zasr_vad_create.argtypes = [C.c_char_p, I32, C.POINTER(P)]
    lib.zasr_vad_create.restype = C.c_int
    lib.zasr_vad_destroy.argtypes = [P]
    lib.zasr_vad_destroy.restype = None
    lib.zasr_vad_probs.argtypes = [P, fp, i64p, i64p, I32, I32, fp]
    lib.zasr_vad_probs.restype = C.c_int
    lib.zasr_vad_probs_device.argtypes = [P, P, i64p, i64p, I32, I32, P, P]
    lib.zasr_vad_probs_device.restype = C.c_int
    lib.zasr_vad_window.argtypes = [P, fp, fp, I32, fp, fp]
    lib.zasr_vad_window.restype = C.c_int
    lib.zasr_vad_last_passes.argtypes = [P]
    lib.zasr_vad_last_passes.restype = I32
    lib.zasr_silence_flags.argtypes = [P, I64, I32, C.c_float, P, P]
    lib.zasr_silence_flags.restype = C.c_int
    lib.zasr_create_stream.argtypes = [P, C.POINTER(P)]
    lib.zasr_create_stream.restype = C.c_int
    lib.zasr_destroy_stream.argtypes = [P]
    lib.zasr_destroy_stream.restype = None
    lib.zasr_stream_accept_waveform.argtypes = [P, I32, fp, I64]
    lib.zasr_stream_accept_waveform.restype = C.c_int
    lib.zasr_decode_stream.argtypes = [P, P]
    lib.zasr_decode_stream.restype = C.c_int
    lib.zasr_decode_streams.argtypes = [P, C.POINTER(P), I32]
    lib.zasr_decode_streams.restype = C.c_int
    for n in ("zasr_stream_is_decoded", "zasr_stream_num_tokens", "zasr_stream_num_frames"):
        getattr(lib, n).argtypes = [P]
        getattr(lib, n).restype = I32
    lib.zasr_stream_tokens.argtypes = [P]
    lib.zasr_stream_tokens.restype = C.POINTER(I32)
    lib.zasr_stream_frames.argtypes = [P]
    lib.zasr_stream_frames.restype = C.POINTER(I32)
    lib.zasr_stream_log_probs.argtypes = [P]
    lib.zasr_stream_log_probs.restype = C.POINTER(C.c_double)
    lib.zasr_stream_token_stats.argtypes = [P]
    lib.zasr_stream_token_stats.restype = fp
    lib.zasr_stream_result_json.argtypes = [P, C.c_char_p, I64, C.POINTER(I64)]
    lib.zasr_stream_result_json.restype = C.c_int
    lib.zasr_set_tokens.argtypes = [P, C.c_char_p]
    lib.zasr_set_tokens.restype = C.c_int
    lib.zasr_model_routes.argtypes = [P, C.c_char_p, I64]
    lib.zasr_model_routes.restype = C.c_int
    lib.zasr_fbank_set_mel_banks.argtypes = [P, fp, I32]
    lib.zasr_fbank_set_mel_banks.restype = C.c_int
    lib.zasr_selftest_launch.argtypes = [I32]
    lib.zasr_selftest_launch.restype = C.c_int
    lib.zasr_selftest_gemm_h3r.argtypes = [I32, I32, I32, I32, fp, fp, fp, fp]
    lib.zasr_selftest_gemm_h3r.restype = C.c_int
    lib.zasr_selftest_ffn_h3.argtypes = [I32, I32, I32, fp, fp, fp, fp, fp, fp, fp, fp]
    lib.zasr_selftest_ffn_h3.restype = C.c_int
    lib.zasr_selftest_ffn_bf16.argtypes = [I32, I32, I32, fp, fp, fp, fp, fp, fp, fp, I32]
    lib.zasr_selftest_ffn_bf16.restype = C.c_int
    lib.zasr_selftest_attn_block_map.argtypes = [C.POINTER(I32), I32, I32, I32,
                                                 C.POINTER(C.c_uint32), I64, C.POINTER(I32)]
    lib.zasr_selftest_attn_block_map.restype = C.c_int
    lib.zasr_selftest_seam.argtypes = [I32, C.POINTER(I32)] + [I32] * 6 + [fp] * 11
    lib.zasr_selftest_seam.restype = C.c_int
    lib.zasr_selftest_ffn_bf16_oop.argtypes = [I32, I32, I32] + [fp] * 8 + [I32]
    lib.zasr_selftest_ffn_bf16_oop.restype = C.c_int
    lib.zasr_selftest_ffn_h3_oop.argtypes = [I32, I32, I32] + [fp] * 8
    lib.zasr_selftest_ffn_h3_oop.restype = C.c_int
    if path is None:
        _lib = lib
    return lib


def convert_model(model_dir: str, out_dir: str, lib_path: Optional[str] = None) -> None:
    lib = load_library(lib_path)
    os.makedirs(out_dir, exist_ok=True)
    rc = lib.zasr_convert_model(model_dir.encode(), out_dir.encode())
    if rc != 0:
        msg = lib.zasr_last_error().decode()
        if rc == 2:
            raise FileNotFoundError(msg)
        raise ZasrError(msg)


def convert_stage_model(kind: str, model_dir: str, out_dir: str,
                        lib_path: Optional[str] = None) -> None:
    lib = load_library(lib_path)
    os.makedirs(out_dir, exist_ok=True)
    rc = lib.zasr_convert_stage_model(kind.encode(), model_dir.encode(), out_dir.encode())
    if rc != 0:
        msg = lib.zasr_last_error().decode()
        if rc == 2:
            raise FileNotFoundError(msg)
        raise ZasrError(msg)


def selftest_launch(block_threads: int, lib_path: Optional[str] = None) -> None:
    lib = load_library(lib_path)
    rc = lib.zasr_selftest_launch(int(block_threads))
    if rc != 0:
        raise ZasrError(lib.zasr_last_error().decode())


def selftest_gemm_h3r(A, W, bias, C, epi: int = 0, lib_path: Optional[str] = None) -> np.ndarray:
    lib = load_library(lib_path)
    A, W, C = _f32(A), _f32(W), _f32(C).copy()
    b = None if bias is None else _f32(bias)
    p = lambda x: None if x is None else x.ctypes.data_as(C_FP)
    rc = lib.zasr_selftest_gemm_h3r(A.shape[0], A.shape[1], W.shape[0], int(epi), p(A), p(W),
                                    p(b), p(C))
    if rc != 0:
        raise ZasrError(lib.zasr_last_error().decode())
    return C


def selftest_ffn_h3(Y, W1, b1, W2, b2, X, byp_orig=None, byp_scale=None,
                    lib_path: Optional[str] = None) -> np.ndarray:
    lib = load_library(lib_path)
    Y, W1, b1, W2, b2, X = (_f32(v) for v in (Y, W1, b1, W2, b2, X))
    X = X.copy()
    bo = None if byp_orig is None else _f32(byp_orig)
    bs = None if byp_scale is None else _f32(byp_scale)
    p = lambda x: None if x is None else x.ctypes.data_as(C_FP)
    rc = lib.zasr_selftest_ffn_h3(Y.shape[0], Y.shape[1], W1.shape[0], p(Y), p(W1), p(b1), p(W2),
                                  p(b2), p(bo), p(bs), p(X))
    if rc != 0:
        raise ZasrError(lib.zasr_last_error().decode())
    return X


def selftest_ffn_bf16(W1, b1, W2, b2, X, byp_orig=None, byp_scale=None, form: int = 0,
                      lib_path: Optional[str] = None) -> np.ndarray:
    lib = load_library(lib_path)
    W1, b1, W2, b2, X = (_f32(v) for v in (W1, b1, W2, b2, X))
    X = X.copy()
    bo = None if byp_orig is None else _f32(byp_orig)
    bs = None if byp_scale is None else _f32(byp_scale)
    p = lambda x: None if x is None else x.ctypes.data_as(C_FP)
    rc = lib.zasr_selftest_ffn_bf16(X.shape[0], X.shape[1], W1.shape[0], p(W1), p(b1), p(W2),
                                    p(b2), p(bo), p(bs), p(X), int(form))
    if rc != 0:
        raise ZasrError(lib.zasr_last_error().decode())
    return X


def selftest_attn_block_map(lens, units_per_seq: int, order: int = 0,
                            lib_path: Optional[str] = None) -> np.ndarray:
    lib = load_library(lib_path)
    lens = np.ascontiguousarray(lens, dtype=np.int32)
    cap = 8 * int(units_per_seq) * int(((lens.astype(np.int64) + 127) // 128).sum())
    out = np.empty(max(cap, 1), dtype=np.uint32)
    grid = C.c_int32(-1)
    rc = lib.zasr_selftest_attn_block_map(lens.ctypes.data_as(C.POINTER(C.c_int32)), len(lens),
                                          int(units_per_seq), int(order),
                                          out.ctypes.data_as(C.POINTER(C.c_uint32)), cap,
                                          C.byref(grid))
    if rc != 0:
        raise ZasrError(lib.zasr_last_error().decode())
    return out[:grid.value].copy()


def selftest_ffn_oop(kind: str, W1, b1, W2, b2, X, byp_orig=None, byp_scale=None, form: int = 0,
                     fill: float = -777.25, lib_path: Optional[str] = None):
    lib = load_library(lib_path)
    W1, b1, W2, b2, X = (_f32(v) for v in (W1, b1, W2, b2, X))
    X = X.copy()
    out = np.full(X.shape, fill, dtype=np.float32)
    bo = None if byp_orig is None else _f32(byp_orig)
    bs = None if byp_scale is None else _f32(byp_scale)
    p = lambda x: None if x is None else x.ctypes.data_as(C_FP)
    args = (X.shape[0], X.shape[1], W1.shape[0], p(W1), p(b1), p(W2), p(b2), p(bo), p(bs), p(X),
            p(out))
    if kind == "bf16":
        rc = lib.zasr_selftest_ffn_bf16_oop(*args, int(form))
    elif kind == "h3":
        rc = lib.zasr_selftest_ffn_h3_oop(*args)
    else:
        raise ValueError(kind)
    if rc != 0:
        raise ZasrError(lib.zasr_last_error().decode())
    return out, X


def selftest_seam(L, d: int, ds: int, dn: int, ds_next: int, c0: int, ldo: int, xd, orig, s,
                  wn8, wo2, fill: float = -777.25, lib_path: Optional[str] = None) -> dict:
    lib = load_library(lib_path)
    L = np.ascontiguousarray(L, dtype=np.int32)
    orig, wn8, wo2 = _f32(orig), _f32(wn8), _f32(wo2)
    xd = None if xd is None else _f32(xd)
    s = None if s is None else _f32(s)
    rows = int(L.sum())
    rn = int(((L + ds_next - 1) // ds_next).sum())
    ro = int(((L + 1) // 2).sum())
    assert orig.shape == (rows, d) and wn8.shape == (8,) and wo2.shape == (2,)
    assert ds == 1 or (xd.shape == (int(((L + ds - 1) // ds).sum()), d) and s.shape == (d,))
    res = {}
    for name, shape in (("next", (rows, dn)), ("xnext", (rn, dn)), ("out", (ro, ldo))):
        for k in (name, name + "_ref"):
            res[k] = np.full(shape, fill, dtype=np.float32)
    p = lambda x: None if x is None else x.ctypes.data_as(C_FP)
    rc = lib.zasr_selftest_seam(len(L), L.ctypes.data_as(C.POINTER(C.c_int32)), int(d), int(ds),
                                int(dn), int(ds_next), int(c0), int(ldo), p(xd), p(orig), p(s),
                                p(wn8), p(wo2), p(res["next"]), p(res["xnext"]), p(res["out"]),
                                p(res["next_ref"]), p(res["xnext_ref"]), p(res["out_ref"]))
    if rc != 0:
        raise ZasrError(lib.zasr_last_error().decode())
    return res


def silence_flags(d_wav_ptr: int, n: int, frame_len: int, threshold: float, d_flags_ptr: int,
                  stream: int = 0, lib_path: Optional[str] = None) -> None:
    lib = load_library(lib_path)
    rc = lib.zasr_silence_flags(C.c_void_p(d_wav_ptr), int(n), int(frame_len),
                                float(threshold), C.c_void_p(d_flags_ptr), C.c_void_p(stream))
    if rc != 0:
        raise ZasrError(lib.zasr_last_error().decode())


@dataclasses.dataclass
class SearchResult:
    token_ids: np.ndarray
    frames: np.ndarray
    log_probs: np.ndarray
    stats: np.ndarray
    T: int


def _f32(a) -> np.ndarray:
    return np.ascontiguousarray(np.asarray(a, dtype=np.float32))


def _ptr_array(arrs: Sequence[np.ndarray]):
    fp = C.POINTER(C.c_float)
    return (fp * len(arrs))(*[a.ctypes.data_as(fp) for a in arrs])


class Recognizer:
    def __init__(self, model_dir: str, decoding_method: str = "modified_beam_search",
                 max_active_paths: int = 8, hotwords: Optional[Sequence[Sequence[int]]] = None,
                 hotword_scores: Optional[Sequence[float]] = None, device_id: int = 0,
                 precision: str = "fp32", lib_path: Optional[str] = None):
        self.lib = load_library(lib_path)
        hotwords = [list(map(int, h)) for h in (hotwords or [])]
        scores = list(hotword_scores or [1.5] * len(hotwords))
        flat = np.array([t for h in hotwords for t in h] or [0], dtype=np.int32)
        lens = np.array([len(h) for h in hotwords] or [0], dtype=np.int32)
        sc = np.array(scores or [0.0], dtype=np.float32)
        self._keep = (flat, lens, sc)
        cfg = _Config(model_dir.encode(), decoding_method.encode(), max_active_paths, 0.0,
                      flat.ctypes.data_as(C.POINTER(C.c_int32)),
                      lens.ctypes.data_as(C.POINTER(C.c_int32)),
                      sc.ctypes.data_as(C.POINTER(C.c_float)), len(hotwords), device_id,
                      PRECISIONS[precision])
        h = C.c_void_p()
        rc = self.lib.zasr_create(C.byref(cfg), C.byref(h))
        if rc != 0:
            msg = self.lib.zasr_last_error().decode()
            if rc == 2:
                raise FileNotFoundError(msg)
            raise ZasrError(msg)
        self.handle = h
        self.device_id = int(device_id)
        self.precision = precision
        self.vocab_size = self.lib.zasr_vocab_size(h)
        self.joiner_dim = self.lib.zasr_joiner_dim(h)
        self._args = (model_dir, decoding_method, max_active_paths, hotwords, scores, device_id,
                      lib_path)
        self._fallback = None

    def close(self):
        if getattr(self, "handle", None):
            self.lib.zasr_destroy(self.handle)
            self.handle = None
        fb = getattr(self, "_fallback", None)
        if fb is not None:
            fb.close()
            self._fallback = None

    FALLBACK_PRECISION = "bf16x6"

    def _retry(self, e: "ZasrError", name: str, *args, **kw):
        if self.precision != "f16x3" or "non-finite encoder output" not in str(e):
            raise e
        if self._fallback is None:
            import logging
            logging.getLogger("zasr").warning(
                "[zasr] f16x3 operand range exceeded; re-decoding with %s", self.FALLBACK_PRECISION)
            md, method, beam, hw, sc, dev, lp = self._args
            self._fallback = Recognizer(md, method, beam, hotwords=hw, hotword_scores=sc,
                                        device_id=dev, precision=self.FALLBACK_PRECISION,
                                        lib_path=lp)
        return getattr(self._fallback, name)(*args, **kw)

    def __del__(self):
        try:
            self.close()
        except Exception:
            pass

    def _check(self, rc):
        if rc != 0:
            raise ZasrError(self.lib.zasr_last_error().decode())

    def _collect(self, res) -> List[SearchResult]:
        out = []
        try:
            n = self.lib.zasr_result_count(res)
            for i in range(n):
                k = self.lib.zasr_result_num_tokens(res, i)
                T = self.lib.zasr_result_num_frames(res, i)
                if k > 0:
                    tok = np.ctypeslib.as_array(self.lib.zasr_result_tokens(res, i), (k,)).copy()
                    fr = np.ctypeslib.as_array(self.lib.zasr_result_frames(res, i), (k,)).copy()
                    lp = np.ctypeslib.as_array(self.lib.zasr_result_log_probs(res, i), (k,)).copy()
                    st = np.ctypeslib.as_array(self.lib.zasr_result_token_stats(res, i),
                                               (k * 4,)).copy().reshape(k, 4)
                else:
                    tok = np.zeros(0, np.int32)
                    fr = np.zeros(0, np.int32)
                    lp = np.zeros(0, np.float64)
                    st = np.zeros((0, 4), np.float32)
                out.append(SearchResult(tok, fr, lp, st, T))
        finally:
            self.lib.zasr_result_free(res)
        return out

    def routes(self) -> dict:
        import json
        buf = C.create_string_buffer(1024)
        self._check(self.lib.zasr_model_routes(self.handle, buf, len(buf)))
        return json.loads(buf.value.decode())

    def set_mel_banks(self, banks) -> None:
        b = _f32(banks)
# ... 334 lines not shown
```

Measured before the change: 134,600 audio-sec/sec.

## Fuse adjacent input projections into the wide FFN kernel as side projections

Adds optional pre and post side projections to the fused wide FFN kernel. The attention-in and nonlin-attention-in projections read the FFN input tile already staged in LDS, and the second self-attention value projection reads the FFN output written back to LDS as bf16. This removes three separate bf16 GEMM launches per layer and their re-reads of X, and packs the projection weights into MFMA fragment layout at load time. In exchange the FFN kernel does more work per block, and its launch bounds change for D=256, which may affect occupancy and register pressure. The feature is on by default and controlled by ZASR_FFN_PROJ.

```diff
diff --git a/include/zasr.h b/include/zasr.h
--- a/include/zasr.h
+++ b/include/zasr.h
@@ -158,6 +158,14 @@
 int zasr_selftest_ffn_h3_oop(int32_t R, int32_t D, int32_t F, const float* W1, const float* b1,
                              const float* W2, const float* b2, const float* byp_orig,
                              const float* byp_scale, float* X, float* Xout);
+int zasr_selftest_ffn_bf16_proj(int32_t R, int32_t D, int32_t F, const float* W1, const float* b1,
+                                const float* W2, const float* b2, const float* byp_orig,
+                                const float* byp_scale, float* X, float* Xout, int32_t n_pre,
+                                const float* W_pre, const float* b_pre, uint16_t* pre_out,
+                                uint16_t* pre_ref, int32_t n_post, const float* W_post,
+                                const float* b_post, uint16_t* post_out, uint16_t* post_ref,
+                                float* X_ref);
+int zasr_selftest_ffn_proj_pack(int32_t n, int32_t D, const float* W, uint16_t* out);
 int zasr_selftest_seam(int32_t nseq, const int32_t* L, int32_t d, int32_t ds, int32_t dn,
                        int32_t ds_next, int32_t c0, int32_t ldo, const float* xd,
                        const float* orig, const float* s, const float* wn8, const float* wo2,
diff --git a/sherpa-vietnamese-asr_amd/csrc/engine.cpp b/sherpa-vietnamese-asr_amd/csrc/engine.cpp
--- a/sherpa-vietnamese-asr_amd/csrc/engine.cpp
+++ b/sherpa-vietnamese-asr_amd/csrc/engine.cpp
@@ -247,6 +247,7 @@
   hw_host_ = build_hotword_dfa(hotwords, hotword_scores, cfg.V);
   ZASR_HIP_CHECK(hipSetDevice(device_));
   if (const char* e = getenv("ZASR_SEARCH_CUS")) search_cus_ = atoi(e);
+  ffn_proj_sites_ = ffn_proj_sites_from_env();
   int ncu = 0;
   ZASR_HIP_CHECK(hipDeviceGetAttribute(&ncu, hipDeviceAttributeMultiprocessorCount, device_));
   if (search_cus_ > 0 && search_cus_ < ncu) {
@@ -639,6 +640,26 @@
             l->wp = p;
           }
         }
+    if (ffn_proj_sites_ != 0)
+      for (auto& s : model_.stacks)
+        for (auto& L : s.layers) {
+          struct Site { DLin* l; int ff, bit; };
+          for (const Site& t : {Site{&L.attn_in, 0, kFfnProjAttn}, Site{&L.na_in, 0, kFfnProjNa},
+                                Site{&L.sa_in[1], 1, kFfnProjSa}}) {
+            DLin* l = t.l;
+            if (!(ffn_proj_sites_ & t.bit) || L.ff_in[t.ff].wp == nullptr || l->K < 256 ||
+                (l->bh ? l->bh : l->b) == nullptr || !ffn_proj_supported(l->K, l->N))
+              continue;
+            std::vector<__bf16> h((size_t)l->N * l->K), pk(ffn_proj_packed_elems(l->N, l->K));
+            ZASR_HIP_CHECK(hipMemcpy(h.data(), l->wh, h.size() * 2, hipMemcpyDeviceToHost));
+            ffn_proj_pack_host(h.data(), l->N, l->K, pk.data());
+            void* p = nullptr;
+            ZASR_HIP_CHECK(hipMalloc(&p, pk.size() * 2));
+            model_.allocations.push_back(p);
+            ZASR_HIP_CHECK(hipMemcpy(p, pk.data(), pk.size() * 2, hipMemcpyHostToDevice));
+            l->wp = p;
+          }
+        }
   }
   {
     const double gb = (double)cfg.V * cfg.V * cfg.joiner_dim * 4.0 / 1e9;
@@ -1025,6 +1046,19 @@
       ZASR_HIP_CHECK(hipMemcpyAsync(O, X, (size_t)R * d * sizeof(float), hipMemcpyDeviceToDevice, st_));
   }
   const bool bf16 = precision_ == 1 || precision_ == 2;
+  auto proj_on = [&](const DLin& l, int k) {
+    return bf16 && l.wp != nullptr && Ly.ff_in[k].wh && Ly.ff_in[k].wp && ffn_proj_supported(d, l.N);
+  };
+  auto proj_of = [&](const DLin& l, void* out, int ld) {
+    FfnProj q;
+    q.w = l.wp;
+    q.b = l.bh ? l.bh : l.b;
+    q.out = out;
+    q.n = l.N;
+    q.ld = ld;
+    return q;
+  };
+  FfnProj pj_attn, pj_na, pj_sa;
   const int np = split_pieces();
   float* qkp = nullptr;
   float* A = nullptr;
@@ -1033,7 +1067,10 @@
   AttnFlashArgs fa{};
   if (bf16) {
     __bf16* qkp16 = ws<__bf16>("ly_qkp_h", (size_t)R * 68 * h);
-    linear_h(Ly.attn_in, X, false, d, R, qkp16, true, 68 * h, EPI_NONE);
+    if (proj_on(Ly.attn_in, 0))
+      pj_attn = proj_of(Ly.attn_in, qkp16, 68 * h);
+    else
+      linear_h(Ly.attn_in, X, false, d, R, qkp16, true, 68 * h, EPI_NONE);
     A16 = ws<__bf16>("ly_attn_h", 1);
     stats = ws<float>("ly_attn_stats", (size_t)R * h);
     fa = AttnFlashArgs{qkp16, h, Ly.pos_tab, model_.pmax, d_off, d_aoff, B, maxL, A16,
@@ -1063,17 +1100,21 @@
     launch_attn_softmax(a, st_);
     prof_end();
   }
-  auto ff = [&](int k, const float* src = nullptr) {
+  auto ff = [&](int k, const float* src = nullptr, const FfnProj* pre = nullptr,
+                const FfnProj* post = nullptr) {
     const DLin& fi = Ly.ff_in[k];
     const float* bo = (bf16 && k == 1) ? O : nullptr;
     const float* bs = (bf16 && k == 1) ? Ly.bypass_mid : nullptr;
     if (fi.wh && ffn_fused_supported(d) && (d < 256 || fi.wp)) {
       prof_begin("ffn_fused");
       launch_ffn_fused(X, R, d, fi.N, d < 256 ? fi.wh : fi.wp, fi.b,
-                       d < 256 ? Ly.ff_out[k].wh : Ly.ff_out[k].wp, Ly.ff_out[k].b, st_, bo, bs, src);
+                       d < 256 ? Ly.ff_out[k].wh : Ly.ff_out[k].wp, Ly.ff_out[k].b, st_, bo, bs, src,
+                       pre, post);
       prof_end();
       return;
     }
+    ZASR_REQUIRE((pre == nullptr || pre->w == nullptr) && (post == nullptr || post->w == nullptr),
+                 "feed-forward: side projections need the wide fused kernel");
     ZASR_REQUIRE(src == nullptr || (!fi.wh && fi.wp && np == kPiecesF16),
                  "feed-forward: only the fused kernels run out of place");
     if (fi.wh) {
@@ -1097,7 +1138,8 @@
     if (bf16) {
       __bf16* vv = ws<__bf16>("ly_vv_h", (size_t)R * 12 * h);
       __bf16* oa = ws<__bf16>("ly_oa_h", (size_t)R * 12 * h);
-      linear_h(Ly.sa_in[k], X, false, d, R, vv, true, 12 * h, EPI_NONE);
+      if (!(k == 1 && pj_sa.w != nullptr))
+        linear_h(Ly.sa_in[k], X, false, d, R, vv, true, 12 * h, EPI_NONE);
       AttnFlashArgs a = fa;
       a.v = vv;
       a.out = oa;
@@ -1165,17 +1207,22 @@
     }
     linear(Ly.cv_out[k], dc, d, R, X, d, EPI_RESADD);
   };
+  __bf16* h3_pj = nullptr;
+  if (proj_on(Ly.na_in, 0)) {
+    h3_pj = ws<__bf16>("ly_h3_h", (size_t)R * 3 * hid);
+    pj_na = proj_of(Ly.na_in, h3_pj, 3 * hid);
+  }
   if (oop) {
     X = Xalt;
-    ff(0, O);
+    ff(0, O, &pj_attn, &pj_na);
   } else {
-    ff(0);
+    ff(0, nullptr, &pj_attn, &pj_na);
   }
   if (bf16) {
     __bf16* h3 = ws<__bf16>("ly_h3_h", (size_t)R * 3 * hid);
     __bf16* t1t = ws<__bf16>("ly_t1t", (size_t)hid * R8);
     __bf16* z = ws<__bf16>("ly_z_h", (size_t)R * hid);
-    linear_h(Ly.na_in, X, false, d, R, h3, true, 3 * hid, EPI_NONE);
+    if (h3_pj == nullptr) linear_h(Ly.na_in, X, false, d, R, h3, true, 3 * hid, EPI_NONE);
     prof_begin("elementwise");
     launch_nonlin_prep_t(h3, true, d_off, d_o8, d_map, R, hid, R8, t1t, st_);
     prof_end();
@@ -1264,7 +1311,9 @@
   }
   self_attn(0);
   conv(0);
-  ff(1);
+  if (proj_on(Ly.sa_in[1], 1))
+    pj_sa = proj_of(Ly.sa_in[1], ws<__bf16>("ly_vv_h", (size_t)R * 12 * h), 12 * h);
+  ff(1, nullptr, nullptr, &pj_sa);
   if (!bf16 && Ly.ff_out[1].wx == nullptr) {
     prof_begin("elementwise");
     launch_bypass(X, O, Ly.bypass_mid, R, d, st_);
diff --git a/sherpa-vietnamese-asr_amd/csrc/engine.h b/sherpa-vietnamese-asr_amd/csrc/engine.h
--- a/sherpa-vietnamese-asr_amd/csrc/engine.h
+++ b/sherpa-vietnamese-asr_amd/csrc/engine.h
@@ -209,6 +209,7 @@
                                bool c16, int epi);
   bool prof_on_ = false;
   bool prof_shapes_ = false;
+  int ffn_proj_sites_ = 0;
   std::vector<ProfEvent> prof_pending_;
   std::map<std::string, std::pair<long, double>> prof_acc_;
   std::vector<hipEvent_t> event_pool_;
diff --git a/sherpa-vietnamese-asr_amd/csrc/ffn_kernels.hip b/sherpa-vietnamese-asr_amd/csrc/ffn_kernels.hip
--- a/sherpa-vietnamese-asr_amd/csrc/ffn_kernels.hip
+++ b/sherpa-vietnamese-asr_amd/csrc/ffn_kernels.hip
@@ -54,6 +54,94 @@
 __device__ __forceinline__ void lds_signal(int* p, int lane) {
   asm volatile("s_waitcnt lgkmcnt(0)" ::: "memory");
   if (lane == 0) __hip_atomic_fetch_add(p, 1, __ATOMIC_RELEASE, __HIP_MEMORY_SCOPE_WORKGROUP);
+}
+
+struct FfnProjDev {
+  const __bf16* w;
+  const float* b;
+  __bf16* out;
+  int n, ld;
+};
+struct FfnProjPair {
+  FfnProjDev pre, post;
+};
+
+template <int D>
+__device__ __forceinline__ void ffn_side_proj(const __bf16* sX, const FfnProjDev pj, long t0, int R,
+                                              int wid, int lane) {
+  typedef __bf16 bf16x2 __attribute__((ext_vector_type(2)));
+  constexpr int XLD = D + 16, KS = D / 16, PF = 4;
+  const int col = lane & 31, h2 = lane >> 5;
+  const int ng = (pj.n + 31) >> 5;
+  const __amdgpu_buffer_rsrc_t rs = wave_rsrc(pj.w, (long)ng * 32 * D * 2);
+  const int voff = lane * 16;
+  bf16x8 ring[PF];
+  auto unit = [&](int g, auto nt_c, int tile0, int so_next) __attribute__((always_inline)) {
+    constexpr int NT = decltype(nt_c)::value;
+    const int so = g * (KS * 1024);
+    f32x16 acc[NT];
+#pragma unroll
+    for (int t = 0; t < NT; ++t)
+#pragma unroll
+      for (int r = 0; r < 16; ++r) acc[t][r] = 0.f;
+    const __bf16* xb = &sX[(tile0 * 32 + col) * XLD + 8 * h2];
+#pragma unroll 1
+    for (int s0 = 0; s0 < KS; s0 += PF) {
+      const int nso = s0 + PF < KS ? so + (s0 + PF) * 1024 : so_next;
+#pragma unroll
+      for (int i = 0; i < PF; ++i) {
+        bf16x8 b[NT];
+#pragma unroll
+        for (int t = 0; t < NT; ++t)
+          b[t] = *reinterpret_cast<const bf16x8*>(xb + t * 32 * XLD + 16 * (s0 + i));
+#pragma unroll
+        for (int t = 0; t < NT; ++t)
+          acc[t] = __builtin_amdgcn_mfma_f32_32x32x16_bf16(ring[i], b[t], acc[t], 0, 0, 0);
+        ring[i] = buf_load16<bf16x8>(rs, voff, nso + i * 1024);
+      }
+    }
+    float4 bb[4];
+#pragma unroll
+    for (int q = 0; q < 4; ++q)
+      bb[q] = *reinterpret_cast<const float4*>(pj.b + min(g * 32 + 8 * q + 4 * h2, pj.n - 4));
+#pragma unroll
+    for (int t = 0; t < NT; ++t) {
+      const long tok = t0 + (tile0 + t) * 32 + col;
+      unsigned pk[4][2];
+#pragma unroll
+      for (int q = 0; q < 4; ++q) {
+        const bf16x2 lo = {(__bf16)(acc[t][4 * q + 0] + bb[q].x), (__bf16)(acc[t][4 * q + 1] + bb[q].y)};
+        const bf16x2 hi = {(__bf16)(acc[t][4 * q + 2] + bb[q].z), (__bf16)(acc[t][4 * q + 3] + bb[q].w)};
+        pk[q][0] = __builtin_bit_cast(unsigned, lo);
+        pk[q][1] = __builtin_bit_cast(unsigned, hi);
+      }
+#pragma unroll
+      for (int gp = 0; gp < 2; ++gp) {
+        const auto s0 = __builtin_amdgcn_permlane32_swap(pk[2 * gp][0], pk[2 * gp + 1][0], false, false);
+        const auto s1 = __builtin_amdgcn_permlane32_swap(pk[2 * gp][1], pk[2 * gp + 1][1], false, false);
+        const uint4 v = make_uint4(s0[0], s1[0], s0[1], s1[1]);
+        const int n = g * 32 + 16 * gp + 8 * h2;
+        if (tok < R && n < pj.n) *reinterpret_cast<uint4*>(pj.out + tok * pj.ld + n) = v;
+      }
+    }
+  };
+  using I1 = std::integral_constant<int, 1>;
+  using I2 = std::integral_constant<int, 2>;
+  const int full = ng & ~7, rem = ng - full;
+  const bool tail2 = rem > 4 && wid < rem, tail1 = rem <= 4 && wid < 2 * rem;
+  const int tg = full + (rem > 4 ? wid : wid >> 1);
+  const int tso = (tail1 || tail2) ? tg * (KS * 1024) : 0;
+  {
+    const int so0 = full > 0 ? wid * (KS * 1024) : tso;
+#pragma unroll
+    for (int i = 0; i < PF; ++i) ring[i] = buf_load16<bf16x8>(rs, voff, so0 + i * 1024);
+  }
+  for (int g = wid; g < full; g += 8) unit(g, I2{}, 0, g + 8 < full ? (g + 8) * (KS * 1024) : tso);
+  if (tail2) {
+    unit(tg, I2{}, 0, tso);
+  } else if (tail1) {
+    unit(tg, I1{}, wid & 1, tso);
+  }
 }
 
 template <int D, bool OOP = false>
@@ -206,15 +294,16 @@
     }
 }
 
-template <int D, bool EB = true, bool OOP = false>
-__global__ __launch_bounds__(512, 1) void ffn_wide_kernel(float* __restrict__ X, int R, int F,
+template <int D, bool EB = true, bool OOP = false, bool PRE = false, bool POST = false>
+__global__ __launch_bounds__(512, (D == 256 && (PRE || POST)) ? 4 : 1) void ffn_wide_kernel(float* __restrict__ X, int R, int F,
                                                           const __bf16* __restrict__ W1,
                                                           const float* __restrict__ b1,
                                                           const __bf16* __restrict__ W2,
                                                           const float* __restrict__ b2,
                                                           const float* __restrict__ byp_orig,
                                                           const float* __restrict__ byp_scale,
-                                                          const float* __restrict__ Xsrc) {
+                                                          const float* __restrict__ Xsrc,
+                                                          const FfnProjPair pj) {
   const float* Xin = OOP ? Xsrc : X;
   typedef float f32x4 __attribute__((ext_vector_type(4)));
   constexpr int TT = 64, HC = 128, NW = 8;
@@ -283,11 +372,18 @@
   };
   using I0 = std::integral_constant<int, 0>;
   using I1 = std::integral_constant<int, W2S - 1>;
-  load_w1(0);
-  load_w2(0, I0{});
+  if constexpr (!PRE) {
+    load_w1(0);
+    load_w2(0, I0{});
+  }
   for (int e = tid; e < F; e += 64 * NW) sB1[e] = b1[e];
   lds_barrier();
   FFN_STAMP(1)
+  if constexpr (PRE) {
+    ffn_side_proj<D>(sX, pj.pre, t0, R, wid, lane);
+    load_w1(0);
+    load_w2(0, I0{});
+  }
   auto chunk = [&](int c, auto set) {
     constexpr int S = decltype(set)::value;
     const int hid0 = c * HC + wid * 16;
@@ -389,11 +485,16 @@
           v.w = b0.w + (v.w - b0.w) * k.w;
         }
         *reinterpret_cast<float4*>(xr + ch) = v;
-      }
-    }
-    }
-    return;
-  }
+        if constexpr (POST) {
+          const bf16x4 b = {(__bf16)v.x, (__bf16)v.y, (__bf16)v.z, (__bf16)v.w};
+          *reinterpret_cast<bf16x4*>(&sX[(16 * u + r16) * XLD + ch]) = b;
+        }
+      }
+    }
+    }
+    if constexpr (!POST) return;
+  }
+  if constexpr (!EB) {
 #pragma unroll
   for (int u = 0; u < 4; ++u) {
     const long tok = t0 + 16 * u + r16;
@@ -418,7 +519,16 @@
         v.w = b0.w + (v.w - b0.w) * k.w;
       }
       *reinterpret_cast<float4*>(xr + ch) = v;
-    }
+      if constexpr (POST) {
+        const bf16x4 b = {(__bf16)v.x, (__bf16)v.y, (__bf16)v.z, (__bf16)v.w};
+        *reinterpret_cast<bf16x4*>(&sX[(16 * u + r16) * XLD + ch]) = b;
+      }
+    }
+  }
+  }
+  if constexpr (POST) {
+    lds_barrier();
+    ffn_side_proj<D>(sX, pj.post, t0, R, wid, lane);
   }
 }
 
@@ -1082,15 +1192,57 @@
   return D == 64 || D == 96 || D == 128 || D == 192 || D == 256 || D == 384 || D == 512;
 }
 
+bool ffn_proj_supported(int D, int n) {
+  return (D == 256 || D == 384 || D == 512) && n >= 8 && n % 8 == 0 && !ffn_rows_on();
+}
+size_t ffn_proj_packed_elems(int n, int D) { return (size_t)((n + 31) / 32 * 32) * D; }
+void ffn_proj_pack_host(const __bf16* w, int n, int D, __bf16* out) {
+  const int np = (n + 31) / 32 * 32;
+  std::vector<__bf16> pad((size_t)np * D, (__bf16)0.f);
+  std::memcpy(pad.data(), w, (size_t)n * D * sizeof(__bf16));
+  pack_frag32_host(pad.data(), np, D, out);
+}
+int ffn_proj_sites_from_env() {
+  const char* e = getenv("ZASR_FFN_PROJ");
+  if (e == nullptr || *e == 0 || std::strcmp(e, "1") == 0) return kFfnProjAttn | kFfnProjNa | kFfnProjSa;
+  if (std::strcmp(e, "0") == 0) return 0;
+  int sites = 0;
+  for (const char* p = e; *p;) {
+    const char* q = std::strchr(p, ',');
+    const size_t len = q ? (size_t)(q - p) : std::strlen(p);
+    if (len == 4 && std::strncmp(p, "attn", 4) == 0) sites |= kFfnProjAttn;
+    else if (len == 2 && std::strncmp(p, "na", 2) == 0) sites |= kFfnProjNa;
+    else if (len == 2 && std::strncmp(p, "sa", 2) == 0) sites |= kFfnProjSa;
+    else ZASR_REQUIRE(false, "ZASR_FFN_PROJ: 0, 1 or a comma list of attn, na, sa");
+    p = q ? q + 1 : p + len;
+  }
+  return sites;
+}
+
 void launch_ffn_fused(float* X, int R, int D, int F, const void* W1, const float* b1,
                       const void* W2, const float* b2, hipStream_t st, const float* byp_orig,
-                      const float* byp_scale, const float* Xin) {
+                      const float* byp_scale, const float* Xin, const FfnProj* pre,
+                      const FfnProj* post) {
   if (R <= 0) return;
   if (Xin == X) Xin = nullptr;
   ZASR_REQUIRE(ffn_fused_supported(D), "ffn_fused: unsupported model dim");
   ZASR_REQUIRE(F % 8 == 0, "ffn_fused: feed-forward dim must be a multiple of 8");
   const __bf16* w1 = reinterpret_cast<const __bf16*>(W1);
   const __bf16* w2 = reinterpret_cast<const __bf16*>(W2);
+  if (pre != nullptr && pre->w == nullptr) pre = nullptr;
+  if (post != nullptr && post->w == nullptr) post = nullptr;
+  FfnProjPair pj{};
+  for (const FfnProj* q : {pre, post}) {
+    if (q == nullptr) continue;
+    ZASR_REQUIRE(ffn_proj_supported(D, q->n), "ffn_fused: side projection needs D in {256, 384, 512}, "
+                                              "n a multiple of 8, and not the rows form");
+    ZASR_REQUIRE(q->b != nullptr && q->out != nullptr && q->ld >= q->n && q->ld % 8 == 0 &&
+                     (reinterpret_cast<uintptr_t>(q->out) & 15) == 0,
+                 "ffn_fused: side projection needs a bias and a 16-byte aligned output, ld % 8 == 0");
+    FfnProjDev& dv = q == pre ? pj.pre : pj.post;
+    dv = FfnProjDev{reinterpret_cast<const __bf16*>(q->w), q->b, reinterpret_cast<__bf16*>(q->out),
+                    q->n, q->ld};
+  }
   if (D >= 256) {
     ZASR_REQUIRE(F % 32 == 0 && F >= 32 && F <= kMaxF,
                  "ffn_fused: feed-forward dim must be a multiple of 32 in [32, 2048] for D >= 256");
@@ -1114,21 +1266,33 @@
                     b1, w2, b2, byp_orig, byp_scale, rpb, Xin);
       return;
     }
-#define ZASR_FFNW(DV)                                                                                  \
+#define ZASR_FFNW_(DV, PR, PO)                                                                         \
   if (Xin != nullptr)                                                                                  \
-    ZASR_LAUNCH((ffn_wide_kernel<DV, DV == 384, true>), grid, dim3(512), 0, st, X, R, F, w1, b1, w2, b2, \
-                byp_orig, byp_scale, Xin);                                                             \
+    ZASR_LAUNCH((ffn_wide_kernel<DV, DV == 384, true, PR, PO>), grid, dim3(512), 0, st, X, R, F, w1, b1, \
+                w2, b2, byp_orig, byp_scale, Xin, pj);                                                 \
   else                                                                                                 \
-    ZASR_LAUNCH((ffn_wide_kernel<DV, DV == 384, false>), grid, dim3(512), 0, st, X, R, F, w1, b1, w2,  \
-                b2, byp_orig, byp_scale, Xin)
+    ZASR_LAUNCH((ffn_wide_kernel<DV, DV == 384, false, PR, PO>), grid, dim3(512), 0, st, X, R, F, w1,  \
+                b1, w2, b2, byp_orig, byp_scale, Xin, pj)
+#define ZASR_FFNW(DV)                              \
+  if (pre && post) {                               \
+    ZASR_FFNW_(DV, true, true);                    \
+  } else if (pre) {                                \
+    ZASR_FFNW_(DV, true, false);                   \
+  } else if (post) {                               \
+    ZASR_FFNW_(DV, false, true);                   \
+  } else {                                         \
+    ZASR_FFNW_(DV, false, false);                  \
+  }
     switch (D) {
       case 256: ZASR_FFNW(256); break;
       case 384: ZASR_FFNW(384); break;
       default: ZASR_FFNW(512); break;
     }
 #undef ZASR_FFNW
+#undef ZASR_FFNW_
     return;
   }
+  ZASR_REQUIRE(pre == nullptr && post == nullptr, "ffn_fused: side projections need D >= 256");
   const dim3 grid(cdiv(R, kTok));
 #define ZASR_FFN(DV)                                                                                \
   if (Xin != nullptr)                                                                               \
diff --git a/sherpa-vietnamese-asr_amd/csrc/kernels.h b/sherpa-vietnamese-asr_amd/csrc/kernels.h
--- a/sherpa-vietnamese-asr_amd/csrc/kernels.h
+++ b/sherpa-vietnamese-asr_amd/csrc/kernels.h
@@ -30,6 +30,18 @@
 void selftest_ffn_bf16(int R, int D, int F, const float* W1, const float* b1, const float* W2,
                        const float* b2, const float* byp_orig, const float* byp_scale, float* X,
                        int form, float* Xout = nullptr);
+struct SelftestProj {
+  int n = 0;
+  const float* W = nullptr;
+  const float* b = nullptr;
+  uint16_t* out = nullptr;
+  uint16_t* ref = nullptr;
+};
+void selftest_ffn_bf16_proj(int R, int D, int F, const float* W1, const float* b1, const float* W2,
+                            const float* b2, const float* byp_orig, const float* byp_scale,
+                            float* X, float* Xout, const SelftestProj& pre,
+                            const SelftestProj& post, float* X_ref);
+void selftest_ffn_proj_pack(int n, int D, const float* W, uint16_t* out);
 
 struct CamppConv2d {
   const float* x;
@@ -276,10 +288,22 @@
 
 bool ffn_fused_supported(int D);
 void ffn_pack_host(const __bf16* w, int rows, int cols, __bf16* out);
+struct FfnProj {
+  const void* w = nullptr;
+  const float* b = nullptr;
+  void* out = nullptr;
+  int n = 0, ld = 0;
+};
+bool ffn_proj_supported(int D, int n);
+size_t ffn_proj_packed_elems(int n, int D);
+void ffn_proj_pack_host(const __bf16* w, int n, int D, __bf16* out);
+enum { kFfnProjAttn = 1, kFfnProjNa = 2, kFfnProjSa = 4 };
+int ffn_proj_sites_from_env();
 void launch_ffn_fused(float* X, int R, int D, int F, const void* W1, const float* b1,
                       const void* W2, const float* b2, hipStream_t st,
                       const float* byp_orig = nullptr, const float* byp_scale = nullptr,
-                      const float* Xin = nullptr);
+                      const float* Xin = nullptr, const FfnProj* pre = nullptr,
+                      const FfnProj* post = nullptr);
 bool ffn_h3_supported(int D, int F);
 void ffn_h3_set_split(int on);
 void ffn_set_rows(int on);
diff --git a/sherpa-vietnamese-asr_amd/csrc/selftest.cpp b/sherpa-vietnamese-asr_amd/csrc/selftest.cpp
--- a/sherpa-vietnamese-asr_amd/csrc/selftest.cpp
+++ b/sherpa-vietnamese-asr_amd/csrc/selftest.cpp
@@ -118,6 +118,112 @@
   ZASR_HIP_CHECK(hipDeviceSynchronize());
   ZASR_HIP_CHECK(hipMemcpy(X, dX.p, xb, hipMemcpyDeviceToHost));
   if (Xout) ZASR_HIP_CHECK(hipMemcpy(Xout, dO.p, xb, hipMemcpyDeviceToHost));
+}
+
+void selftest_ffn_proj_pack(int n, int D, const float* W, uint16_t* out) {
+  ZASR_REQUIRE(n >= 1 && D >= 16 && D % 16 == 0, "selftest ffn_proj_pack: n >= 1, D % 16 == 0");
+  std::vector<__bf16> h((size_t)n * D), pk(ffn_proj_packed_elems(n, D));
+  for (size_t i = 0; i < h.size(); ++i) h[i] = (__bf16)W[i];
+  ffn_proj_pack_host(h.data(), n, D, pk.data());
+  std::memcpy(out, pk.data(), pk.size() * 2);
+}
+
+void selftest_ffn_bf16_proj(int R, int D, int F, const float* W1, const float* b1, const float* W2,
+                            const float* b2, const float* byp_orig, const float* byp_scale,
+                            float* X, float* Xout, const SelftestProj& pre,
+                            const SelftestProj& post, float* X_ref) {
+  ZASR_REQUIRE(R >= 1, "selftest ffn_bf16_proj: R >= 1");
+  ZASR_REQUIRE(D >= 256 && ffn_fused_supported(D), "selftest ffn_bf16_proj: D in {256, 384, 512}");
+  ZASR_REQUIRE(!ffn_rows_on(), "selftest ffn_bf16_proj: not with the rows form");
+  std::vector<__bf16> h1((size_t)F * D), h2((size_t)D * F), p1(h1.size()), p2(h2.size());
+  for (size_t i = 0; i < h1.size(); ++i) h1[i] = (__bf16)W1[i];
+  for (size_t i = 0; i < h2.size(); ++i) h2[i] = (__bf16)W2[i];
+  ffn_pack_host(h1.data(), F, D, p1.data());
+  ffn_pack_host(h2.data(), D, F, p2.data());
+  const size_t xb = (size_t)R * D * 4;
+  DevBuf dX(xb), rX(xb), d1(p1.size() * 2), d2(p2.size() * 2), db1((size_t)F * 4),
+      db2((size_t)D * 4), dbo(byp_orig ? xb : 4), dbs((size_t)D * 4), dO(Xout ? xb : 4),
+      rO(Xout ? xb : 4);
+  up(dX, X, xb);
+  up(rX, X, xb);
+  if (Xout) {
+    up(dO, Xout, xb);
+    up(rO, Xout, xb);
+  }
+  up(d1, p1.data(), p1.size() * 2);
+  up(d2, p2.data(), p2.size() * 2);
+  up(db1, b1, (size_t)F * 4);
+  up(db2, b2, (size_t)D * 4);
+  if (byp_orig) {
+    ZASR_REQUIRE(byp_scale != nullptr, "selftest ffn_bf16_proj: bypass needs its scale");
+    up(dbo, byp_orig, xb);
+    up(dbs, byp_scale, (size_t)D * 4);
+  }
+  struct Side {
+    std::unique_ptr<DevBuf> wh, wp, b, out, ref;
+    FfnProj d;
+  } sd[2];
+  const SelftestProj* sp[2] = {&pre, &post};
+  for (int k = 0; k < 2; ++k) {
+    const SelftestProj& q = *sp[k];
+    if (q.n <= 0) continue;
+    ZASR_REQUIRE(q.W && q.b && q.out && q.ref, "selftest ffn_bf16_proj: null projection operand");
+    ZASR_REQUIRE(ffn_proj_supported(D, q.n), "selftest ffn_bf16_proj: unsupported projection width");
+    std::vector<__bf16> h((size_t)q.n * D), pk(ffn_proj_packed_elems(q.n, D));
+    for (size_t i = 0; i < h.size(); ++i) h[i] = (__bf16)q.W[i];
+    ffn_proj_pack_host(h.data(), q.n, D, pk.data());
+    const size_t ob = (size_t)R * q.n * 2;
+    sd[k].wh.reset(new DevBuf(h.size() * 2));
+    sd[k].wp.reset(new DevBuf(pk.size() * 2));
+    sd[k].b.reset(new DevBuf((size_t)q.n * 4));
+    sd[k].out.reset(new DevBuf(ob));
+    sd[k].ref.reset(new DevBuf(ob));
+    up(*sd[k].wh, h.data(), h.size() * 2);
+    up(*sd[k].wp, pk.data(), pk.size() * 2);
+    up(*sd[k].b, q.b, (size_t)q.n * 4);
+    up(*sd[k].out, q.out, ob);
+    up(*sd[k].ref, q.out, ob);
+    sd[k].d.w = sd[k].wp->p;
+    sd[k].d.b = sd[k].b->as<float>();
+    sd[k].d.out = sd[k].out->p;
+    sd[k].d.n = sd[k].d.ld = q.n;
+  }
+  const float* bo = byp_orig ? dbo.as<float>() : nullptr;
+  const float* bs = byp_orig ? dbs.as<float>() : nullptr;
+  launch_ffn_fused(Xout ? dO.as<float>() : dX.as<float>(), R, D, F, d1.p, db1.as<float>(), d2.p,
+                   db2.as<float>(), nullptr, bo, bs, Xout ? dX.as<float>() : nullptr, &sd[0].d,
+                   &sd[1].d);
+  auto gemm = [&](int k, const float* A) {
+    GemmParams p{};
+    p.A = A;
+    p.lda = D;
+    p.B = nullptr;
+    p.sbk = 1;
+    p.sbn = D;
+    p.C = sd[k].ref->as<float>();
+    p.ldc = sp[k]->n;
+    p.bias = sd[k].b->as<float>();
+    p.M = R;
+    p.N = sp[k]->n;
+    p.K = D;
+    p.alpha = 1.f;
+    p.max_M = R;
+    gemm_bf16(p, sd[k].wh->p, EPI_NONE, ALOAD_DENSE, nullptr, false, true);
+  };
+  if (pre.n > 0) gemm(0, rX.as<float>());
+  launch_ffn_fused(Xout ? rO.as<float>() : rX.as<float>(), R, D, F, d1.p, db1.as<float>(), d2.p,
+                   db2.as<float>(), nullptr, bo, bs, Xout ? rX.as<float>() : nullptr);
+  if (post.n > 0) gemm(1, Xout ? rO.as<float>() : rX.as<float>());
+  ZASR_HIP_CHECK(hipDeviceSynchronize());
+  ZASR_HIP_CHECK(hipMemcpy(X, dX.p, xb, hipMemcpyDeviceToHost));
+  if (Xout) ZASR_HIP_CHECK(hipMemcpy(Xout, dO.p, xb, hipMemcpyDeviceToHost));
+  ZASR_HIP_CHECK(hipMemcpy(X_ref, Xout ? rO.p : rX.p, xb, hipMemcpyDeviceToHost));
+  for (int k = 0; k < 2; ++k) {
+    if (sp[k]->n <= 0) continue;
+    const size_t ob = (size_t)R * sp[k]->n * 2;
+    ZASR_HIP_CHECK(hipMemcpy(sp[k]->out, sd[k].out->p, ob, hipMemcpyDeviceToHost));
+    ZASR_HIP_CHECK(hipMemcpy(sp[k]->ref, sd[k].ref->p, ob, hipMemcpyDeviceToHost));
+  }
 }
 
 void selftest_seam(int nseq, const int* L, int d, int ds, int dn, int ds_next, int c0, int ldo,
diff --git a/sherpa-vietnamese-asr_amd/csrc/zasr_api.cpp b/sherpa-vietnamese-asr_amd/csrc/zasr_api.cpp
--- a/sherpa-vietnamese-asr_amd/csrc/zasr_api.cpp
+++ b/sherpa-vietnamese-asr_amd/csrc/zasr_api.cpp
@@ -691,6 +691,32 @@
   });
 }
 
+int zasr_selftest_ffn_bf16_proj(int32_t R, int32_t D, int32_t F, const float* W1, const float* b1,
+                                const float* W2, const float* b2, const float* byp_orig,
+                                const float* byp_scale, float* X, float* Xout, int32_t n_pre,
+                                const float* W_pre, const float* b_pre, uint16_t* pre_out,
+                                uint16_t* pre_ref, int32_t n_post, const float* W_post,
+                                const float* b_post, uint16_t* post_out, uint16_t* post_ref,
+                                float* X_ref) {
+  if (!W1 || !b1 || !W2 || !b2 || !X || !X_ref) return fail(ZASR_ERR_INVALID, "null argument");
+  if (n_pre <= 0 && n_post <= 0) return fail(ZASR_ERR_INVALID, "no projection given");
+  return guarded([&]() {
+    zasr::SelftestProj pre{n_pre, W_pre, b_pre, pre_out, pre_ref};
+    zasr::SelftestProj post{n_post, W_post, b_post, post_out, post_ref};
+    zasr::selftest_ffn_bf16_proj(R, D, F, W1, b1, W2, b2, byp_orig, byp_scale, X, Xout, pre, post,
+                                 X_ref);
+    return (int)ZASR_OK;
+  });
+}
+
+int zasr_selftest_ffn_proj_pack(int32_t n, int32_t D, const float* W, uint16_t* out) {
+  if (!W || !out) return fail(ZASR_ERR_INVALID, "null argument");
+  return guarded([&]() {
+    zasr::selftest_ffn_proj_pack(n, D, W, out);
+    return (int)ZASR_OK;
+  });
+}
+
 int zasr_selftest_ffn_h3_oop(int32_t R, int32_t D, int32_t F, const float* W1, const float* b1,
                              const float* W2, const float* b2, const float* byp_orig,
                              const float* byp_scale, float* X, float* Xout) {
diff --git a/sherpa-vietnamese-asr_amd/zasr/binding.py b/sherpa-vietnamese-asr_amd/zasr/binding.py
--- a/sherpa-vietnamese-asr_amd/zasr/binding.py
+++ b/sherpa-vietnamese-asr_amd/zasr/binding.py
@@ -31,7 +31,7 @@
     "zasr_fbank_set_mel_banks", "zasr_selftest_launch", "zasr_decode_host_batches",
     "zasr_selftest_gemm_h3r", "zasr_selftest_ffn_h3", "zasr_selftest_ffn_bf16",
     "zasr_selftest_attn_block_map", "zasr_selftest_seam", "zasr_selftest_ffn_bf16_oop",
-    "zasr_selftest_ffn_h3_oop",
+    "zasr_selftest_ffn_h3_oop", "zasr_selftest_ffn_bf16_proj", "zasr_selftest_ffn_proj_pack",
 )
 
 
@@ -219,6 +219,12 @@
     lib.zasr_selftest_ffn_bf16_oop.restype = C.c_int
     lib.zasr_selftest_ffn_h3_oop.argtypes = [I32, I32, I32] + [fp] * 8
     lib.zasr_selftest_ffn_h3_oop.restype = C.c_int
+    u16p = C.POINTER(C.c_uint16)
+    lib.zasr_selftest_ffn_bf16_proj.argtypes = ([I32, I32, I32] + [fp] * 8 +
+                                                [I32, fp, fp, u16p, u16p] * 2 + [fp])
+    lib.zasr_selftest_ffn_bf16_proj.restype = C.c_int
+    lib.zasr_selftest_ffn_proj_pack.argtypes = [I32, I32, fp, u16p]
+    lib.zasr_selftest_ffn_proj_pack.restype = C.c_int
     if path is None:
         _lib = lib
     return lib
@@ -332,6 +338,53 @@
     if rc != 0:
         raise ZasrError(lib.zasr_last_error().decode())
     return out, X
+
+
+def selftest_ffn_bf16_proj(W1, b1, W2, b2, X, byp_orig=None, byp_scale=None, pre=None, post=None,
+                           oop: bool = False, fill: float = -777.25, fill16: int = 0x7FC1,
+                           lib_path: Optional[str] = None) -> dict:
+    lib = load_library(lib_path)
+    W1, b1, W2, b2, X = (_f32(v) for v in (W1, b1, W2, b2, X))
+    X = X.copy()
+    R = X.shape[0]
+    out = np.full(X.shape, fill, dtype=np.float32) if oop else None
+    xref = np.empty_like(X)
+    bo = None if byp_orig is None else _f32(byp_orig)
+    bs = None if byp_scale is None else _f32(byp_scale)
+    p = lambda x: None if x is None else x.ctypes.data_as(C_FP)
+    p16 = lambda x: None if x is None else x.ctypes.data_as(C.POINTER(C.c_uint16))
+    sides, keep = [], {}
+    for name, pr in (("pre", pre), ("post", post)):
+        if pr is None:
+            sides += [0, None, None, None, None]
+            continue
+        W, b = _f32(pr[0]), _f32(pr[1])
+        o = np.full((R, W.shape[0]), fill16, dtype=np.uint16)
+        r = o.copy()
+        keep[name], keep[name + "_ref"], keep[name + "_w"] = o, r, (W, b)
+        sides += [W.shape[0], p(W), p(b), p16(o), p16(r)]
+    rc = lib.zasr_selftest_ffn_bf16_proj(R, X.shape[1], W1.shape[0], p(W1), p(b1), p(W2), p(b2),
+                                         p(bo), p(bs), p(X), p(out), *sides, p(xref))
+    if rc != 0:
+        raise ZasrError(lib.zasr_last_error().decode())
+    res = {k: v for k, v in keep.items() if not k.endswith("_w")}
+    res["x"] = out if oop else X
+    res["x_ref"] = xref
+    if oop:
+        res["x_in"] = X
+    return res
+
+
+def selftest_ffn_proj_pack(W, lib_path: Optional[str] = None) -> np.ndarray:
+    lib = load_library(lib_path)
+    W = _f32(W)
+    n, D = W.shape
+    out = np.empty(((n + 31) // 32, D // 16, 64, 8), dtype=np.uint16)
+    rc = lib.zasr_selftest_ffn_proj_pack(n, D, W.ctypes.data_as(C_FP),
+                                         out.ctypes.data_as(C.POINTER(C.c_uint16)))
+    if rc != 0:
+        raise ZasrError(lib.zasr_last_error().decode())
+    return out
 
 
 def selftest_seam(L, d: int, ds: int, dn: int, ds_next: int, c0: int, ldo: int, xd, orig, s,
```

Result: no change. 134,200 audio-sec/sec (-0.3%).
